# oxfordcontrol/Clarabel.rs

Measured on AMD Instinct MI355X. Metric: IPM iterations/sec (KKT factor+solve) at n=10^6 SOCP, 1/2/4/8 GPUs, higher is better.
Workload: dtype f64

## Files before the change

### clarabel.rs_amd/__init__.py

```python
import ctypes as C
import os
import subprocess

import numpy as np

_HERE = os.path.dirname(os.path.abspath(__file__))
LIB_PATH = os.environ.get("CLARABEL_HIP_LIB") or os.path.join(_HERE, "libclarabel_hip.so")
SHIP_LIB_PATH = os.path.join(_HERE, "libclarabel_hip_ship.so")
HEADER_PATH = os.path.join(os.path.dirname(_HERE), "include", "clarabel_hip.h")

u64 = np.uint64
f64 = np.float64
P_U64 = C.POINTER(C.c_uint64)
P_I64 = C.POINTER(C.c_int64)
P_F64 = C.POINTER(C.c_double)
P_I8 = C.POINTER(C.c_int8)
P_I32 = C.POINTER(C.c_int32)

OK, ERR_DIM, ERR_EMPTY_COLUMN, ERR_NOT_TRIU, ERR_ZERO_PIVOT, ERR_BAD_PERM = 0, -1, -2, -3, -4, -5
ERR_NOT_FACTORED, ERR_NO_DEVICE, ERR_HIP, ERR_ARG, ERR_UNSUPPORTED = -6, -7, -8, -9, -10
ERR_UPDATE_NOT_ALLOWED = -11
STATUS_NAMES = {0: "ok", -1: "IncompatibleDimension", -2: "EmptyColumn", -3: "NotUpperTriangular",
                -4: "ZeroPivot", -5: "InvalidPermutation", -6: "NotFactored", -7: "NoDevice", -8: "HipError",
                -9: "BadArgument", -10: "Unsupported", -11: "UpdateNotAllowed"}
# ... 1471 lines not shown
            continue
        if form[0] == "full":
            idxs.append(offsets[k] + np.arange(length, dtype=np.int64))
        elif form[0] == "partial":
            if np.any(form[1] >= np.uint64(length)):
                raise ChipError(ERR_DIM, "update %s: member %d: an index is out of the member's range" % (key, k))
            idxs.append(offsets[k] + form[1].astype(np.int64))
        else:
            raise TypeError("update %s: member %d: the entries of a list are host arrays" % (key, k))
        vals.append(form[2])
    if not idxs:
        return ("none",)
    return ("partial", _u(np.concatenate(idxs)), _f(np.concatenate(vals)))


COMM_ID_BYTES = 128


def comm_unique_id():
    buf = (C.c_uint8 * COMM_ID_BYTES)()
    _check(lib().chip_comm_get_unique_id(buf), "chip_comm_get_unique_id")
    return bytes(buf)


class Comm:

    def __init__(self, unique_id, world, rank, device=-1):
        assert len(unique_id) == COMM_ID_BYTES
        self._h = C.c_void_p()
        buf = (C.c_uint8 * COMM_ID_BYTES).from_buffer_copy(unique_id)
        _check(lib().chip_comm_create(C.byref(self._h), buf, C.c_int32(world), C.c_int32(rank), C.c_int32(device)),
               "chip_comm_create")
        self.world, self.rank = world, rank

    def __del__(self):
        if getattr(self, "_h", None):
            lib().chip_comm_destroy(self._h)
            self._h = None

    def attach(self, kkt):
        _check(lib().chip_kkt_attach_comm(kkt._h, self._h), "attach_comm")

    def allgather_step(self, kkt, send_ptr, recv_ptr, counts):
        cnt = np.ascontiguousarray(counts, dtype=np.int64)
        assert len(cnt) == self.world
        _check(lib().chip_kkt_allgather_step(kkt._h, self._h, C.c_void_p(send_ptr), C.c_void_p(recv_ptr),
                                             cnt.ctypes.data_as(P_I64)), "allgather_step")

    def wait(self, kkt):
        _check(lib().chip_kkt_wait_comm(kkt._h, self._h), "wait_comm")

    def debug_spin(self, blocks, threads=256, usec=60.0):
        lib().chip_comm_debug_spin.argtypes = [C.c_void_p, C.c_int32, C.c_int32, C.c_double]
        _check(lib().chip_comm_debug_spin(self._h, blocks, threads, float(usec)), "comm_debug_spin")

    def synchronize(self):
        _check(lib().chip_comm_synchronize(self._h), "comm_synchronize")

    def allreduce(self, vals, op="sum"):
        v = np.ascontiguousarray(np.atleast_1d(vals), dtype=np.float64).copy()
        _check(lib().chip_comm_allreduce(self._h, _pf(v), C.c_int32(len(v)), C.c_int32({"sum": 0, "min": 1, "max": 2}[op])),
               "comm_allreduce")
        return v

    def barrier(self):
        self.allreduce([0.0])


_HIPRT = None


def _hiprt():
    global _HIPRT
    if _HIPRT is None:
        lib()
        _HIPRT = C.CDLL("libamdhip64.so.7")
    return _HIPRT


class DeviceArray:

    def __init__(self, n_or_array):
        rt = _hiprt()
        host = None
        if not np.isscalar(n_or_array):
            host = _f(n_or_array)
            n = len(host)
        else:
            n = int(n_or_array)
        self.n = n
        self._p = C.c_void_p()
        rc = rt.hipMalloc(C.byref(self._p), C.c_size_t(max(n, 1) * 8))
        if rc != 0:
            raise RuntimeError("hipMalloc failed: %d" % rc)
        if host is not None:
            self.copy_from(host)
        else:
            rt.hipMemset(self._p, 0, C.c_size_t(max(n, 1) * 8))

    @classmethod
    def view(cls, ptr, n):
        a = cls.__new__(cls)
        a.n = int(n)
        a._p = C.c_void_p(ptr)
        a._borrowed = True
        return a

    @property
    def ptr(self):
        return self._p.value

    def copy_from(self, host):
        host = _f(host)
        assert len(host) == self.n
        rc = _hiprt().hipMemcpy(self._p, host.ctypes.data_as(C.c_void_p), C.c_size_t(self.n * 8), C.c_int(1))
        if rc != 0:
            raise RuntimeError("hipMemcpy H2D failed: %d" % rc)

    def numpy(self):
        out = np.zeros(self.n)
        rc = _hiprt().hipMemcpy(out.ctypes.data_as(C.c_void_p), self._p, C.c_size_t(self.n * 8), C.c_int(2))
        if rc != 0:
            raise RuntimeError("hipMemcpy D2H failed: %d" % rc)
        return out

    def __del__(self):
        if getattr(self, "_borrowed", False):
            return
        if getattr(self, "_p", None) and self._p.value:
            try:
                _hiprt().hipFree(self._p)
            except Exception:
                pass
            self._p = C.c_void_p()


def debug_spin(device, blocks, threads=256, lds_bytes=0, usec=1000.0):
    lib().chip_debug_spin.argtypes = [C.c_int32, C.c_int32, C.c_int32, C.c_int32, C.c_double]
    _check(lib().chip_debug_spin(device, blocks, threads, lds_bytes, float(usec)), "debug_spin")


def debug_set_switch(name, value=None):
    lib().chip_debug_set_switch.argtypes = [C.c_char_p, C.c_char_p]
    _check(lib().chip_debug_set_switch(name.encode(), None if value is None else str(value).encode()), "debug_set_switch")


def debug_counter(kkt, name):
    out = C.c_double(0.0)
    lib().chip_debug_counter.argtypes = [C.c_void_p, C.c_char_p, C.POINTER(C.c_double)]
    _check(lib().chip_debug_counter(kkt._h, name.encode(), C.byref(out)), "debug_counter")
    return out.value


def set_device(ordinal):
    rc = _hiprt().hipSetDevice(C.c_int(int(ordinal)))
    if rc != 0:
        raise RuntimeError("hipSetDevice(%d) failed: %d" % (ordinal, rc))


def device_synchronize():
    _hiprt().hipDeviceSynchronize()
```

### clarabel.rs_amd/csrc/bundle_ir.hip

```cpp
#include "dev_common.hpp"
#include "bundle_symv.hpp"
#include "grid_sync.hpp"

namespace chip {
namespace dev {

namespace {

constexpr int IR_SH_FWD = 3, IR_SH_BWD = 3, IR_SH_SYMV = 3;
constexpr int IR_RPT = 2;
constexpr int IR_FATCAP = 256;

template <bool FWDMODE, int SH, int RPT, int TW>
__device__ __forceinline__ void bundle_sweep_cols(const LdlView &v, const BundleView &bv, int b, double *xs,
                                                  const double *xt, double *tacc, int k, int *fat, int &nfat,
                                                  const double *__restrict__ dinv = nullptr) {
    constexpr int CH = RPT * TW;
    const int s0 = bv.bundle_ptr[b], nloc = bv.bundle_ptr[b + 1] - s0;
    const int *lv = bv.blvl + bv.blvl_ptr[b];
    const int nl = bv.blvl_ptr[b + 1] - bv.blvl_ptr[b] - 1;
    const int lane = threadIdx.x & 63, wv = threadIdx.x >> 6;
    if (FWDMODE && (int)threadIdx.x < 8) tacc[threadIdx.x] = 0.0;
    double tpart = 0.0;
    struct Chunk {
// ... 97 lines not shown
#pragma unroll
                        for (int e = 0; e < SH; ++e) {
                            ii[u][e] = (tb[u] + e < te[u]) ? ci[u][e] : -1;
                            vv[u][e] = cv[u][e];
                        }
                } else {
#pragma unroll
                    for (int u = 0; u < RPT; ++u)
#pragma unroll
                        for (int e = 0; e < SH; ++e) {
                            const unsigned t = (unsigned)(tb[u] + kk + e);
                            const bool ok = (int)t < te[u];
                            ii[u][e] = ok ? (int)v.Li16[t] : -1;
                            vv[u][e] = ok ? v.Lx[t] : 0.0;
                        }
                }
#pragma unroll
                for (int u = 0; u < RPT; ++u)
#pragma unroll
                    for (int e = 0; e < SH; ++e) {
                        const int i = ii[u][e];
                        if (FWDMODE) {
                            const double val = vv[u][e] * yj[u];
                            int tgt = -1;
                            if (i >= 0) {
                                if (i < nloc) tgt = i;
                                else if (k == 1) tpart += val;
                                else atomicAdd(&tacc[i - nloc], val);
                            }
                            lds_scatter_add(xs, tgt, -val);
                        } else if (i >= 0) {
                            sum[u] += vv[u][e] * (i < nloc ? xs[i] : xt[i - nloc]);
                        }
                    }
            }
            if (!FWDMODE) {
#pragma unroll
                for (int u = 0; u < RPT; ++u)
                    if (jr[u] >= 0) xs[jr[u] - s0] = xs[jr[u] - s0] * dj[u] - sum[u];
            }
        }
        if (!FWDMODE && level_ends) {
            __syncthreads();
            const int nf = min(nfat, IR_FATCAP);
            for (int f = wv; f < nf; f += TW / 64) {
                const int j = fat[f];
                double sacc = 0.0;
                for (int t = v.Lp[j] + lane; t < v.Lp[j + 1]; t += 64) {
                    const int i = (int)v.Li16[t];
                    sacc += v.Lx[t] * (i < nloc ? xs[i] : xt[i - nloc]);
                }
                sacc = wave_sum(sacc);
                if (lane == 0) xs[j - s0] -= sacc;
            }
        }
        cur = nx1;
        nx1 = nx2;
        nx2 = advance(nx2);
    }
    __syncthreads();
    if (FWDMODE && k == 1) {
        tpart = wave_sum_all(tpart);
        if (lane == 0 && tpart != 0.0) atomicAdd(&tacc[0], tpart);
        __syncthreads();
    }
}

constexpr int FLAT_U = 4;
constexpr int FLAT_MAXLEV = 64;
constexpr int FLAT_MIN_NODES = 512;
__device__ __forceinline__ void flat_level_table(const LdlView &v, const BundleView &bv, int b, int *lev_e) {
    const int *lv = bv.blvl + bv.blvl_ptr[b];
    const int nl = bv.blvl_ptr[b + 1] - bv.blvl_ptr[b] - 1;
    if ((int)threadIdx.x <= nl && nl <= FLAT_MAXLEV) lev_e[threadIdx.x] = v.Lp[lv[threadIdx.x]];
}
template <bool FWDMODE, int TW>
__device__ __forceinline__ void bundle_sweep_flat(const LdlView &v, const BundleView &bv, int b, double *xs,
                                                  const double *xt, double *tacc, int k, const int *lev_e, int dl = 0) {
    const int s0 = bv.bundle_ptr[b], nloc = bv.bundle_ptr[b + 1] - s0;
    const int nl = bv.blvl_ptr[b + 1] - bv.blvl_ptr[b] - 1;
    int tid = threadIdx.x;
    asm volatile("" : "+v"(tid));
    const int lane = tid & 63;
    if (FWDMODE && tid < 8) tacc[tid] = 0.0;
    if (!FWDMODE)
        for (int i = tid; i < nloc; i += TW) xs[i] *= v.Dinv[s0 + i];
    double tpart = 0.0;
    int step = 0, base = 0, ee = 0;
    auto level_range = [&](int st_, int &eb_, int &ee_) {
        const int l = FWDMODE ? st_ : nl - 1 - st_;
        eb_ = lev_e[l];
        ee_ = lev_e[l + 1];
    };
    auto skip_empty = [&]() {
        while (step < nl) {
            level_range(step, base, ee);
            if (base < ee) return;
            ++step;
        }
    };
    lds_barrier();
    if (TW == 512) {
        for (int st_ = 0; st_ < nl; ++st_) {
            int eb_, ee_;
            level_range(st_, eb_, ee_);
            for (int bs = eb_; bs < ee_; bs += TW * FLAT_U) {
                int ii[FLAT_U], jj[FLAT_U];
                double vv[FLAT_U];
#pragma unroll
                for (int u = 0; u < FLAT_U; ++u) {
                    const int t = bs + u * TW + tid;
                    const bool ok = t < ee_;
                    ii[u] = ok ? (int)v.Li16[t + dl] : -1;
                    jj[u] = ok ? (int)v.Lj16[t + dl] : 0;
                    vv[u] = ok ? v.Lx[t] : 0.0;
                }
#pragma unroll
                for (int u = 0; u < FLAT_U; ++u) {
                    const int i = ii[u];
                    if (i < 0) continue;
                    if (FWDMODE) {
                        const double val = vv[u] * xs[jj[u]];
                        if (i < nloc) atomicAdd(&xs[i], -val);
                        else if (k == 1) tpart += val;
                        else atomicAdd(&tacc[i - nloc], val);
                    } else {
                        atomicAdd(&xs[jj[u]], -(vv[u] * (i < nloc ? xs[i] : xt[i - nloc])));
                    }
                }
            }
            lds_barrier();
        }
        if (FWDMODE && k == 1) {
            tpart = wave_sum_all(tpart);
            if (lane == 0 && tpart != 0.0) atomicAdd(&tacc[0], tpart);
        }
        lds_barrier();
        return;
    }
    skip_empty();
    int ci[FLAT_U], cj[FLAT_U], ni[FLAT_U], nj[FLAT_U];
    double cv[FLAT_U], nv[FLAT_U];
    auto request = [&](int bs, int en, int *ii, int *jj, double *vv) {
#pragma unroll
        for (int u = 0; u < FLAT_U; ++u) {
            const int t = bs + u * TW + tid;
            const bool ok = t < en;
            ii[u] = ok ? (int)v.Li16[t + dl] : -1;
            jj[u] = ok ? (int)v.Lj16[t + dl] : 0;
            vv[u] = ok ? v.Lx[t] : 0.0;
        }
    };
    if (step < nl) request(base, ee, ci, cj, cv);
    while (step < nl) {
        int nstep = step, nbase = base + TW * FLAT_U, nee = ee;
        if (nbase >= nee) {
            nstep = step + 1;
            while (nstep < nl) {
                level_range(nstep, nbase, nee);
                if (nbase < nee) break;
                ++nstep;
            }
        }
        if (nstep < nl) request(nbase, nee, ni, nj, nv);
#pragma unroll
        for (int u = 0; u < FLAT_U; ++u) {
            const int i = ci[u];
            if (i < 0) continue;
            if (FWDMODE) {
                const double val = cv[u] * xs[cj[u]];
                if (i < nloc) atomicAdd(&xs[i], -val);
                else if (k == 1) tpart += val;
                else atomicAdd(&tacc[i - nloc], val);
            } else {
                atomicAdd(&xs[cj[u]], -(cv[u] * (i < nloc ? xs[i] : xt[i - nloc])));
            }
        }
        if (nstep != step) lds_barrier();
        step = nstep;
        base = nbase;
        ee = nee;
#pragma unroll
        for (int u = 0; u < FLAT_U; ++u) {
            ci[u] = ni[u];
            cj[u] = nj[u];
            cv[u] = nv[u];
        }
    }
    if (FWDMODE && k == 1) {
        tpart = wave_sum_all(tpart);
        if (lane == 0 && tpart != 0.0) atomicAdd(&tacc[0], tpart);
    }
    lds_barrier();
}

template <int TW>
__device__ __forceinline__ void bundle_symv_flat(const LdlView &v, const BundleView &bv, const double *x,
                                                 const double *__restrict__ b, double *spill, double *xs, double *red,
                                                 int k, int bid, const double *xt, double *out_norm, double *out_share) {
    const int *__restrict__ Up = v.Up;
    const unsigned short *__restrict__ Ucol16 = v.Ucol16, *__restrict__ Urow16 = v.Urow16;
    const double *__restrict__ Ux = v.Ux;
    const int s0 = bv.bundle_ptr[bid], nloc = bv.bundle_ptr[bid + 1] - s0;
    const int nleaf = bv.blvl[bv.blvl_ptr[bid] + 1] - s0, nin = nloc - nleaf;
    int tid = threadIdx.x;
    asm volatile("" : "+v"(tid));
    auto xpos = [&](int t) { return t < nleaf ? t : nloc + (t - nleaf); };
    constexpr int LR = 4, LS = 3;
    int tb[LR], te[LR];
#pragma unroll
    for (int u = 0; u < LR; ++u) {
        const int i = tid + u * TW;
        tb[u] = i < nleaf ? Up[s0 + i] : 0;
        te[u] = i < nleaf ? Up[s0 + i + 1] : 0;
    }
    const int fb = Up[s0 + nleaf], fe = Up[s0 + nloc];
    for (int t = tid; t < nin; t += TW) {
        const double xv = x[s0 + nleaf + t], bv_ = b[s0 + nleaf + t];
        xs[xpos(t)] = xv;
        xs[nleaf + t] = bv_;
    }
    double tpart = 0.0;
    __shared__ double tacc3[8];
    if (k > 1 && tid < 8) tacc3[tid] = 0.0;
    double mleaf = 0.0;
    bool nan = false;
    __syncthreads();
    for (int w0 = 0; w0 < nleaf; w0 += LR * TW) {
        int jj[LR][LS];
        double vv[LR][LS], xi[LR], bi[LR], acc[LR];
#pragma unroll
        for (int u = 0; u < LR; ++u) {
            const int i = w0 + tid + u * TW;
            xi[u] = i < nleaf ? x[s0 + i] : 0.0;
            bi[u] = i < nleaf ? b[s0 + i] : 0.0;
            acc[u] = 0.0;
#pragma unroll
            for (int q = 0; q < LS; ++q) {
                const int t = tb[u] + q;
                const bool ok = t < te[u];
                jj[u][q] = ok ? (int)Ucol16[t] : -1;
                vv[u][q] = ok ? Ux[t] : 0.0;
            }
        }
#pragma unroll
        for (int u = 0; u < LR; ++u) {
            const int i = w0 + tid + u * TW;
            auto apply = [&](int j, double val) {
                if (j >= nloc) {
                    acc[u] += val * xt[j - nloc];
                    if (k == 1) tpart += val * xi[u];
                    else atomicAdd(&tacc3[j - nloc], val * xi[u]);
                } else if (j == i) {
                    acc[u] += val * xi[u];
                } else {
                    acc[u] += val * xs[xpos(j - nleaf)];
                    atomicAdd(&xs[j], -(val * xi[u]));
                }
            };
#pragma unroll
            for (int q = 0; q < LS; ++q)
                if (jj[u][q] >= 0) apply(jj[u][q], vv[u][q]);
            for (int t = tb[u] + LS; t < te[u]; ++t) apply((int)Ucol16[t], Ux[t]);
            if (i < nleaf) {
                const double val = bi[u] - acc[u];
                spill[s0 + i] = val;
                if (val != val) nan = true;
                else mleaf = fmax(mleaf, fabs(val));
            }
            const int in = i + LR * TW;
            tb[u] = in < nleaf ? Up[s0 + in] : 0;
            te[u] = in < nleaf ? Up[s0 + in + 1] : 0;
        }
    }
    int ii[FLAT_U], jj[FLAT_U], ni[FLAT_U], nj[FLAT_U];
    double vv[FLAT_U], nv[FLAT_U];
    auto request = [&](int bs, int *pi, int *pj, double *pv) {
#pragma unroll
        for (int u = 0; u < FLAT_U; ++u) {
            const int t = bs + u * TW + tid;
            const bool ok = t < fe;
            pi[u] = ok ? (int)Urow16[t] : -1;
            pj[u] = ok ? (int)Ucol16[t] : 0;
            pv[u] = ok ? Ux[t] : 0.0;
        }
    };
    if (fb < fe) request(fb, ii, jj, vv);
    for (int base = fb; base < fe; base += TW * FLAT_U) {
        if (base + TW * FLAT_U < fe) request(base + TW * FLAT_U, ni, nj, nv);
        else {
#pragma unroll
            for (int u = 0; u < FLAT_U; ++u) ni[u] = -1;
        }
#pragma unroll
        for (int u = 0; u < FLAT_U; ++u) {
            const int i = ii[u], j = jj[u];
            if (i < 0) continue;
            const double xi = xs[xpos(i - nleaf)];
            if (j >= nloc) {
                atomicAdd(&xs[i], -(vv[u] * xt[j - nloc]));
                if (k == 1) tpart += vv[u] * xi;
                else atomicAdd(&tacc3[j - nloc], vv[u] * xi);
            } else if (j == i) {
                atomicAdd(&xs[i], -(vv[u] * xi));
            } else {
                atomicAdd(&xs[i], -(vv[u] * xs[xpos(j - nleaf)]));
// ... 407 lines not shown
                    for (int i = tid; i < nloc; i += TW) alt[s0 + i] = xs[i];
                } else {
                    for (int i = tid; i < nloc; i += TW) alt[s0 + i] = 1.0 * cur[s0 + i] + 1.0 * xs[i];
                }
                if (!ir.ir_enable) {
                    double mx = 0.0;
                    bool nan = false;
                    for (int i = tid; i < nloc; i += TW) {
                        const double val = xs[i];
                        if (val != val) nan = true;
                        else mx = fmax(mx, fabs(val));
                    }
                    mx = block_max(mx, red);
                    const bool anynan = __syncthreads_or(nan);
                    if (tid == 0) ir_store(&pn[(size_t)par * nb + b], anynan ? __longlong_as_double(0x7ff8000000000000ll) : mx);
                    continue;
                }
                __syncthreads();
                stamp();
                double *share_out = GR ? &gf.rsh[((size_t)par * nb + b) * 8] : &shs[(size_t)par * nb * k + (size_t)b * k];
                if (single && bv.symv_split && flat)
                    bundle_symv_flat<TW>(v, bv, alt, ir.bp, ir.ebuf, xs, red, k, b, st.candt, &pn[(size_t)par * nb + b], share_out);
                else if (single && bv.symv_split)
                    bundle_symv_split<IR_SH_SYMV, TW, 2>(bv, v.Up, v.Ucol16, v.Ux, alt, ir.bp, ir.ebuf, xs, red, k, b, st.candt,
                                                         &pn[(size_t)par * nb + b], share_out);
                else
                    bundle_symv_body<true, IR_SH_SYMV, TW, 2>(bv, v.Up, (const int *)v.Ucol16, v.Ux, alt, ir.bp, single ? nullptr : ir.ebuf, nullptr, nullptr,
                                       xs, red, lfold, b, st.candt, &pn[(size_t)par * nb + b], share_out);
                if (GR && grp >= 0) {
                    ++gph;
                    if (ir_group_arrive(gf.gcnt + grp * 32, gnb * gph)) {
                        group_sums(gf.rsh + (size_t)par * nb * 8);
                        if (tid == 0) {
                            double m = 0.0, mb = 0.0;
                            for (int i = 0; i < k; ++i) {
                                double sacc = st.tacc[i];
                                for (int c = 0; c < k; ++c) sacc += st.ktt[i * 8 + c] * st.candt[c];
                                const double rt = st.btop[i] - sacc;
                                ir_store(&grec[par * 32 + 16 + i], rt);
                                m = nanmax(m, fabs(rt));
                                mb = nanmax(mb, fabs(st.btop[i]));
                            }
                            ir_store(&grec[par * 32 + 24], m);
                            ir_store(&grec[par * 32 + 25], mb);
                        }
                    }
                }
            }
        }
        if (stop) break;
        pending = true;
        const bool more_possible = ir.ir_enable && round < ir.maxiter;
        if (GR && more_possible) {
            if (tid == 0) st.gen += 1;
            if (ir_arrive_nowait(ir.ctl, st.gen, G) == IR_LAST) {
                reduce_residual(par, round == 0);
                ir_release(ir.ctl, st.gen, G);
            }
            continue;
        }
        if (folded && more_possible) continue;
        stamp();
        if (tid == 0) st.gen += 1;
        const int state = ir_arrive_wait(ir.ctl, st.gen, G);
        if (state == IR_TIMEOUT) {
            if (tid == 0) ir.res[2] = 1;
            return;
        }
        stamp();
        if (state == IR_LAST) {
            reduce_residual(par, round == 0);
            ir_release(ir.ctl, st.gen, G);
        }
        __syncthreads();
        decide(round, par);
        pending = false;
        if (__builtin_amdgcn_readfirstlane(st.done)) break;
    }
    stamp();
    const int ok = __builtin_amdgcn_readfirstlane(st.ok);
    if (ok) {
        double *cur = __builtin_amdgcn_readfirstlane(st.sel) ? ir.xb : ir.xa;
        auto put = [&](int j, double val) {
            const int o = ir.perm[j];
            if (o < ir.n) {
                if (ir.lhsx) ir.lhsx[o] = val;
            } else if (o < ir.n + ir.m) {
                if (ir.lhsz) ir.lhsz[o - ir.n] = val;
            }
        };
        for (int b = blockIdx.x; b < nb; b += G) {
            const int s0 = bv.bundle_ptr[b], nloc = bv.bundle_ptr[b + 1] - s0;
            const int nruns = ir.runs ? ir.run_ptr[b + 1] - ir.run_ptr[b] : 0;
            if (nruns > 0 && nruns <= IR_MAXRUNS) {
                __syncthreads();
                if (tid < 3 * nruns) st.runs[tid] = ir.runs[3 * ir.run_ptr[b] + tid];
                __syncthreads();
                int r = 0;
                for (int i = tid; i < nloc; i += TW) {
                    while (i >= st.runs[3 * r] + st.runs[3 * r + 2]) ++r;
                    const int o = st.runs[3 * r + 1] + (i - st.runs[3 * r]);
                    const double val = cur[s0 + i];
                    if (o < ir.n) {
                        if (ir.lhsx) ir.lhsx[o] = val;
                    } else if (o < ir.n + ir.m) {
                        if (ir.lhsz) ir.lhsz[o - ir.n] = val;
                    }
                }
            } else {
                for (int i = tid; i < nloc; i += TW) put(s0 + i, cur[s0 + i]);
            }
        }
        if ((GR ? gfirst : blockIdx.x == 0) && tid < k) {
            put(topnode(tid), st.curt[tid]);
            cur[topnode(tid)] = st.curt[tid];
        }
    }
    if (GR && gfirst && tid == 0) {
        __hip_atomic_store(gf.gcnt + grp * 32, 0, __ATOMIC_RELAXED, __HIP_MEMORY_SCOPE_AGENT);
        __hip_atomic_store(gf.gcnt + grp * 32 + 1, 0, __ATOMIC_RELAXED, __HIP_MEMORY_SCOPE_AGENT);
    }
    if (blockIdx.x == 0 && tid == 0) {
        ir.res[0] = ok ? 1 : -1;
        ir.res[1] = st.rounds;
        ir.res[3] = st.sel;
        pub[64] = st.normb;
        pub[65] = st.norme;
    }
    stamp();
    ir_grid_exit(ir.ctl, __builtin_amdgcn_readfirstlane(st.gen) + 1, G);
}


constexpr int IRS_NPT = 12;
__device__ __forceinline__ int opaque_tid() {
    int t = threadIdx.x;
    asm volatile("" : "+v"(t));
    return t;
}

struct RunWalk {
    const int *runs;
    int r;
    __device__ __forceinline__ int orig(int i) {
        while (i >= runs[3 * r] + runs[3 * r + 2]) ++r;
        return runs[3 * r + 1] + (i - runs[3 * r]);
    }
};

template <int TW, int NPT, int NLP>
__device__ __forceinline__ void irs_symv(const LdlView &v, const IrView &ir, const int *runs, const double (&c)[NPT],
                                         bool keep_e, double *xs, double *red, double *tacc3, int k, int s0,
                                         int nloc, int nleaf, const double *xt, double *out_norm, double *out_share,
                                         int du) {
    double cl[NLP];
    const int *__restrict__ Up = v.Up;
    const unsigned short *__restrict__ Ucol16 = v.Ucol16, *__restrict__ Urow16 = v.Urow16;
    const double *__restrict__ Ux = v.Ux;
    const int tid = opaque_tid();
    auto xpos = [&](int t) { return t < nleaf ? t : nloc + (t - nleaf); };
    auto rhs_of = [&](int o) { return o < ir.n ? ir.rx[o] : (o < ir.n + ir.m ? ir.rz[o - ir.n] : 0.0); };
    constexpr int LR = 4, LS = 3;
    static_assert(NLP % LR == 0 && NLP <= NPT, "leaf passes");
    int tb[LR], te[LR];
#pragma unroll
    for (int u = 0; u < LR; ++u) {
        const int i = tid + u * TW;
        tb[u] = i < nleaf ? Up[s0 + i] : 0;
        te[u] = i < nleaf ? Up[s0 + i + 1] : 0;
    }
    const int fb = Up[s0 + nleaf], fe = Up[s0 + nloc];
    {
        RunWalk rw{runs, 0};
        double bq[NPT];
#pragma unroll
        for (int u = 0; u < NPT; ++u) {
            const int i = tid + u * TW;
            bq[u] = (i >= nleaf && i < nloc) ? rhs_of(rw.orig(i)) : 0.0;
        }
        lds_barrier();
#pragma unroll
        for (int u = 0; u < NPT; ++u) {
            const int i = tid + u * TW;
            if (i >= nleaf && i < nloc) {
                xs[xpos(i - nleaf)] = c[u];
                xs[i] = bq[u];
            }
        }
#pragma unroll
        for (int u = 0; u < NLP; ++u) cl[u] = c[u];
    }
    double tpart = 0.0;
    if (k > 1 && tid < 8) tacc3[tid] = 0.0;
    double mleaf = 0.0;
    bool nan = false;
    lds_barrier();
    RunWalk rl{runs, 0};
#pragma unroll
    for (int p = 0; p < NLP / LR; ++p) {
        if (p * LR * TW < nleaf) {
            int jj[LR][LS];
            double vv[LR][LS], bi[LR], acc[LR];
#pragma unroll
            for (int u = 0; u < LR; ++u) {
                const int i = (p * LR + u) * TW + tid;
                bi[u] = i < nleaf ? rhs_of(rl.orig(i)) : 0.0;
                acc[u] = 0.0;
#pragma unroll
                for (int q = 0; q < LS; ++q) {
                    const int t = tb[u] + q;
                    const bool ok = t < te[u];
                    jj[u][q] = ok ? (int)Ucol16[t + du] : -1;
                    vv[u][q] = ok ? Ux[t] : 0.0;
                }
            }
#pragma unroll
            for (int u = 0; u < LR; ++u) {
                const int i = (p * LR + u) * TW + tid;
                const double xi = cl[p * LR + u];
                auto apply = [&](int j, double val) {
                    if (j >= nloc) {
                        acc[u] += val * xt[j - nloc];
                        if (k == 1) tpart += val * xi;
                        else atomicAdd(&tacc3[j - nloc], val * xi);
                    } else if (j == i) {
                        acc[u] += val * xi;
                    } else {
                        acc[u] += val * xs[xpos(j - nleaf)];
                        atomicAdd(&xs[j], -(val * xi));
                    }
                };
#pragma unroll
                for (int q = 0; q < LS; ++q)
                    if (jj[u][q] >= 0) apply(jj[u][q], vv[u][q]);
                for (int t = tb[u] + LS; t < te[u]; ++t) apply((int)Ucol16[t + du], Ux[t]);
                if (i < nleaf) {
                    const double val = bi[u] - acc[u];
                    if (keep_e) cl[p * LR + u] = val;
                    if (val != val) nan = true;
                    else mleaf = fmax(mleaf, fabs(val));
                }
                const int in = i + LR * TW;
                tb[u] = in < nleaf ? Up[s0 + in] : 0;
                te[u] = in < nleaf ? Up[s0 + in + 1] : 0;
            }
        }
    }
    {
        int ii[FLAT_U], jj[FLAT_U], ni[FLAT_U], nj[FLAT_U];
        double vv[FLAT_U], nv[FLAT_U];
        auto request = [&](int bs, int *pi, int *pj, double *pv) {
#pragma unroll
            for (int u = 0; u < FLAT_U; ++u) {
                const int t = bs + u * TW + tid;
                const bool ok = t < fe;
                pi[u] = ok ? (int)Urow16[t + du] : -1;
                pj[u] = ok ? (int)Ucol16[t + du] : 0;
                pv[u] = ok ? Ux[t] : 0.0;
            }
        };
        if (fb < fe) request(fb, ii, jj, vv);
        for (int base = fb; base < fe; base += TW * FLAT_U) {
            if (base + TW * FLAT_U < fe) request(base + TW * FLAT_U, ni, nj, nv);
            else {
#pragma unroll
                for (int u = 0; u < FLAT_U; ++u) ni[u] = -1;
            }
#pragma unroll
            for (int u = 0; u < FLAT_U; ++u) {
                const int i = ii[u], j = jj[u];
                if (i < 0) continue;
                const double xi = xs[xpos(i - nleaf)];
                if (j >= nloc) {
                    atomicAdd(&xs[i], -(vv[u] * xt[j - nloc]));
                    if (k == 1) tpart += vv[u] * xi;
                    else atomicAdd(&tacc3[j - nloc], vv[u] * xi);
                } else if (j == i) {
                    atomicAdd(&xs[i], -(vv[u] * xi));
                } else {
                    atomicAdd(&xs[i], -(vv[u] * xs[xpos(j - nleaf)]));
                    atomicAdd(&xs[j], -(vv[u] * xi));
                }
            }
#pragma unroll
            for (int u = 0; u < FLAT_U; ++u) {
                ii[u] = ni[u];
                jj[u] = nj[u];
                vv[u] = nv[u];
            }
        }
    }
    lds_barrier();
    double m = mleaf;
#pragma unroll
    for (int u = 0; u < NPT; ++u) {
        const int i = tid + u * TW;
        if (i >= nleaf && i < nloc) {
            const double val = xs[i];
            if (val != val) nan = true;
            else m = fmax(m, fabs(val));
        }
    }
    if (keep_e) {
#pragma unroll
        for (int u = 0; u < NLP; ++u)
            if (tid + u * TW < nleaf) xs[tid + u * TW] = cl[u];
    }
    m = block_max(m, red);
    const bool anynan = __syncthreads_or(nan);
    if (tid == 0)
        __hip_atomic_store(out_norm, anynan ? __longlong_as_double(0x7ff8000000000000ll) : m, __ATOMIC_RELAXED,
                           __HIP_MEMORY_SCOPE_AGENT);
    if (k == 1) {
        tpart = block_sum(tpart, red);
        if (tid == 0) __hip_atomic_store(out_share, tpart, __ATOMIC_RELAXED, __HIP_MEMORY_SCOPE_AGENT);
    } else if (k > 1) {
        lds_barrier();
        if (tid == 0)
            for (int i = 0; i < k; ++i)
                __hip_atomic_store(out_share + i, tacc3[i], __ATOMIC_RELAXED, __HIP_MEMORY_SCOPE_AGENT);
    }
}

template <int TW, int NLP>
__global__ __launch_bounds__(TW) __attribute__((amdgpu_waves_per_eu(4, 4)))
void k_bundle_irs(LdlView v, BundleView bv, FoldView fold, IrView ir) {
    constexpr int NPT = IRS_NPT;
    extern __shared__ __attribute__((aligned(16))) char smem[];
    double *xs = (double *)smem;
    __shared__ double red[16];
    __shared__ int lev_e[FLAT_MAXLEV + 1];
    __shared__ double tacc3[8];
    __shared__ IrState st;
    __shared__ int pat[2];
    const int nb = bv.nb, G = gridDim.x, tid = threadIdx.x, b = blockIdx.x;
    const int k = fold.k;
    const bool folded = k > 0;
    const int NF = k ? fold.NF : ir.N;
    if (ir.test_drop && b == G - 1 && G > 1) return;
    const int s0 = bv.bundle_ptr[b], nloc = bv.bundle_ptr[b + 1] - s0;
    const int nleaf = bv.blvl[bv.blvl_ptr[b] + 1] - s0;
    double *pnb = ir.part;
    double *pn = pnb + nb;
    double *shf = pn + 2 * nb;
    double *shs = shf + (size_t)nb * k;
    double *pub = shs + 2 * (size_t)nb * k;
    auto rhs_of = [&](int o) { return o < ir.n ? ir.rx[o] : (o < ir.n + ir.m ? ir.rz[o - ir.n] : 0.0); };
    if (tid == 0) {
        st.normb = st.norme = st.lastnorme = 0.0;
        st.rounds = 0;
        st.ok = 1;
        st.done = 0;
        st.sel = 0;
        st.par = 0;
        st.gen = 0;
        st.pad = 0;
        pat[0] = ir.pat_off ? ir.pat_off[2 * b] : 0;
        pat[1] = ir.pat_off ? ir.pat_off[2 * b + 1] : 0;
        if (b == 0) {
            ir.res[0] = 0;
            ir.res[2] = 0;
        }
    }
    if (tid < 64) {
        st.ltt[tid] = 0.0;
        st.ktt[tid] = 0.0;
    }
    {
        const int r0 = ir.run_ptr[b], nruns = ir.run_ptr[b + 1] - r0;
        if (tid < 3 * nruns) st.runs[tid] = ir.runs[3 * r0 + tid];
    }
    flat_level_table(v, bv, b, lev_e);
    __syncthreads();
    auto load_top_constants = [&]() {
        if (tid < 8) {
            st.btop[tid] = tid < k ? rhs_of(ir.perm[NF + tid]) : 0.0;
            if (ir.bp && tid < k && b == 0) ir.bp[NF + tid] = st.btop[tid];
            st.curt[tid] = 0.0;
            st.dinvt[tid] = tid < k ? v.Dinv[NF + tid] : 0.0;
        } else if (tid >= 64 && tid < 64 + k * k) {
            const int ti = (tid - 64) / k, tj = (tid - 64) % k;
            const int q = fold.tt[tid - 64];
            if (q >= 0) st.ltt[ti * 8 + tj] = v.Lx[q];
        } else if (tid >= 128 && tid < 128 + k) {
            const int i = tid - 128;
            for (int t = fold.sp[i]; t < fold.sp[i + 1]; ++t) st.ktt[i * 8 + fold.scol[t]] += v.Ux[fold.sslot[t]];
        }
    };
    if (k == 0) load_top_constants();
    int dbgn = 0;
    auto stamp = [&]() {
        if (ir.dbg_all) {
            if (tid == 0 && dbgn < 31) {
                if (dbgn == 0)
                    ir.dbg_all[(size_t)b * 32] = (long long)__builtin_amdgcn_s_getreg((32 - 1) << 11 | 4) |
                                                 ((long long)__builtin_amdgcn_s_getreg((32 - 1) << 11 | 20) << 32);
                ir.dbg_all[(size_t)b * 32 + 1 + dbgn++] = wall_clock64();
            }
        } else if (ir.dbg && tid == 0 && (b == 0 || b == G / 2) && dbgn < 64)
            ir.dbg[(b ? 64 : 0) + dbgn++] = wall_clock64();
    };
    __shared__ double redm[4 * 16];
    const int nmsg = 2 * k + 2;
    const int tagbase = ir.epoch << 8;
    auto barrier = [&](bool fwd, bool resid, int rpar, bool first) -> int {
        if (tid == 0) st.gen += 1;
        const int state = ir_arrive_nowait(ir.ctl, st.gen, G);
        const int tag = tagbase | (__builtin_amdgcn_readfirstlane(st.gen) & 0xff);
        if (state == IR_LAST) {
            double f0 = 0.0, r0 = 0.0, mb = 0.0, m = 0.0;
            for (int q = tid; q < nb; q += TW) {
                if (fwd && k >= 1) f0 += ir_load(&shf[(size_t)q * k]);
                if (resid) {
                    if (first) mb = nanmax(mb, ir_load(&pnb[q]));
                    m = nanmax(m, ir_load(&pn[(size_t)rpar * nb + q]));
                    if (ir.ir_enable && k >= 1) r0 += ir_load(&shs[(size_t)rpar * nb * k + (size_t)q * k]);
                }
            }
            f0 = wave_sum(f0);
            r0 = wave_sum(r0);
#pragma unroll
            for (int o = 32; o > 0; o >>= 1) {
                mb = nanmax(mb, __shfl_down(mb, o, 64));
                m = nanmax(m, __shfl_down(m, o, 64));
            }
            const int lane = tid & 63, wv = tid >> 6;
            if (lane == 0) {
                redm[wv * 4 + 0] = f0;
                redm[wv * 4 + 1] = r0;
                redm[wv * 4 + 2] = mb;
                redm[wv * 4 + 3] = m;
            }
            __syncthreads();
            if (tid == 0) {
                double tf = redm[0], tr = redm[1], tmb = redm[2], tm = redm[3];
                for (int w = 1; w < TW / 64; ++w) {
                    tf += redm[w * 4 + 0];
                    tr += redm[w * 4 + 1];
                    tmb = nanmax(tmb, redm[w * 4 + 2]);
                    tm = nanmax(tm, redm[w * 4 + 3]);
                }
                if (k >= 1) {
                    st.pubv[0] = tf;
                    st.pubv[k + 2] = tr;
                }
                st.pubv[k] = tm;
                if (first || !resid) st.pubv[k + 1] = tmb;
            }
            for (int i = 1; i < k; ++i) {
                double pf = 0.0, pr = 0.0;
                for (int q = tid; q < nb; q += TW) {
                    if (fwd) pf += ir_load(&shf[(size_t)q * k + i]);
                    if (resid && ir.ir_enable) pr += ir_load(&shs[(size_t)rpar * nb * k + (size_t)q * k + i]);
                }
                pf = block_sum(pf, red);
                pr = block_sum(pr, red);
                if (tid == 0) {
                    st.pubv[i] = pf;
                    st.pubv[k + 2 + i] = pr;
                }
            }
            __syncthreads();
            ir_publish(ir.rel, st.pubv, nmsg, tag, G);
            return IR_LAST;
        }
        return ir_wait_record(ir.rel, st.pubv, nmsg, tag);
    };
    auto decide = [&](int round, int par) {
        if (tid == 0) {
            double m = st.pubv[k];
            if (round == 0) {
                double nbm = st.pubv[k + 1];
                for (int i = 0; i < k; ++i) nbm = nanmax(nbm, fabs(st.btop[i]));
                st.normb = nbm;
            }
            for (int i = 0; i < k; ++i) {
                double sacc = st.pubv[k + 2 + i];
                for (int cc = 0; cc < k; ++cc) sacc += st.ktt[i * 8 + cc] * st.candt[cc];
                st.rtop[i] = ir.ir_enable ? st.btop[i] - sacc : st.candt[i];
                m = nanmax(m, fabs(st.rtop[i]));
            }
            const double newnorm = m, tol = ir.abstol + ir.reltol * st.normb;
            bool accept, done = false;
            if (round == 0) {
                accept = true;
                st.norme = newnorm;
                if (!(newnorm - newnorm == 0.0)) {
                    st.ok = 0;
                    done = true;
                } else if (!ir.ir_enable || ir.maxiter <= 0 || newnorm <= tol) {
                    done = true;
                }
            } else {
                st.rounds += 1;
                if (!(newnorm - newnorm == 0.0)) {
                    st.ok = 0;
                    accept = false;
                    done = true;
                } else {
                    const double improved = st.lastnorme / newnorm;
                    accept = !(improved < ir.stopratio) || improved > 1.0;
                    if (improved < ir.stopratio) done = true;
                    if (accept) st.norme = newnorm;
                }
            }
            st.pad = accept ? 1 : 0;
            if (accept) {
                st.sel ^= 1;
                for (int i = 0; i < k; ++i) st.curt[i] = st.candt[i];
            }
            if (!done && (st.rounds >= ir.maxiter || st.norme <= tol)) done = true;
            st.lastnorme = st.norme;
            st.done = done ? 1 : 0;
        }
        __syncthreads();
    };
    stamp();
    {
        double c[NPT];
        RunWalk rw{st.runs, 0};
#pragma unroll
        for (int u = 0; u < NPT; ++u) {
            const int i = tid + u * TW;
            c[u] = i < nloc ? rhs_of(rw.orig(i)) : 0.0;
        }
        double mx = 0.0;
        bool nan = false;
#pragma unroll
        for (int u = 0; u < NPT; ++u) {
            const int i = tid + u * TW;
            if (i < nloc) {
                xs[i] = c[u];
                if (ir.bp) ir.bp[s0 + i] = c[u];
                if (c[u] != c[u]) nan = true;
                else mx = fmax(mx, fabs(c[u]));
            }
        }
        mx = block_max(mx, red);
        const bool anynan = __syncthreads_or(nan);
        if (tid == 0) ir_store(&pnb[b], anynan ? __longlong_as_double(0x7ff8000000000000ll) : mx);
    }
    bool pending = false;
    double xk[NPT];
    bool xk_valid = false;
    bool spec_done = false;
    for (int round = 0;; ++round) {
        const int par = round & 1;
        __syncthreads();
        stamp();
        bundle_sweep_flat<true, TW>(v, bv, b, xs, nullptr, st.tacc, k, lev_e, __builtin_amdgcn_readfirstlane(pat[0]));
        stamp();
        if (tid < k) ir_store(&shf[(size_t)b * k + tid], st.tacc[tid]);
        if (folded) {
            stamp();
            if (round == 0) load_top_constants();
            if (barrier(true, pending, par ^ 1, round == 1) == IR_TIMEOUT) {
                if (tid == 0) ir.res[2] = 1;
                return;
            }
            stamp();
            if (pending) {
                decide(round - 1, par ^ 1);
                pending = false;
                if (__builtin_amdgcn_readfirstlane(st.done)) break;
            }
            if (tid == 0) {
                for (int i = 0; i < k; ++i) {
                    double sacc = (round == 0 ? st.btop[i] : st.rtop[i]) - st.pubv[i];
                    for (int j = 0; j < i; ++j) sacc -= st.ltt[i * 8 + j] * st.dxt[j];
                    st.dxt[i] = sacc;
                }
                for (int i = k - 1; i >= 0; --i) {
                    double sacc = st.dxt[i] * st.dinvt[i];
                    for (int j = i + 1; j < k; ++j) sacc -= st.ltt[j * 8 + i] * st.dxt[j];
                    st.dxt[i] = sacc;
                }
                for (int i = 0; i < k; ++i)
                    st.candt[i] = round == 0 ? st.dxt[i] : 1.0 * st.curt[i] + 1.0 * st.dxt[i];
            }
        }
        __syncthreads();
        stamp();
        bundle_sweep_flat<false, TW>(v, bv, b, xs, st.dxt, nullptr, k, lev_e, __builtin_amdgcn_readfirstlane(pat[0]));
        stamp();
        const bool more_possible = ir.ir_enable && round < ir.maxiter;
        double c[NPT];
        {
            const int tid = opaque_tid();
            const int sel = __builtin_amdgcn_readfirstlane(st.sel);
            double *cur = sel ? ir.xb : ir.xa;
            double *alt = sel ? ir.xa : ir.xb;
            if (round == 0) {
#pragma unroll
                for (int u = 0; u < NPT; ++u) {
                    const int i = tid + u * TW;
                    c[u] = i < nloc ? xs[i] : 0.0;
                }
            } else {
                if (!xk_valid) {
#pragma unroll
                    for (int u = 0; u < NPT; ++u) {
                        const int i = tid + u * TW;
                        xk[u] = i < nloc ? cur[s0 + i] : 0.0;
                    }
                }
#pragma unroll
                for (int u = 0; u < NPT; ++u) {
                    const int i = tid + u * TW;
                    c[u] = i < nloc ? 1.0 * xk[u] + 1.0 * xs[i] : 0.0;
                }
            }
            if (more_possible && round == 0 && (ir.sf_flags & 1)) {
#pragma unroll
                for (int u = 0; u < NPT; ++u) xk[u] = c[u];
                xk_valid = true;
            } else if (more_possible || !ir.spec_out) {
#pragma unroll
                for (int u = 0; u < NPT; ++u) {
                    const int i = tid + u * TW;
                    if (i < nloc) {
                        alt[s0 + i] = c[u];
                        if (xk_valid) cur[s0 + i] = xk[u];
                    }
                }
                xk_valid = false;
            } else {
                RunWalk rw{st.runs, 0};
#pragma unroll
                for (int u = 0; u < NPT; ++u) {
                    const int i = tid + u * TW;
                    if (i < nloc) {
                        const int o = rw.orig(i);
                        if (o < ir.n) {
                            if (ir.lhsx) ir.lhsx[o] = c[u];
                        } else if (o < ir.n + ir.m) {
                            if (ir.lhsz) ir.lhsz[o - ir.n] = c[u];
                        }
                    }
                }
                spec_done = true;
            }
        }
        if (!ir.ir_enable) {
            double mx = 0.0;
            bool nan = false;
#pragma unroll
            for (int u = 0; u < NPT; ++u) {
                if (tid + u * TW < nloc) {
                    if (c[u] != c[u]) nan = true;
                    else mx = fmax(mx, fabs(c[u]));
                }
            }
            mx = block_max(mx, red);
            const bool anynan = __syncthreads_or(nan);
            if (tid == 0) ir_store(&pn[(size_t)par * nb + b], anynan ? __longlong_as_double(0x7ff8000000000000ll) : mx);
        } else {
            stamp();
            irs_symv<TW, NPT, NLP>(v, ir, st.runs, c, more_possible, xs, red, tacc3, k, s0, nloc, nleaf, st.candt,
                                   &pn[(size_t)par * nb + b], &shs[(size_t)par * nb * k + (size_t)b * k],
                                   __builtin_amdgcn_readfirstlane(pat[1]));
        }
        pending = true;
        if (folded && more_possible) continue;
        stamp();
        if (barrier(false, true, par, round == 0) == IR_TIMEOUT) {
            if (tid == 0) ir.res[2] = 1;
            return;
        }
        stamp();
        decide(round, par);
        pending = false;
        if (__builtin_amdgcn_readfirstlane(st.done)) break;
    }
    stamp();
    const int ok = __builtin_amdgcn_readfirstlane(st.ok);
    if (ok) {
        const bool accepted_last = __builtin_amdgcn_readfirstlane(st.pad) != 0;
        if (!(spec_done && accepted_last)) {
            const int tid = opaque_tid();
            const double *cur = __builtin_amdgcn_readfirstlane(st.sel) ? ir.xb : ir.xa;
            if (!xk_valid) {
#pragma unroll
                for (int u = 0; u < NPT; ++u) {
                    const int i = tid + u * TW;
                    xk[u] = i < nloc ? cur[s0 + i] : 0.0;
                }
            }
            RunWalk rw{st.runs, 0};
#pragma unroll
            for (int u = 0; u < NPT; ++u) {
                const int i = tid + u * TW;
                if (i < nloc) {
                    const int o = rw.orig(i);
                    if (o < ir.n) {
                        if (ir.lhsx) ir.lhsx[o] = xk[u];
                    } else if (o < ir.n + ir.m) {
                        if (ir.lhsz) ir.lhsz[o - ir.n] = xk[u];
                    }
                }
            }
        }
        if (b == 0 && tid < k) {
            const int o = ir.perm[NF + tid];
            if (o < ir.n) {
                if (ir.lhsx) ir.lhsx[o] = st.curt[tid];
            } else if (o < ir.n + ir.m) {
                if (ir.lhsz) ir.lhsz[o - ir.n] = st.curt[tid];
            }
        }
    }
    if (b == 0 && tid == 0) {
        ir.res[0] = ok ? 1 : -1;
        ir.res[1] = st.rounds;
        ir.res[3] = st.sel;
        pub[64] = st.normb;
        pub[65] = st.norme;
    }
    stamp();
    ir_grid_exit(ir.ctl, __builtin_amdgcn_readfirstlane(st.gen) + 1, G);
}

}

int ir_ctl_ints() { return IR_CTL_INTS; }
int ir_rel_ints() { return IR_REL_INTS; }
size_t ir_part_doubles(int nb, int k) { return (size_t)nb * (3 + 3 * (size_t)k) + 72; }
static size_t bundle_ir_lds(const BundleView &bv) {
    return ((size_t)std::max(bv.max_nodes, bv.ir_lds_doubles) * sizeof(double) + 15) & ~(size_t)15;
}
template <int TW> static int bundle_ir_capacity_tw(const BundleView &bv) {
    const size_t lds = bundle_ir_lds(bv);
    if (raise_dynamic_lds((const void *)k_bundle_ir<TW, false>, (size_t)lds) != hipSuccess ||
        raise_dynamic_lds((const void *)k_bundle_ir<TW, true>, (size_t)lds) != hipSuccess) {
        (void)hipGetLastError();
        return 0;
    }
    int per_cu = 0, dev = 0;
    hipDeviceProp_t prop;
    int per_cu_g = 0;
    if (hipOccupancyMaxActiveBlocksPerMultiprocessor(&per_cu, (const void *)k_bundle_ir<TW, false>, TW, lds) != hipSuccess ||
        hipOccupancyMaxActiveBlocksPerMultiprocessor(&per_cu_g, (const void *)k_bundle_ir<TW, true>, TW, lds) != hipSuccess ||
        hipGetDevice(&dev) != hipSuccess || hipGetDeviceProperties(&prop, dev) != hipSuccess) {
        (void)hipGetLastError();
        return 0;
    }
    per_cu = std::min(per_cu, per_cu_g);
    hipFuncAttributes fa;
    if (hipFuncGetAttributes(&fa, (const void *)k_bundle_ir<TW, true>) != hipSuccess) {
        (void)hipGetLastError();
        return 0;
    }
    const size_t per_wg = ((fa.sharedSizeBytes + lds + 1023) / 1024) * 1024;
    const int by_lds = (int)(prop.maxSharedMemoryPerMultiProcessor / per_wg);
    const int by_waves = (TW == 512 ? 24 : 16) / (TW / 64);
    per_cu = std::min(per_cu, std::min(by_lds, by_waves));
    return per_cu * prop.multiProcessorCount;
}
int bundle_ir_capacity(const BundleView &bv, int *tw) {
    if (!bv.nb) return 0;
    const int c256 = bundle_ir_capacity_tw<256>(bv);
    hipDeviceProp_t prop;
    int dev = 0;
    if (hipGetDevice(&dev) != hipSuccess || hipGetDeviceProperties(&prop, dev) != hipSuccess) return 0;
    if (c256 >= 4 * prop.multiProcessorCount) {
        *tw = 256;
        return c256;
    }
    const bool no1024 = false;
    if (!no1024 && bv.nb <= prop.multiProcessorCount) {
        const int c1024 = bundle_ir_capacity_tw<1024>(bv);
        if (c1024 >= bv.nb) {
            *tw = 1024;
            return c1024;
        }
    }
    *tw = 512;
    return bundle_ir_capacity_tw<512>(bv);
}
bool bundle_irs_capacity_ok(const BundleView &bv) {
    if (!bv.nb || !bv.symv_split) return false;
    const size_t lds = bundle_ir_lds(bv);
    if (raise_dynamic_lds((const void *)k_bundle_irs<256, 4>, lds) != hipSuccess) return false;
    int per_cu = 0, dev = 0;
    hipDeviceProp_t prop;
    hipFuncAttributes fa;
    if (hipOccupancyMaxActiveBlocksPerMultiprocessor(&per_cu, (const void *)k_bundle_irs<256, 4>, 256, lds) != hipSuccess ||
        hipGetDevice(&dev) != hipSuccess || hipGetDeviceProperties(&prop, dev) != hipSuccess ||
        hipFuncGetAttributes(&fa, (const void *)k_bundle_irs<256, 4>) != hipSuccess) {
        (void)hipGetLastError();
        return false;
    }
    const size_t per_wg = ((fa.sharedSizeBytes + lds + 1023) / 1024) * 1024;
    per_cu = std::min(per_cu, std::min((int)(prop.maxSharedMemoryPerMultiProcessor / per_wg), 4));
    return per_cu * prop.multiProcessorCount >= bv.nb;
}
bool irs_bundle_ok(int nloc, int nleaf, int nlevels, int nruns) {
    return nloc >= FLAT_MIN_NODES && nloc <= IRS_NPT * 256 && nleaf <= 4 * 256 && nlevels <= FLAT_MAXLEV && nruns > 0 &&
           nruns <= IR_MAXRUNS;
}
int bundle_ir(hipStream_t s, const LdlView &v, const BundleView &bv, const FoldView &fold, const IrView &ir, int grid,
              int tw, const GFoldView &gf) {
    const size_t lds = bundle_ir_lds(bv);
    if (ir.sf) {
        k_bundle_irs<256, 4><<<bv.nb, 256, lds, s>>>(v, bv, fold, ir);
        return (int)hipGetLastError();
    }
    if (gf.ng > 0) {
        if (tw == 256) k_bundle_ir<256, true><<<grid, 256, lds, s>>>(v, bv, fold, ir, gf);
        else if (tw == 1024) k_bundle_ir<1024, true><<<grid, 1024, lds, s>>>(v, bv, fold, ir, gf);
        else k_bundle_ir<512, true><<<grid, 512, lds, s>>>(v, bv, fold, ir, gf);
    } else {
        if (tw == 256) k_bundle_ir<256, false><<<grid, 256, lds, s>>>(v, bv, fold, ir, gf);
        else if (tw == 1024) k_bundle_ir<1024, false><<<grid, 1024, lds, s>>>(v, bv, fold, ir, gf);
        else k_bundle_ir<512, false><<<grid, 512, lds, s>>>(v, bv, fold, ir, gf);
    }
    return (int)hipGetLastError();
}

// ... 3 lines not shown
```

### clarabel.rs_amd/csrc/capi.cpp

```cpp
#include <algorithm>
#include <cmath>
#include <cstdio>
#include <cstdlib>
#include <cstring>
#include <memory>

#include "engine.hpp"
#include "host_util.hpp"
#include "problem_update.hpp"
#include "../../include/clarabel_hip_testing.h"

using namespace chip;

namespace {

thread_local std::string g_last;

const i64 *as_i64(const uint64_t *p) { return reinterpret_cast<const i64 *>(p); }

void fill_info(const Engine &E, chip_info *info) {
    std::memset(info, 0, sizeof(*info));
    std::strncpy(info->name, "hip", sizeof(info->name) - 1);
    info->threads = 1;
    info->direct = 1;
// ... 30 lines not shown
        state += 3 * side * side + 2 * side;
        maxdim = std::max<int>(maxdim, (int)side);
        scratch_stride = maxdim > 64 ? 4LL * maxdim * maxdim + 4LL * maxdim + 16 : 0;
    }
};
template <typename Mem>
int psd_view_build(Mem &mem, dev::PsdView &pv, const PsdSizing &sz, const int *mapHs, int *fail_flag) {
    int rc;
    const size_t nc = sz.start.size();
    int *q[4] = {nullptr, nullptr, nullptr, nullptr};
    const std::vector<int> *src[4] = {&sz.start, &sz.dim, &sz.hs, &sz.off};
    for (int k = 0; k < 4; k++) {
        if ((rc = mem.alloc(&q[k], nc))) return rc;
        if (nc) CHIP_HIP(hipMemcpy(q[k], src[k]->data(), nc * sizeof(int), hipMemcpyHostToDevice));
    }
    double *qs;
    if ((rc = mem.alloc(&qs, (size_t)(sz.state ? sz.state : 1)))) return rc;
    pv.ncones = (int)nc;
    pv.maxdim = sz.maxdim;
    pv.scratch = nullptr;
    pv.scratch_stride = sz.scratch_stride;
    if (sz.scratch_stride)
        if ((rc = mem.alloc(&pv.scratch, (size_t)sz.scratch_stride * nc))) return rc;
    pv.start = q[0];
    pv.dim = q[1];
    pv.hs_start = q[2];
    pv.state_off = q[3];
    pv.state = qs;
    pv.mapHs = mapHs;
    pv.fail = fail_flag;
    return CHIP_OK;
}

#ifdef CHIP_TESTING
struct DebugPsd {
    PsdSizing sz;
    i64 m = 0;
    DevPool mem;
    dev::PsdView pv{};
    int *fail_flag = nullptr;
    int gen = 0, last_jacobi_lds = 0;
    bool uploaded = false;
    int device = 0;
    hipStream_t stream = nullptr;
    ~DebugPsd() {
        if (stream) {
            (void)hipStreamSynchronize(stream);
            (void)hipStreamDestroy(stream);
        }
    }
    int ready() {
        if (uploaded) {
            CHIP_HIP(hipSetDevice(device));
            return CHIP_OK;
        }
        if (chip_device_count() < 1) return fail(CHIP_ERR_NO_DEVICE, "chip_debug_psd: no HIP device");
        CHIP_HIP(hipGetDevice(&device));
        int rc;
        if ((rc = mem.alloc(&fail_flag, 1))) return rc;
        CHIP_HIP(hipMemset(fail_flag, 0, sizeof(int)));
        if ((rc = psd_view_build(mem, pv, sz, nullptr, fail_flag))) return rc;
        CHIP_HIP(hipMemset(pv.state, 0, (size_t)(sz.state ? sz.state : 1) * sizeof(double)));
        CHIP_HIP(hipStreamCreateWithFlags(&stream, hipStreamNonBlocking));
        uploaded = true;
        return CHIP_OK;
    }
};
struct DebugPsdStage {
    DevPool mem;
    struct Buf {
        void *host, *dev;
        size_t bytes;
    };
    std::vector<Buf> outs;
    int in(const double *host, size_t len, const double **devp) {
        double *d = nullptr;
        *devp = nullptr;
        if (!host) return CHIP_OK;
        int rc = mem.upload(&d, host, len);
        *devp = d;
        return rc;
    }
    int out(double *host, size_t len, double **devp) {
        *devp = nullptr;
        if (!host) return CHIP_OK;
        int rc = mem.upload(devp, (const double *)host, len);
        if (rc) return rc;
        outs.push_back(Buf{host, *devp, len * sizeof(double)});
        return CHIP_OK;
    }
    int finish(hipStream_t s) {
        CHIP_HIP(hipGetLastError());
        CHIP_HIP(hipStreamSynchronize(s));
        for (const Buf &b : outs)
            if (b.bytes) CHIP_HIP(hipMemcpy(b.host, b.dev, b.bytes, hipMemcpyDeviceToHost));
        return CHIP_OK;
    }
};
#endif

}

struct chip_ldl {
    Engine E;
    std::vector<double> hK;
    bool dirty = true;
    double *d_b = nullptr, *d_x = nullptr, *d_y = nullptr;
    struct IndexSet {
        int *pos = nullptr;
        int8_t *signs = nullptr;
        i64 k = 0;
    };
    std::vector<IndexSet> sets;
    double *d_vals = nullptr;
    i64 d_vals_cap = 0;
    bool dev_values = false;
    double *r_bp = nullptr, *r_x = nullptr, *r_e = nullptr, *r_w = nullptr;
    std::vector<void *> pinned;
    ~chip_ldl() {
        for (void *p : pinned) (void)hipHostUnregister(p);
    }
};

struct chip_kkt {
    KktLayout K;
    Engine E;
    int *mapHs = nullptr, *diag_full = nullptr, *mapP = nullptr, *mapA = nullptr;
    int nn_count = 0, zero_count = 0;
    int *nn_rows = nullptr, *nn_hsidx = nullptr, *zero_rows = nullptr;
    dev::SocView soc{};
    dev::Ns3View ns3{};
    dev::GpwView gpw{};
    std::vector<int> gpw_cone_index, gpw_state_off, gpw_dim1;
    dev::PsdView psd{};
    bool has_hostHs = false;
    double *d_s = nullptr, *d_z = nullptr, *d_w = nullptr, *d_lam = nullptr;
    double *d_rhs = nullptr, *d_lhs = nullptr;
    struct SolveVecs {
        double *bp = nullptr, *x = nullptr, *e = nullptr, *dx = nullptr;
        int last_ir = 0;
    } wk[2];
    double *d_tmp = nullptr;
    size_t tmp_len = 0;
    double last_eps = 0;
    bool scaling_pending_check = false;
    bool psd_rows_all_blocks = false;
    int scaling_gen = 0;
    bool x_holds_b = false;
    double static_diag_max = 0.0;
    const double *rhs_x = nullptr, *rhs_z = nullptr;
    bool rhs_deferred = false;
    int *ir_run_ptr = nullptr, *ir_runs = nullptr;
    bool ir_sf = false, bp_stale = false;
    int pend_update = 0;
    int pend_update_ok = 1;
    std::vector<int> pend_slots;
    struct FusedArgs {
        const double *rx, *rz;
        double *lx, *lz;
    } fused_args[Engine::IR_RING] = {};
    int fused_fallbacks = 0;
    #ifdef CHIP_TESTING
    bool ir_test_drop = switches().ir_test_drop;
#else
    static constexpr bool ir_test_drop = false;
#endif
    int world = 1;
    double *d_partial = nullptr;
    int partial_cap = 0;
    std::vector<double> h_partial;
};

extern "C" {

void chip_settings_default(chip_settings *s) {
    std::memset(s, 0, sizeof(*s));
    s->static_regularization_enable = 1;
    s->static_regularization_constant = 1e-8;
    s->static_regularization_proportional = 2.220446049250313e-16 * 2.220446049250313e-16;
    s->dynamic_regularization_enable = 1;
    s->dynamic_regularization_eps = 1e-13;
    s->dynamic_regularization_delta = 2e-7;
    s->iterative_refinement_enable = 1;
    s->iterative_refinement_reltol = 1e-13;
    s->iterative_refinement_abstol = 1e-12;
    s->iterative_refinement_max_iter = 10;
    s->iterative_refinement_stop_ratio = 5.0;
    s->device = -1;
    s->amd_dense_scale = 1.5;
    s->use_graph = 0;
    s->linesearch_backtrack_step = 0.8;
    s->min_terminate_step_length = 1e-4;
}

int32_t chip_auto_select(double lnz, double n_div, double n_mult_subs_ldl) {
    const double flops = n_div + n_mult_subs_ldl, thresh = 40.0;
    return (flops / lnz) < thresh ? 0 : 1;
}

const char *chip_last_error(void) {
    g_last = get_error();
    return g_last.c_str();
}

int32_t chip_device_count(void) {
    int n = 0;
    if (hipGetDeviceCount(&n) != hipSuccess) return 0;
    return n;
}

int32_t chip_amd_order(int64_t n, const uint64_t *colptr, const uint64_t *rowval, double dense_scale,
                       uint64_t *perm, uint64_t *iperm, double *info3) {
    if (n < 0 || !colptr || !perm) return fail(CHIP_ERR_ARG, "chip_amd_order: bad argument");
    for (i64 c = 0; c < n; c++)
        for (uint64_t p = colptr[c]; p < colptr[c + 1]; p++)
            if (rowval[p] > (uint64_t)c) return fail(CHIP_ERR_NOT_TRIU, "matrix is not upper triangular");
    std::vector<i64> p;
    AmdInfo info;
    int rc = amd_order(n, as_i64(colptr), as_i64(rowval), dense_scale, p, &info);
    if (rc) return fail(CHIP_ERR_ARG, "amd_order failed");
    for (i64 k = 0; k < n; k++) {
        perm[k] = (uint64_t)p[k];
        if (iperm) iperm[p[k]] = (uint64_t)k;
    }
    if (info3) {
        info3[0] = info.lnz;
        info3[1] = info.ndiv;
        info3[2] = info.nmultsubs_ldl;
    }
    return CHIP_OK;
}

static int target_workgroups(const chip_settings &st) {
    if (switches().has_target_wg) return switches().target_wg;
    if (st.device == CHIP_DEVICE_HOST_ONLY) return 1024;
    int dev = st.device, cus = 0;
    if (dev < 0 && hipGetDevice(&dev) != hipSuccess) return 1024;
    if (hipDeviceGetAttribute(&cus, hipDeviceAttributeMultiprocessorCount, dev) != hipSuccess || cus <= 0) {
        (void)hipGetLastError();
        return 1024;
    }
    return 4 * cus;
}

int32_t chip_ldl_create(chip_ldl **out, int64_t n, const uint64_t *colptr, const uint64_t *rowval,
                        const double *nzval, const int8_t *dsigns, const uint64_t *perm_or_null,
                        const chip_settings *settings) {
    if (!out || n < 0 || !colptr || !rowval || !nzval) return fail(CHIP_ERR_ARG, "chip_ldl_create: bad argument");
    *out = nullptr;
    switches_reload();
    chip_settings st;
    if (settings) st = *settings;
    else chip_settings_default(&st);
    std::vector<i64> perm0;
    if (perm_or_null) perm0.assign(as_i64(perm_or_null), as_i64(perm_or_null) + n);
    Symbolic S;
    int rc = analyse(n, as_i64(colptr), as_i64(rowval), dsigns, perm0, st.amd_dense_scale, S, 0);
    if (rc) return rc;
    std::unique_ptr<chip_ldl> h(new chip_ldl());
    h->hK.assign(nzval, nzval + S.nnzK);
    if (st.device == CHIP_DEVICE_HOST_ONLY) {
        h->E.init_host_only(S, st);
        *out = h.release();
        return CHIP_OK;
    }
    rc = h->E.init(S, st);
    if (rc) return rc;
    h->dirty = true;
    if ((rc = h->E.alloc(&h->d_b, (size_t)n))) return rc;
    if ((rc = h->E.alloc(&h->d_x, (size_t)n))) return rc;
    if ((rc = h->E.alloc(&h->d_y, (size_t)n))) return rc;
    *out = h.release();
    return CHIP_OK;
}

void chip_ldl_destroy(chip_ldl *h) { delete h; }

static int ldl_plain_on_device(chip_ldl *h, int kind, const uint64_t *index, const double *values, double scalar,
                               const int8_t *signs, int64_t k);
int32_t chip_ldl_update_values(chip_ldl *h, const uint64_t *index, const double *values, int64_t k) {
    if (!h) return CHIP_ERR_ARG;
    if (h->dev_values) return ldl_plain_on_device(h, 0, index, values, 0.0, nullptr, k);
    for (i64 i = 0; i < k; i++) {
        if (index[i] >= (uint64_t)h->E.nnzK) return fail(CHIP_ERR_ARG, "update_values: index out of range");
        h->hK[index[i]] = values[i];
    }
    h->dirty = true;
    return CHIP_OK;
}
int32_t chip_ldl_scale_values(chip_ldl *h, const uint64_t *index, double scale, int64_t k) {
    if (!h) return CHIP_ERR_ARG;
    if (h->dev_values) return ldl_plain_on_device(h, 1, index, nullptr, scale, nullptr, k);
    for (i64 i = 0; i < k; i++) {
        if (index[i] >= (uint64_t)h->E.nnzK) return fail(CHIP_ERR_ARG, "scale_values: index out of range");
        h->hK[index[i]] *= scale;
    }
    h->dirty = true;
    return CHIP_OK;
}
int32_t chip_ldl_offset_values(chip_ldl *h, const uint64_t *index, double offset, const int8_t *signs,
                               int64_t k) {
    if (!h) return CHIP_ERR_ARG;
    if (h->dev_values) return ldl_plain_on_device(h, 2, index, nullptr, offset, signs, k);
    for (i64 i = 0; i < k; i++) {
        if (index[i] >= (uint64_t)h->E.nnzK) return fail(CHIP_ERR_ARG, "offset_values: index out of range");
        if (signs[i] > 0) h->hK[index[i]] += offset;
        else if (signs[i] < 0) h->hK[index[i]] -= offset;
    }
    h->dirty = true;
    return CHIP_OK;
}
int32_t chip_ldl_set_values(chip_ldl *h, const double *kkt_nzval) {
    if (!h || !kkt_nzval) return CHIP_ERR_ARG;
    std::memcpy(h->hK.data(), kkt_nzval, (size_t)h->E.nnzK * sizeof(double));
    h->dirty = true;
    h->dev_values = false;
    return CHIP_OK;
}
extern "C++" {
namespace chip {
int kkt_device(const ::chip_kkt *h) { return h->E.device; }
hipStream_t kkt_stream(::chip_kkt *h) { return h->E.host_only ? nullptr : h->E.stream; }
void kkt_set_world(::chip_kkt *h, int world) { h->world = world; }
int kkt_note_exchange(::chip_kkt *h, hipStream_t comm_stream) {
    Engine &E = h->E;
    if (!E.exch_event && hipEventCreateWithFlags(&E.exch_event, hipEventDisableTiming) != hipSuccess) {
        (void)hipGetLastError();
        E.exch_event = nullptr;
        return CHIP_ERR_HIP;
    }
    if (hipEventRecord(E.exch_event, comm_stream) != hipSuccess) {
        (void)hipGetLastError();
        return CHIP_ERR_HIP;
    }
    E.exch_pending = true;
    return CHIP_OK;
}
bool kkt_host_only(const ::chip_kkt *h) { return h->E.host_only; }
int kkt_update_values_dev(::chip_kkt *h, int block, const double *src_dev, const int64_t *idx_dev, int k) {
    Engine &E = h->E;
    if (E.host_only) return fail(CHIP_ERR_NO_DEVICE, "host-only handle: no numeric work without a GPU");
    dev::pu_scatter(E.stream, E.Kx, block == 0 ? h->mapP : h->mapA, src_dev, idx_dev, k);
    CHIP_HIP(hipGetLastError());
    return CHIP_OK;
}
void kkt_set_static_diag_max(::chip_kkt *h, double v) { h->static_diag_max = v; }
}
}

#define NEED_DEVICE(E) \
    if ((E).host_only) return fail(CHIP_ERR_NO_DEVICE, "host-only handle: no numeric work without a GPU")

int32_t chip_ldl_get_symbolic(const chip_ldl *h, uint64_t *etree, uint64_t *Lp, uint64_t *Li,
                              uint64_t *lvlptr) {
    if (!h) return CHIP_ERR_ARG;
    return h->E.get_symbolic(etree, Lp, Li, lvlptr);
}

int32_t chip_ldl_refactor(chip_ldl *h) {
    if (!h) return CHIP_ERR_ARG;
    Engine &E = h->E;
    NEED_DEVICE(E);
    CHIP_HIP(hipSetDevice(E.device));
    if (h->dirty && !h->dev_values && E.nnzK) {
        int rc = E.upload_values(h->hK.data());
        if (rc) return rc;
    }
    h->dirty = false;
    return E.refactor(false, nullptr);
}
int32_t chip_ldl_solve_dev(chip_ldl *h, double *x_dev, const double *b_dev) {
    if (!h) return CHIP_ERR_ARG;
    Engine &E = h->E;
    NEED_DEVICE(E);
    if (!E.factored) return fail(CHIP_ERR_NOT_FACTORED, "solve() before the first refactor()");
    CHIP_HIP(hipSetDevice(E.device));
    dev::permute_in(E.stream, h->d_y, b_dev, E.perm, E.N);
    E.enqueue_solve_inplace(E.ctx[0], h->d_y);
    dev::permute_out(E.stream, x_dev, h->d_y, E.perm, E.N);
    CHIP_HIP(hipGetLastError());
    return CHIP_OK;
}
int32_t chip_ldl_solve(chip_ldl *h, double *x, const double *b) {
    if (!h) return CHIP_ERR_ARG;
    Engine &E = h->E;
    NEED_DEVICE(E);
    if (!E.factored) return fail(CHIP_ERR_NOT_FACTORED, "solve() before the first refactor()");
    CHIP_HIP(hipSetDevice(E.device));
    const size_t bytes = (size_t)E.N * sizeof(double);
    if (E.N) CHIP_HIP(hipMemcpyAsync(h->d_b, b, bytes, hipMemcpyHostToDevice, E.stream));
    int rc = chip_ldl_solve_dev(h, h->d_x, h->d_b);
    if (rc) return rc;
    if (E.N) CHIP_HIP(hipMemcpyAsync(x, h->d_x, bytes, hipMemcpyDeviceToHost, E.stream));
    CHIP_HIP(hipStreamSynchronize(E.stream));
    return CHIP_OK;
}
int32_t chip_ldl_info(const chip_ldl *h, chip_info *info) {
    if (!h || !info) return CHIP_ERR_ARG;
    fill_info(h->E, info);
    if (h->E.factored && !h->E.host_only) {
        i64 c = 0;
        int rc = count_positive(const_cast<Engine &>(h->E), &c);
        if (rc) return rc;
        info->positive_inertia = c;
    }
    return CHIP_OK;
}
int32_t chip_ldl_get_perm(const chip_ldl *h, uint64_t *perm) {
    if (!h || !perm) return CHIP_ERR_ARG;
    for (int i = 0; i < h->E.N; i++) perm[i] = (uint64_t)h->E.h_perm[i];
    return CHIP_OK;
}
int32_t chip_ldl_get_factors(chip_ldl *h, uint64_t *Lp, uint64_t *Li, double *Lx, double *D, double *Dinv) {
    if (!h) return CHIP_ERR_ARG;
    Engine &E = h->E;
    NEED_DEVICE(E);
    CHIP_HIP(hipSetDevice(E.device));
    CHIP_HIP(hipStreamSynchronize(E.stream));
    const size_t n = (size_t)E.N, nl = (size_t)E.nnzL;
    std::vector<int> tmp;
    if (Lp) {
        tmp.resize(n + 1);
        CHIP_HIP(hipMemcpy(tmp.data(), E.Lp, (n + 1) * sizeof(int), hipMemcpyDeviceToHost));
        for (size_t i = 0; i <= n; i++) Lp[i] = (uint64_t)tmp[i];
    }
    if (Li && nl) {
        tmp.resize(nl);
        CHIP_HIP(hipMemcpy(tmp.data(), E.Li, nl * sizeof(int), hipMemcpyDeviceToHost));
        for (size_t i = 0; i < nl; i++) Li[i] = (uint64_t)tmp[i];
    }
    if (Lx && nl) CHIP_HIP(hipMemcpy(Lx, E.Lx, nl * sizeof(double), hipMemcpyDeviceToHost));
    if (D && n) CHIP_HIP(hipMemcpy(D, E.D, n * sizeof(double), hipMemcpyDeviceToHost));
    if (Dinv && n) CHIP_HIP(hipMemcpy(Dinv, E.Dinv, n * sizeof(double), hipMemcpyDeviceToHost));
    return CHIP_OK;
}

static std::vector<int> narrow_plain(const std::vector<i64> &v, size_t n) {
    std::vector<int> o(n);
    for (size_t i = 0; i < n; i++) o[i] = (int)v[i];
    return o;
}

int32_t chip_kkt_create(chip_kkt **out, int64_t n, int64_t m, const uint64_t *Pcolptr,
                        const uint64_t *Prowval, const double *Pnzval, const uint64_t *Acolptr,
                        const uint64_t *Arowval, const double *Anzval, int64_t ncones,
                        const int32_t *cone_tags, const int64_t *cone_dims, const int64_t *cone_dims2,
                        const double *cone_alphas_or_null, const chip_settings *settings,
                        const uint64_t *perm_or_null) {
    if (!out || n < 0 || m < 0 || !Pcolptr || !Acolptr) return fail(CHIP_ERR_ARG, "chip_kkt_create: bad argument");
    *out = nullptr;
    switches_reload();
    chip_settings st;
    if (settings) st = *settings;
    else chip_settings_default(&st);
    std::unique_ptr<chip_kkt> h(new chip_kkt());
    KktLayout &K = h->K;
    i64 mm = 0;
    PhaseClock clk;
    clk.tag = "kkt_create";
    int rc = build_cone_specs(ncones, cone_tags, cone_dims, cone_dims2, K.cones, mm, K.p, K.nHs);
    if (rc) return CHIP_ERR_ARG;
    if (mm != m) return fail(CHIP_ERR_DIM, "cone dimensions do not add up to m");
    rc = assemble_kkt_triu(n, m, as_i64(Pcolptr), as_i64(Prowval), Pnzval, as_i64(Acolptr), as_i64(Arowval),
                           Anzval, K);
    if (rc) return rc;
    clk("KKT assembly");
    std::vector<i64> perm0;
    if (perm_or_null) perm0.assign(as_i64(perm_or_null), as_i64(perm_or_null) + K.N);
    Symbolic S;
    std::vector<i32> clique_of;
    {
        i32 g = 0;
        for (const ConeSpec &c : K.cones)
            if (!c.hs_diag && c.numel >= 16) {
                if (clique_of.empty()) clique_of.assign((size_t)K.N, -1);
                for (i64 r = 0; r < c.numel; r++) clique_of[(size_t)(n + c.start + r)] = g;
                g++;
            }
    }
    rc = analyse(K.N, K.colptr.data(), K.rowval.data(), K.dsigns.data(), perm0, st.amd_dense_scale, S, target_workgroups(st),
                 clique_of.empty() ? nullptr : &clique_of);
    if (rc) return rc;
    clk("analysis (total)");
    Engine &E = h->E;
    PatternShare pat;
    {
        const i32 nbun = S.bundle_ptr.empty() ? 0 : (i32)S.bundle_ptr.size() - 1;
        bool cand = !S.Li16.empty() && S.gf_ng == 0 && S.nfold >= 1 && nbun > 0;
        for (i32 b = 0; b < nbun && cand; b++) {
            const i32 s0 = S.bundle_ptr[(size_t)b], nloc = S.bundle_ptr[(size_t)b + 1] - s0;
            const i32 nleaf = S.blvl[(size_t)S.blvl_ptr[(size_t)b] + 1] - s0;
            cand = dev::irs_bundle_ok(nloc, nleaf, S.blvl_ptr[(size_t)b + 1] - S.blvl_ptr[(size_t)b] - 1, 1);
        }
        if (cand) {
            bundle_pattern_classes(S, pat);
            E.note_patterns(pat);
            clk("pattern classes");
        }
    }
    if (st.device == CHIP_DEVICE_HOST_ONLY) {
        E.init_host_only(S, st);
        *out = h.release();
        return CHIP_OK;
    }
    rc = E.init(S, st);
    if (rc) return rc;
    clk("engine init (uploads)");
    if (K.nnz) {
        rawvec<double> vx((size_t)K.nnz);
        run_threads(K.nnz >= (i64)1 << 22 ? host_threads() : 1, [&](int t, int TT) {
            for (i64 u = K.nnz * t / TT; u < K.nnz * (t + 1) / TT; u++) vx[(size_t)u] = K.nzval[(size_t)S.v2k[(size_t)u]];
        });
        CHIP_HIP(hipMemcpy(E.Kx, vx.data(), (size_t)K.nnz * sizeof(double), hipMemcpyHostToDevice));
    }
    const bigvec &k2v = S.k2v;
    auto narrow = [&k2v](const auto &v, size_t cnt) {
        rawvec<int> o(cnt);
        run_threads(cnt >= (size_t)1 << 22 ? host_threads() : 1, [&](int t, int TT) {
            for (size_t i = cnt * (size_t)t / (size_t)TT; i < cnt * (size_t)(t + 1) / (size_t)TT; i++) o[i] = k2v[(size_t)v[i]];
        });
        return o;
    };
    {
        double mx = 0.0;
        for (i64 i = 0; i < K.n; i++) {
            const double a = K.nzval[(size_t)K.diagP[(size_t)i]];
            if (a != a) mx = a;
            else if (mx == mx) mx = std::max(mx, std::fabs(a));
        }
        h->static_diag_max = mx;
    }

    if ((rc = E.upload(&h->mapHs, narrow(K.mapHs, (size_t)K.nHs), (size_t)K.nHs))) return rc;
    if ((rc = E.upload(&h->diag_full, narrow(K.diag_full, (size_t)K.N), (size_t)K.N))) return rc;
    const size_t nnzP = (size_t)Pcolptr[n], nnzA = (size_t)Acolptr[n];
    if ((rc = E.upload(&h->mapP, narrow(K.mapP, nnzP), nnzP))) return rc;
    if ((rc = E.upload(&h->mapA, narrow(K.mapA, nnzA), nnzA))) return rc;

    std::vector<int> nn_rows, nn_hs, zero_rows, s_start, s_dim, s_hs, s_sidx, s_ptr, mapU, mapV, mapD;
    std::vector<int> n3_start, n3_hs, n3_tag;
    PsdSizing pd;
    std::vector<int> gp_start, gp_d1, gp_d2, gp_hs, gp_off, gp_mapptr, gp_map, gp_mapD;
    i64 gp_state = 0;
    std::vector<double> n3_alpha;
    for (const ConeSpec &c : K.cones) {
        if (c.tag == CHIP_CONE_NONNEGATIVE) {
            for (i64 k = 0; k < c.numel; k++) {
                nn_rows.push_back((int)(c.start + k));
                nn_hs.push_back((int)(c.block_start + k));
            }
        } else if (c.tag == CHIP_CONE_ZERO) {
            for (i64 k = 0; k < c.numel; k++) zero_rows.push_back((int)(c.start + k));
        } else if (c.tag == CHIP_CONE_SECONDORDER) {
            s_start.push_back((int)c.start);
            s_dim.push_back((int)c.numel);
            s_hs.push_back((int)c.block_start);
            s_sidx.push_back((int)c.sparse_idx);
        } else if (c.tag == CHIP_CONE_EXPONENTIAL || c.tag == CHIP_CONE_POWER) {
            const size_t ci = (size_t)(&c - K.cones.data());
            n3_start.push_back((int)c.start);
            n3_hs.push_back((int)c.block_start);
            n3_tag.push_back((int)c.tag);
            const double al = cone_alphas_or_null ? cone_alphas_or_null[ci] : 0.5;
            if (c.tag == CHIP_CONE_POWER && !(al > 0.0 && al < 1.0))
                return fail(CHIP_ERR_ARG, "PowerConeT exponent must lie in (0,1)");
            n3_alpha.push_back(al);
        } else if (c.tag == CHIP_CONE_GENPOWER) {
            gp_start.push_back((int)c.start);
            gp_d1.push_back((int)c.dim);
            gp_d2.push_back((int)c.dim2);
            gp_hs.push_back((int)c.block_start);
            gp_off.push_back((int)gp_state);
            gp_state += 6 * c.dim + 4 * c.dim2 + 3;
            gp_mapptr.push_back((int)gp_map.size());
            const i64 sidx = c.sparse_idx;
            for (i64 k = 0; k < c.dim; k++) gp_map.push_back(k2v[(size_t)K.sp_q[K.sp_q_ptr[sidx] + k]]);
            for (i64 k = 0; k < c.dim2; k++) gp_map.push_back(k2v[(size_t)K.sp_r[K.sp_r_ptr[sidx] + k]]);
            for (i64 k = 0; k < c.numel; k++) gp_map.push_back(k2v[(size_t)K.sp_u[K.sp_ptr[sidx] + k]]);
            for (int k = 0; k < 3; k++) gp_mapD.push_back(k2v[(size_t)K.sp_D[3 * sidx + k]]);
            h->gpw_cone_index.push_back((int)(&c - K.cones.data()));
        } else if (c.tag == CHIP_CONE_PSDTRIANGLE) {
            pd.add(c.start, c.dim, c.block_start);
        } else {
            h->has_hostHs = true;
        }
    }
    {
        dev::GpwView &gv = h->gpw;
        gv.ncones = (int)gp_start.size();
        int *g1, *g2, *g3, *g4, *g5, *g6, *g7, *g8;
        double *gs;
        if ((rc = E.upload(&g1, gp_start, gp_start.size()))) return rc;
        if ((rc = E.upload(&g2, gp_d1, gp_d1.size()))) return rc;
        if ((rc = E.upload(&g3, gp_d2, gp_d2.size()))) return rc;
        if ((rc = E.upload(&g4, gp_hs, gp_hs.size()))) return rc;
        if ((rc = E.upload(&g5, gp_off, gp_off.size()))) return rc;
        if ((rc = E.upload(&g6, gp_mapptr, gp_mapptr.size()))) return rc;
        if ((rc = E.upload(&g7, gp_map, gp_map.size()))) return rc;
        if ((rc = E.upload(&g8, gp_mapD, gp_mapD.size()))) return rc;
        std::vector<double> st0((size_t)(gp_state ? gp_state : 1), 0.0);
        for (size_t c = 0; c < gp_start.size(); c++) {
            double *st = st0.data() + gp_off[c];
            for (int k = 0; k < gp_d1[c]; k++) st[k] = 1.0 / gp_d1[c];
            st[6 * gp_d1[c] + 4 * gp_d2[c] + 1] = 1.0;
            st[6 * gp_d1[c] + 4 * gp_d2[c] + 2] = (double)gp_d1[c];
        }
        if ((rc = E.upload(&gs, st0, st0.size()))) return rc;
        gv.start = g1;
        gv.dim1 = g2;
        gv.dim2 = g3;
        gv.hs_start = g4;
        gv.state_off = g5;
        gv.map_ptr = g6;
        gv.mapQRP = g7;
        gv.mapD = g8;
        gv.mapHs = h->mapHs;
        gv.state = gs;
        h->gpw_state_off = gp_off;
        h->gpw_dim1 = gp_d1;
    }
    {
        dev::PsdView &pv = h->psd;
        if ((rc = psd_view_build(E, pv, pd, h->mapHs, &E.mb_dev->soc_fail))) return rc;
        if (pv.ncones > 0 && pd.maxdim <= 64 && E.dblk.nblk > 0) {
            const int nblk = E.dblk.nblk;
            std::vector<i32> blk_cone((size_t)nblk, -1), row_ij(E.h_dblk_node.size(), 0);
            std::vector<char> covered(pd.start.size(), 0);
            size_t nc = 0;
            for (int b = 0, o = 0; b < nblk; o += E.h_dblk_m[(size_t)b], b++) {
                const i32 mb = E.h_dblk_m[(size_t)b];
                const i64 z0 = (i64)E.h_perm[(size_t)E.h_dblk_node[(size_t)o]] - n;
                if (z0 < 0) continue;
                const size_t c = (size_t)(std::upper_bound(pd.start.begin(), pd.start.end(), (i32)z0) - pd.start.begin());
                if (c == 0) continue;
                const i32 st = pd.start[c - 1], nd = pd.dim[c - 1], numel = nd * (nd + 1) / 2;
                if (mb != numel || covered[c - 1]) continue;
                bool ok = true;
                for (i32 a = 0; a < mb && ok; a++) {
                    const i64 t = (i64)E.h_perm[(size_t)E.h_dblk_node[(size_t)(o + a)]] - n - st;
                    if (t < 0 || t >= numel) {
                        ok = false;
                        break;
                    }
                    i32 j = (i32)((std::sqrt(8.0 * (double)t + 1.0) - 1.0) * 0.5);
                    while ((i64)j * (j + 1) / 2 > t) j--;
                    while ((i64)(j + 1) * (j + 2) / 2 <= t) j++;
                    row_ij[(size_t)(o + a)] = (i32)(t - (i64)j * (j + 1) / 2) | (j << 16);
                }
                if (!ok) continue;
                blk_cone[(size_t)b] = (i32)(c - 1);
                covered[c - 1] = 1;
                nc++;
            }
            if (nc == pd.start.size()) {
                h->psd_rows_all_blocks = std::all_of(blk_cone.begin(), blk_cone.end(), [](i32 c) { return c >= 0; });
                int *r1, *r2;
                if ((rc = E.upload(&r1, blk_cone, blk_cone.size()))) return rc;
                if ((rc = E.upload(&r2, row_ij, row_ij.size()))) return rc;
                pv.rows_nblk = nblk;
                pv.blk_cone = r1;
                pv.row_ij = r2;
                pv.blk_m = E.dblk.m;
                pv.blk_rowbase = E.dblk.rowbase;
                pv.blk_start = E.dblk.start;
            }
        }
    }
    {
        dev::Ns3View &nv = h->ns3;
        nv.ncones = (int)n3_start.size();
        int *p1, *p2, *p3;
        double *pa, *pst;
        if ((rc = E.upload(&p1, n3_start, n3_start.size()))) return rc;
        if ((rc = E.upload(&p2, n3_hs, n3_hs.size()))) return rc;
        if ((rc = E.upload(&p3, n3_tag, n3_tag.size()))) return rc;
        if ((rc = E.upload(&pa, n3_alpha, n3_alpha.size()))) return rc;
        if ((rc = E.alloc(&pst, (size_t)(nv.ncones ? nv.ncones : 1) * 18))) return rc;
        CHIP_HIP(hipMemset(pst, 0, (size_t)(nv.ncones ? nv.ncones : 1) * 18 * sizeof(double)));
        nv.start = p1;
        nv.hs_start = p2;
        nv.tag = p3;
        nv.alpha = pa;
        nv.state = pst;
        nv.mapHs = h->mapHs;
    }
    const size_t nsp = K.sp_ptr.size() ? K.sp_ptr.size() - 1 : 0;
    s_ptr = narrow_plain(K.sp_ptr, nsp + 1);
    {
        const auto nu = narrow(K.sp_u, (size_t)(nsp ? K.sp_ptr[nsp] : 0)), nv_ = narrow(K.sp_v, (size_t)(nsp ? K.sp_ptr[nsp] : 0));
        mapU.assign(nu.begin(), nu.end());
        mapV.assign(nv_.begin(), nv_.end());
    }
    for (size_t s = 0; s < nsp; s++) {
        mapD.push_back(k2v[(size_t)K.sp_D[3 * s]]);
        mapD.push_back(k2v[(size_t)K.sp_D[3 * s + 1]]);
    }
    h->nn_count = (int)nn_rows.size();
    h->zero_count = (int)zero_rows.size();
    if ((rc = E.upload(&h->nn_rows, nn_rows, nn_rows.size()))) return rc;
    if ((rc = E.upload(&h->nn_hsidx, nn_hs, nn_hs.size()))) return rc;
    if ((rc = E.upload(&h->zero_rows, zero_rows, zero_rows.size()))) return rc;
    dev::SocView &sv = h->soc;
    sv.ncones = (int)s_start.size();
    int *p_start, *p_dim, *p_hs, *p_sidx, *p_ptr, *p_mu, *p_mv, *p_md;
    if ((rc = E.upload(&p_start, s_start, s_start.size()))) return rc;
    if ((rc = E.upload(&p_dim, s_dim, s_dim.size()))) return rc;
    if ((rc = E.upload(&p_hs, s_hs, s_hs.size()))) return rc;
    if ((rc = E.upload(&p_sidx, s_sidx, s_sidx.size()))) return rc;
    if ((rc = E.upload(&p_ptr, s_ptr, s_ptr.size()))) return rc;
    if ((rc = E.upload(&p_mu, mapU, mapU.size()))) return rc;
    if ((rc = E.upload(&p_mv, mapV, mapV.size()))) return rc;
    if ((rc = E.upload(&p_md, mapD, mapD.size()))) return rc;
    sv.start = p_start;
    sv.dim = p_dim;
    sv.hs_start = p_hs;
    sv.sparse_idx = p_sidx;
    sv.sp_ptr = p_ptr;
    sv.mapHs = h->mapHs;
    sv.mapU = p_mu;
    sv.mapV = p_mv;
    sv.mapD = p_md;
    if ((rc = E.alloc(&h->d_s, (size_t)m))) return rc;
    if ((rc = E.alloc(&h->d_z, (size_t)m))) return rc;
    if ((rc = E.alloc(&h->d_w, (size_t)m))) return rc;
    if ((rc = E.alloc(&h->d_lam, (size_t)m))) return rc;
    CHIP_HIP(hipMemset(h->d_w, 0, (size_t)(m ? m : 1) * sizeof(double)));
    CHIP_HIP(hipMemset(h->d_lam, 0, (size_t)(m ? m : 1) * sizeof(double)));
    sv.w = h->d_w;
    sv.lam = h->d_lam;
    double *st8;
    if ((rc = E.alloc(&st8, (size_t)(sv.ncones ? sv.ncones : 1) * 8))) return rc;
    CHIP_HIP(hipMemset(st8, 0, (size_t)(sv.ncones ? sv.ncones : 1) * 8 * sizeof(double)));
    sv.eta = st8;
    sv.d = st8;
    sv.fail = &E.mb_dev->soc_fail;
    if ((rc = E.alloc(&h->d_rhs, (size_t)(n + m)))) return rc;
    if ((rc = E.alloc(&h->d_lhs, (size_t)(n + m)))) return rc;
    if ((rc = E.alloc(&h->wk[0].bp, (size_t)K.N))) return rc;
    if ((rc = E.alloc(&h->wk[0].x, (size_t)K.N))) return rc;
    if ((rc = E.alloc(&h->wk[0].e, (size_t)K.N))) return rc;
    if ((rc = E.alloc(&h->wk[0].dx, (size_t)K.N))) return rc;
    h->tmp_len = std::max<size_t>({(size_t)K.N, (size_t)K.nHs, nnzP, nnzA, 1});
    if ((rc = E.alloc(&h->d_tmp, h->tmp_len))) return rc;
    CHIP_HIP(hipMemset(h->wk[0].bp, 0, (size_t)(K.N ? K.N : 1) * sizeof(double)));
    if (E.ir_fused) {
        std::vector<int> rp(1, 0), runs;
        const std::vector<i32> &pm = E.h_perm;
        const i64 n1 = K.n, n2 = K.n + K.m;
        auto range_of = [&](i64 o) { return o < n1 ? 0 : (o < n2 ? 1 : 2); };
        for (int b = 0; b < E.bundles.nb; b++) {
            const int s0 = S.bundle_ptr[(size_t)b], s1 = S.bundle_ptr[(size_t)b + 1];
            int t = s0;
            while (t < s1) {
                int e = t + 1;
                while (e < s1 && pm[(size_t)e] == pm[(size_t)e - 1] + 1 && range_of(pm[(size_t)e]) == range_of(pm[(size_t)t])) e++;
                runs.push_back(t - s0);
                runs.push_back(pm[(size_t)t]);
                runs.push_back(e - t);
                t = e;
            }
            rp.push_back((int)(runs.size() / 3));
        }
        if (!runs.empty() && (i64)(runs.size() / 3) * 64 <= (i64)E.NF) {
            if ((rc = E.upload(&h->ir_run_ptr, rp, rp.size()))) return rc;
            if ((rc = E.upload(&h->ir_runs, runs, runs.size()))) return rc;
            bool sf = E.gfold.ng == 0 && E.fold.k >= 1 && E.ir_tw == 256 && E.bundles.symv_split && E.bundles.nb == E.ir_grid &&
                      !switches().no_ir_sf && !switches().no_flat;
            for (int b = 0; b < E.bundles.nb && sf; b++) {
                const int s0 = S.bundle_ptr[(size_t)b], nloc = S.bundle_ptr[(size_t)b + 1] - s0;
                const int nleaf = S.blvl[(size_t)S.blvl_ptr[(size_t)b] + 1] - s0;
                const int nlev = S.blvl_ptr[(size_t)b + 1] - S.blvl_ptr[(size_t)b] - 1;
                sf = dev::irs_bundle_ok(nloc, nleaf, nlev, rp[(size_t)b + 1] - rp[(size_t)b]);
            }
            h->ir_sf = sf && dev::bundle_irs_capacity_ok(E.bundles);
            if (h->ir_sf && !switches().no_shared_pattern && (rc = E.upload_patterns(pat))) return rc;
        }
    }
    clk("maps, cone tables");
    *out = h.release();
    return CHIP_OK;
}

void chip_kkt_destroy(chip_kkt *h) { delete h; }

int32_t chip_kkt_dims(const chip_kkt *h, int64_t out[8]) {
    if (!h) return CHIP_ERR_ARG;
    out[0] = h->K.n;
    out[1] = h->K.m;
    out[2] = h->K.p;
    out[3] = h->K.N;
    out[4] = h->K.nnz;
    out[5] = h->K.nHs;
    out[6] = h->E.NF;
    out[7] = h->E.nnzU;
    return CHIP_OK;
}
int32_t chip_kkt_degree(const chip_kkt *h, int64_t *degree) {
    if (!h || !degree) return CHIP_ERR_ARG;
    i64 d = 0;
    for (const ConeSpec &c : h->K.cones) {
        switch (c.tag) {
        case CHIP_CONE_ZERO: break;
        case CHIP_CONE_NONNEGATIVE: d += c.dim; break;
        case CHIP_CONE_SECONDORDER: d += 1; break;
        case CHIP_CONE_PSDTRIANGLE: d += c.dim; break;
        case CHIP_CONE_EXPONENTIAL:
        case CHIP_CONE_POWER: d += 3; break;
        case CHIP_CONE_GENPOWER: d += c.dim + 1; break;
        default: break;
        }
    }
    *degree = d;
    return CHIP_OK;
}
static int32_t get_supernodes(const Engine &E, int64_t *count, uint64_t *ptr, uint64_t *cols) {
    if (!count) return CHIP_ERR_ARG;
    *count = E.nsn > 0 ? E.nsn : 0;
    if (ptr)
        for (size_t i = 0; i < E.h_sn_ptr.size(); i++) ptr[i] = (uint64_t)E.h_sn_ptr[i];
    if (cols)
        for (size_t i = 0; i < E.h_sn_col.size(); i++) cols[i] = (uint64_t)E.h_sn_col[i];
    return CHIP_OK;
}
int32_t chip_kkt_get_supernodes(const chip_kkt *h, int64_t *count, uint64_t *ptr, uint64_t *cols) {
    return h ? get_supernodes(h->E, count, ptr, cols) : CHIP_ERR_ARG;
}
int32_t chip_ldl_get_supernodes(const chip_ldl *h, int64_t *count, uint64_t *ptr, uint64_t *cols) {
    return h ? get_supernodes(h->E, count, ptr, cols) : CHIP_ERR_ARG;
}
int32_t chip_kkt_get_matrix(const chip_kkt *h, uint64_t *colptr, uint64_t *rowval, double *nzval) {
    if (!h) return CHIP_ERR_ARG;
    const KktLayout &K = h->K;
    if (colptr)
        for (i64 i = 0; i <= K.N; i++) colptr[i] = (uint64_t)K.colptr[i];
    if (rowval)
        for (i64 i = 0; i < K.nnz; i++) rowval[i] = (uint64_t)K.rowval[i];
    if (nzval) std::memcpy(nzval, K.nzval.data(), (size_t)K.nnz * sizeof(double));
    return CHIP_OK;
}
int32_t chip_kkt_get_map(const chip_kkt *h, uint64_t *mapP, uint64_t *mapA, uint64_t *mapHs, uint64_t *diagP,
                         uint64_t *diag_full, int8_t *dsigns) {
    if (!h) return CHIP_ERR_ARG;
    const KktLayout &K = h->K;
    auto cp = [](uint64_t *dst, const auto &src, size_t n) {
        if (dst)
            for (size_t i = 0; i < n; i++) dst[i] = (uint64_t)src[i];
    };
    cp(mapP, K.mapP, K.mapP.size() - 1);
    cp(mapA, K.mapA, K.mapA.size() - 1);
    cp(mapHs, K.mapHs, (size_t)K.nHs);
    cp(diagP, K.diagP, (size_t)K.n);
    cp(diag_full, K.diag_full, (size_t)K.N);
    if (dsigns) std::memcpy(dsigns, K.dsigns.data(), (size_t)K.N);
    return CHIP_OK;
}

int32_t chip_kkt_update_scaling_dev(chip_kkt *h, const double *s_dev, const double *z_dev, double mu,
                                    int32_t strategy) {
    if (!h) return CHIP_ERR_ARG;
    Engine &E = h->E;
    NEED_DEVICE(E);
    CHIP_HIP(hipSetDevice(E.device));
    h->scaling_gen += 1;
    h->soc.fail_gen = h->scaling_gen;
    h->psd.fail_gen = h->scaling_gen;
    dev::sym_update_scaling(E.stream, h->soc, h->nn_rows, h->nn_count, s_dev, z_dev, h->d_w, h->d_lam);
    dev::ns3_update_scaling(E.stream, h->ns3, s_dev, z_dev, mu, strategy);
    dev::gpw_update_scaling(E.stream, h->gpw, z_dev, mu);
    dev::psd_update_scaling(E.stream, h->psd, s_dev, z_dev);
    CHIP_HIP(hipGetLastError());
    h->scaling_pending_check = h->soc.ncones > 0 || h->psd.ncones > 0;
    return 1;
}
int32_t chip_kkt_update_scaling(chip_kkt *h, const double *s, const double *z, double mu, int32_t strategy) {
    if (!h || !s || !z) return CHIP_ERR_ARG;
    Engine &E = h->E;
    NEED_DEVICE(E);
    CHIP_HIP(hipSetDevice(E.device));
    const size_t bytes = (size_t)h->K.m * sizeof(double);
    if (bytes) {
        CHIP_HIP(hipMemcpyAsync(h->d_s, s, bytes, hipMemcpyHostToDevice, E.stream));
        CHIP_HIP(hipMemcpyAsync(h->d_z, z, bytes, hipMemcpyHostToDevice, E.stream));
    }
    int rc = chip_kkt_update_scaling_dev(h, h->d_s, h->d_z, mu, strategy);
    if (rc < 0) return rc;
    if (h->soc.ncones || h->psd.ncones) {
        rc = E.read_mailbox();
        if (rc) return rc;
        h->scaling_pending_check = false;
        return E.mb_host->soc_fail == h->scaling_gen ? 0 : 1;
    }
    CHIP_HIP(hipStreamSynchronize(E.stream));
    return 1;
}

static int update_enqueue(chip_kkt *h, const double *hsblocks_or_null) {
    Engine &E = h->E;
    const KktLayout &K = h->K;
    CHIP_HIP(hipSetDevice(E.device));
    if (h->has_hostHs) {
        if (!hsblocks_or_null)
            return fail(CHIP_ERR_ARG, "update: Hs blocks are required for PSD cones");
        for (const ConeSpec &c : K.cones) {
            if (c.tag <= CHIP_CONE_PSDTRIANGLE) continue;
            CHIP_HIP(hipMemcpyAsync(h->d_tmp + c.block_start, hsblocks_or_null + c.block_start,
                                    (size_t)c.block_len * sizeof(double), hipMemcpyHostToDevice, E.stream));
            dev::scatter_values(E.stream, E.Kx, h->mapHs + c.block_start, h->d_tmp + c.block_start,
                                (int)c.block_len, -1.0);
        }
    }
    const bool slot_eps = !(h->has_hostHs || h->ns3.ncones || h->gpw.ncones || h->psd.ncones);
    unsigned long long *dslots = slot_eps && E.st.static_regularization_enable ? E.diag_slots() : nullptr;
    dev::sym_write_kkt(E.stream, h->soc, h->nn_rows, h->nn_hsidx, h->nn_count, h->d_w, h->mapHs, E.Kx, dslots);
    dev::ns3_write_hs(E.stream, h->ns3, E.Kx);
    dev::gpw_write_kkt(E.stream, h->gpw, E.Kx);
    const bool direct = h->psd_rows_all_blocks && dev::psd_write_hs_rows_active(h->psd) && E.hs_direct_begin();
    dev::psd_write_hs(E.stream, h->psd, E.Kx, direct ? E.Lx : nullptr, direct ? E.dblk_l0 : nullptr);
    return E.refactor_enqueue(h->E.st.static_regularization_enable != 0, slot_eps ? nullptr : h->diag_full,
                              h->static_diag_max);
}
static int update_verdict(chip_kkt *h, int ok) {
    Engine &E = h->E;
    if (ok < 0) return ok;
    h->last_eps = E.st.static_regularization_enable ? E.mb_host->eps : 0.0;
    if (h->scaling_pending_check) {
        h->scaling_pending_check = false;
        if (E.mb_host->soc_fail == h->scaling_gen) return 0;
    }
// ... 296 lines not shown
    CHIP_HIP(hipStreamSynchronize(E.stream));
    E.sx_valid = false;
    h->dirty = true;
    return CHIP_OK;
}
int32_t chip_ldl_scale_values_id(chip_ldl *h, int32_t id, double scale) {
    chip_ldl::IndexSet *st;
    int rc = ldl_set_of(h, id, &st);
    if (rc) return rc;
    Engine &E = h->E;
    NEED_DEVICE(E);
    CHIP_HIP(hipSetDevice(E.device));
    if ((rc = ldl_values_to_device(h))) return rc;
    dev::scale_values(E.stream, E.Kx, st->pos, (int)st->k, scale);
    E.sx_valid = false;
    h->dirty = true;
    return CHIP_OK;
}
int32_t chip_ldl_offset_values_id(chip_ldl *h, int32_t id, double offset) {
    chip_ldl::IndexSet *st;
    int rc = ldl_set_of(h, id, &st);
    if (rc) return rc;
    Engine &E = h->E;
    NEED_DEVICE(E);
    CHIP_HIP(hipSetDevice(E.device));
    if ((rc = ldl_values_to_device(h))) return rc;
    dev::offset_values(E.stream, E.Kx, st->pos, st->signs, (int)st->k, offset);
    E.sx_valid = false;
    h->dirty = true;
    return CHIP_OK;
}
int32_t chip_ldl_pin_buffer(chip_ldl *h, void *ptr, uint64_t bytes) {
    if (!h || !ptr || !bytes) return CHIP_ERR_ARG;
    NEED_DEVICE(h->E);
    CHIP_HIP(hipSetDevice(h->E.device));
    for (void *p : h->pinned)
        if (p == ptr) return CHIP_OK;
    CHIP_HIP(hipHostRegister(ptr, (size_t)bytes, hipHostRegisterDefault));
    h->pinned.push_back(ptr);
    return CHIP_OK;
}
int32_t chip_ldl_solve_refined(chip_ldl *h, double *x, const double *b, const chip_settings *ir_settings, int32_t *iterations) {
    if (!h || !x || !b) return CHIP_ERR_ARG;
    Engine &E = h->E;
    NEED_DEVICE(E);
    if (!E.factored) return fail(CHIP_ERR_NOT_FACTORED, "solve() before the first refactor()");
    CHIP_HIP(hipSetDevice(E.device));
    int rc;
    const size_t N = (size_t)E.N;
    if (!h->r_bp) {
        if ((rc = E.alloc(&h->r_bp, N))) return rc;
        if ((rc = E.alloc(&h->r_x, N))) return rc;
        if ((rc = E.alloc(&h->r_e, N))) return rc;
        if ((rc = E.alloc(&h->r_w, N))) return rc;
    }
    if (h->dirty && !h->dev_values && E.nnzK) {
        if ((rc = E.upload_values(h->hK.data()))) return rc;
        E.sx_valid = false;
        h->dirty = false;
    }
    struct RestoreSettings {
        Engine &E;
        chip_settings saved;
        ~RestoreSettings() { E.st = saved; }
    } restore{E, E.st};
    if (ir_settings) {
        E.st.iterative_refinement_enable = ir_settings->iterative_refinement_enable;
        E.st.iterative_refinement_reltol = ir_settings->iterative_refinement_reltol;
        E.st.iterative_refinement_abstol = ir_settings->iterative_refinement_abstol;
        E.st.iterative_refinement_max_iter = ir_settings->iterative_refinement_max_iter;
        E.st.iterative_refinement_stop_ratio = ir_settings->iterative_refinement_stop_ratio;
    }
    if (N) CHIP_HIP(hipMemcpyAsync(h->d_b, b, N * sizeof(double), hipMemcpyHostToDevice, E.stream));
    SolveCtx &c = E.ctx[0];
    if ((rc = E.zero_norm_sets(c))) return rc;
    dev::permute_in(E.stream, h->r_bp, h->d_b, E.perm, E.N);
    if (N) CHIP_HIP(hipMemcpyAsync(h->r_x, h->r_bp, N * sizeof(double), hipMemcpyDeviceToDevice, E.stream));
    dev::norm_inf(E.stream, h->r_bp, E.N, c.norm_set(0), c.norm_nan(0));
    E.enqueue_solve_inplace(c, h->r_x);
    int its = 0;
    const int ok = refine_core(E, c, h->r_bp, h->r_x, h->r_e, h->r_w, its);
    if (ok == 0) (void)E.sweeps_after_failure();
    if (iterations) *iterations = its;
    if (ok != 1) return ok;
    dev::permute_out(E.stream, h->d_x, h->r_x, E.perm, E.N);
    if (N) CHIP_HIP(hipMemcpyAsync(x, h->d_x, N * sizeof(double), hipMemcpyDeviceToHost, E.stream));
    CHIP_HIP(hipStreamSynchronize(E.stream));
    return 1;
}

static int fused_enqueue(chip_kkt *h, double *lhsx_dev, double *lhsz_dev, int *slot) {
    Engine &E = h->E;
    int rc0;
    if (!E.factored) return fail(CHIP_ERR_NOT_FACTORED, "solve() before the first update()");
    const chip_settings &st = E.st;
    *slot = E.ir_next;
    E.ir_next = (E.ir_next + 1) % Engine::IR_RING;
    dev::IrView ir{};
    ir.rx = h->rhs_x;
    ir.rz = h->rhs_z;
    ir.n = (int)h->K.n;
    ir.m = (int)h->K.m;
    ir.N = E.N;
    ir.perm = E.perm;
    ir.run_ptr = h->ir_run_ptr;
    ir.runs = h->ir_runs;
    ir.bp = h->wk[0].bp;
    ir.xa = h->wk[0].x;
    ir.xb = h->wk[0].e;
    ir.ebuf = h->wk[0].dx;
    ir.lhsx = lhsx_dev;
    ir.lhsz = lhsz_dev;
    ir.part = E.ir_part;
    ir.ctl = E.ir_ctl;
    ir.rel = E.ir_rel;
    ir.epoch = (E.ir_epoch = (E.ir_epoch + 1) & 0x3fffff);
    ir.res = E.ir_res + 4 * *slot;
    ir.abstol = st.iterative_refinement_abstol;
    ir.reltol = st.iterative_refinement_reltol;
    ir.stopratio = st.iterative_refinement_stop_ratio;
    ir.maxiter = st.iterative_refinement_max_iter;
    ir.ir_enable = st.iterative_refinement_enable;
    static long long *dbg_dev = nullptr;
    const bool dbg_on = switches().ir_debug > 0;
    if (dbg_on && !dbg_dev) {
        (void)hipMalloc((void **)&dbg_dev, 256 * sizeof(long long));
    }
    if (dbg_on) (void)hipMemsetAsync(dbg_dev, 0, 256 * sizeof(long long), E.stream);
    ir.dbg = dbg_on ? dbg_dev : nullptr;
    const bool dbg_all_on = switches().ir_debug >= 2;
    static long long *dbg_all_dev = nullptr;
    static size_t dbg_all_len = 0;
    ir.dbg_all = nullptr;
    if (dbg_all_on) {
        const size_t need = (size_t)E.ir_grid * 32;
        if (need > dbg_all_len) {
            if (dbg_all_dev) (void)hipFree(dbg_all_dev);
            (void)hipMalloc((void **)&dbg_all_dev, need * sizeof(long long));
            dbg_all_len = need;
        }
        (void)hipMemsetAsync(dbg_all_dev, 0, need * sizeof(long long), E.stream);
        ir.dbg_all = dbg_all_dev;
    }
    ir.test_drop = h->ir_test_drop ? 1 : 0;
    ir.flat = switches().no_flat ? 0 : 1;
    const bool step_kernel = E.gstep_solve_on && !switches().no_step_kernel && ir.maxiter <= 30;
    ir.sf = (h->ir_sf && !step_kernel) ? 1 : 0;
    if (ir.sf) ir.bp = nullptr;
    {
        auto overlap = [](const double *a, size_t na, const double *b_, size_t nb_) {
            return a && b_ && a < b_ + nb_ && b_ < a + na;
        };
        const size_t n = (size_t)h->K.n, m = (size_t)h->K.m;
        const int flags = switches().irs_flags < 0 ? 3 : switches().irs_flags;
        ir.sf_flags = flags;
        ir.spec_out = (flags & 2) && !(overlap(lhsx_dev, n, ir.rx, n) || overlap(lhsx_dev, n, ir.rz, m) || overlap(lhsz_dev, m, ir.rx, n) ||
                        overlap(lhsz_dev, m, ir.rz, m));
    }
    h->bp_stale = ir.sf != 0;
    if ((rc0 = E.wait_for_exchange())) return rc0;
    h->fused_args[*slot] = {h->rhs_x, h->rhs_z, lhsx_dev, lhsz_dev};
    h->rhs_deferred = false;
    h->x_holds_b = false;
    E.prof_begin(PF_IR);
    int rc;
    if (step_kernel) {
        E.gstep.epoch += 1;
        dev::GStepView gsv = E.gstep;
        if (!E.gstep_vals_valid) gsv.gsl = gsv.gsu = nullptr;
        rc = dev::gstep_solve(E.stream, E.view(), E.bundles, ir, E.gfold, gsv);
    } else if (ir.sf) {
        dev::LdlView lv = E.view();
        ir.pat_off = nullptr;
        if (E.pat_off && !switches().no_shared_pattern) {
            lv.Li16 = E.pat_Li16;
            lv.Lj16 = E.pat_Lj16;
            lv.Ucol16 = E.pat_Ucol16;
            lv.Urow16 = E.pat_Urow16;
            ir.pat_off = E.pat_off;
        }
        rc = dev::bundle_ir(E.stream, lv, E.bundles, E.fold, ir, E.ir_grid, E.ir_tw, E.gfold);
    } else {
        rc = dev::bundle_ir(E.stream, E.view(), E.bundles, E.fold, ir, E.ir_grid, E.ir_tw, E.gfold);
    }
    E.prof_end(PF_IR);
    if (rc) return fail(CHIP_ERR_HIP, hip_err((hipError_t)rc, "fused solve launch"));
    if (dbg_all_on) {
        (void)hipStreamSynchronize(E.stream);
        std::vector<long long> t((size_t)E.ir_grid * 32);
        (void)hipMemcpy(t.data(), dbg_all_dev, t.size() * sizeof(long long), hipMemcpyDeviceToHost);
        const std::string &path = switches().ir_debug_file;
        if (FILE *f = std::fopen(path.empty() ? "/tmp/chip_ir_stamps.bin" : path.c_str(), "wb")) {
            const int g = E.ir_grid;
            std::fwrite(&g, sizeof(int), 1, f);
            std::fwrite(t.data(), sizeof(long long), t.size(), f);
            std::fclose(f);
        }
    } else if (dbg_on) {
        long long t[256];
        (void)hipStreamSynchronize(E.stream);
        (void)hipMemcpy(t, dbg_dev, sizeof(t), hipMemcpyDeviceToHost);
        for (int w = 0; w < 2; w++) {
            std::fprintf(stderr, "k_bundle_ir wg%d phases (us):", w);
            for (int i = 1; i < 64 && t[64 * w + i]; i++) std::fprintf(stderr, " %.1f", (t[64 * w + i] - t[64 * w + i - 1]) * 0.01);
            std::fprintf(stderr, "\n");
        }
    }
    return CHIP_OK;
}
constexpr int FUSED_TIMEOUT = -1000;
static int fused_verdict(chip_kkt *h, int slot) {
    Engine &E = h->E;
    const int *r = E.ir_res_host + 4 * slot;
    if (r[2] || r[0] == 0) {
        (void)hipMemsetAsync(E.ir_ctl, 0, E.ir_ctl_len * sizeof(int), E.stream);
        return FUSED_TIMEOUT;
    }
    h->wk[0].last_ir = r[1];
    return r[0] > 0 ? 1 : 0;
}
static int fused_retry_unfused(chip_kkt *h, int slot) {
    Engine &E = h->E;
    const chip_kkt::FusedArgs &a = h->fused_args[slot];
    h->fused_fallbacks += 1;
    h->rhs_x = a.rx;
    h->rhs_z = a.rz;
    h->rhs_deferred = true;
    h->x_holds_b = true;
    const int ok = solve_core(h, 0);
    if (ok != 1) return ok;
    dev::getlhs_perm(E.stream, a.lx, a.lz, h->wk[0].x, E.iperm, (int)h->K.n, (int)h->K.m);
    CHIP_HIP(hipGetLastError());
    CHIP_HIP(hipStreamSynchronize(E.stream));
    return 1;
}
static int fused_read_ring(chip_kkt *h) { return h->E.read_mailbox(); }

int32_t chip_kkt_solve_dev(chip_kkt *h, double *lhsx_dev, double *lhsz_dev) {
    if (!h) return CHIP_ERR_ARG;
    Engine &E = h->E;
    NEED_DEVICE(E);
    CHIP_HIP(hipSetDevice(E.device));
    if (h->bp_stale && !h->rhs_deferred) {
        h->rhs_deferred = true;
        h->x_holds_b = true;
    }
    if (E.ir_fused && h->rhs_deferred && (E.prof_family == PF_NONE || E.prof_family >= PF_IR)) {
        int slot = 0;
        int rc = fused_enqueue(h, lhsx_dev, lhsz_dev, &slot);
        if (rc) return rc;
        if ((rc = fused_read_ring(h))) return rc;
        rc = fused_verdict(h, slot);
        return rc == FUSED_TIMEOUT ? fused_retry_unfused(h, slot) : rc;
    }
    int ok = solve_core(h, 0);
    if (ok != 1) return ok;
    dev::getlhs_perm(E.stream, lhsx_dev, lhsz_dev, h->wk[0].x, E.iperm, (int)h->K.n, (int)h->K.m);
    CHIP_HIP(hipGetLastError());
    return 1;
}
int32_t chip_kkt_solve_dev_enqueue(chip_kkt *h, double *lhsx_dev, double *lhsz_dev) {
    if (!h) return CHIP_ERR_ARG;
    Engine &E = h->E;
    NEED_DEVICE(E);
    CHIP_HIP(hipSetDevice(E.device));
    if ((int)h->pend_slots.size() >= Engine::IR_RING) return fail(CHIP_ERR_ARG, "solve_dev_enqueue: 16 solves pending, collect first");
    if (h->bp_stale && !h->rhs_deferred) {
        h->rhs_deferred = true;
        h->x_holds_b = true;
    }
    if (E.ir_fused && h->rhs_deferred && (E.prof_family == PF_NONE || E.prof_family >= PF_IR)) {
        int slot = 0;
        int rc = fused_enqueue(h, lhsx_dev, lhsz_dev, &slot);
        if (rc) return rc;
        h->pend_slots.push_back(slot);
        return CHIP_OK;
    }
    if (h->pend_update) {
        h->pend_update = 2;
        h->pend_update_ok = update_verdict(h, E.refactor_collect());
        if (h->pend_update_ok != 1) {
            h->pend_slots.push_back(-1 - 0);
            return CHIP_OK;
        }
    }
    const int ok = chip_kkt_solve_dev(h, lhsx_dev, lhsz_dev);
    if (ok < 0) return ok;
    h->pend_slots.push_back(-1 - ok);
    return CHIP_OK;
}
int32_t chip_kkt_solve2_dev_enqueue(chip_kkt *h, const double *rhsx_a, const double *rhsz_a, double *lhsx_a, double *lhsz_a,
                                    const double *rhsx_b, const double *rhsz_b, double *lhsx_b, double *lhsz_b) {
    if (!h) return CHIP_ERR_ARG;
    Engine &E = h->E;
    NEED_DEVICE(E);
    CHIP_HIP(hipSetDevice(E.device));
    if ((int)h->pend_slots.size() + 2 > Engine::IR_RING) return fail(CHIP_ERR_ARG, "solve2_dev_enqueue: 16 solves pending, collect first");
    int rc;
    if (E.ir_fused || !E.pair_ok() || switches().no_solve_pair || E.prof_family != PF_NONE) {
        if ((rc = chip_kkt_setrhs_dev(h, rhsx_a, rhsz_a))) return rc;
        if ((rc = chip_kkt_solve_dev_enqueue(h, lhsx_a, lhsz_a))) return rc;
        if ((rc = chip_kkt_setrhs_dev(h, rhsx_b, rhsz_b))) return rc;
        return chip_kkt_solve_dev_enqueue(h, lhsx_b, lhsz_b);
    }
    if (h->pend_update) {
        h->pend_update = 2;
        h->pend_update_ok = update_verdict(h, E.refactor_collect());
        if (h->pend_update_ok != 1) {
            h->pend_slots.push_back(-1);
            h->pend_slots.push_back(-1);
            return CHIP_OK;
        }
    }
    if (!E.factored) return fail(CHIP_ERR_NOT_FACTORED, "solve() before the first update()");
    const size_t N = (size_t)E.N;
    chip_kkt::SolveVecs &wb = h->wk[1];
    if (!wb.bp) {
        if ((rc = E.alloc(&wb.bp, N))) return rc;
        if ((rc = E.alloc(&wb.x, N))) return rc;
        if ((rc = E.alloc(&wb.e, N))) return rc;
        if ((rc = E.alloc(&wb.dx, N))) return rc;
    }
    if ((rc = E.pair_begin())) return rc;
    const int n = (int)h->K.n, m = (int)h->K.m;
    h->rhs_deferred = false;
    h->x_holds_b = false;
    h->bp_stale = false;
    const double *const rhsx[2] = {rhsx_a, rhsx_b}, *const rhsz[2] = {rhsz_a, rhsz_b};
    double *const lhsx[2] = {lhsx_a, lhsx_b}, *const lhsz[2] = {lhsz_a, lhsz_b};
    const bool lockstep = E.pair_lockstep_ok();
    for (int k = 0; k < 2; k++) {
        chip_kkt::SolveVecs &w = h->wk[k];
// ... 356 lines not shown
    *beta_out = b;
    return CHIP_OK;
}
int32_t chip_kkt_info(const chip_kkt *h, chip_info *info) {
    if (!h || !info) return CHIP_ERR_ARG;
    fill_info(h->E, info);
    info->threads = h->world;
    info->last_ir_iterations = h->wk[0].last_ir;
    info->last_regularizer = h->last_eps;
    if (h->E.factored && !h->E.host_only) {
        i64 c = 0;
        int rc = count_positive(const_cast<Engine &>(h->E), &c);
        if (rc) return rc;
        info->positive_inertia = c;
    }
    return CHIP_OK;
}
int32_t chip_kkt_get_perm(const chip_kkt *h, uint64_t *perm) {
    if (!h || !perm) return CHIP_ERR_ARG;
    for (int i = 0; i < h->E.N; i++) perm[i] = (uint64_t)h->E.h_perm[i];
    return CHIP_OK;
}
int32_t chip_kkt_get_symbolic(const chip_kkt *h, uint64_t *etree, uint64_t *Lp, uint64_t *Li,
                              uint64_t *lvlptr) {
    if (!h) return CHIP_ERR_ARG;
    return h->E.get_symbolic(etree, Lp, Li, lvlptr);
}
int32_t chip_kkt_get_values(chip_kkt *h, double *nzval) {
    if (!h || !nzval) return CHIP_ERR_ARG;
    Engine &E = h->E;
    NEED_DEVICE(E);
    CHIP_HIP(hipSetDevice(E.device));
    return E.download_values(nzval);
}
int32_t chip_kkt_synchronize(chip_kkt *h) {
    if (!h) return CHIP_ERR_ARG;
    NEED_DEVICE(h->E);
    CHIP_HIP(hipStreamSynchronize(h->E.stream));
    return CHIP_OK;
}
void *chip_kkt_stream(chip_kkt *h) { return (h && !h->E.host_only) ? (void *)h->E.stream : nullptr; }
int32_t chip_kkt_profile(chip_kkt *h, int32_t family) {
    if (!h) return CHIP_ERR_ARG;
    h->E.prof_collect();
    h->E.prof_family = family;
    h->E.prof_ms_total = 0;
    h->E.prof_launches = 0;
    return CHIP_OK;
}
int32_t chip_kkt_profile_read(chip_kkt *h, double out[8]) {
    if (!h) return CHIP_ERR_ARG;
    h->E.prof_collect();
    std::memset(out, 0, 8 * sizeof(double));
    out[0] = (double)h->E.prof_launches;
    out[1] = h->E.prof_ms_total;
    out[2] = (double)h->E.prof_family;
    return CHIP_OK;
}
int32_t chip_kkt_step_kernels(const chip_kkt *h) {
    if (!h) return CHIP_ERR_ARG;
    const bool on = !switches().no_step_kernel;
    return (on && h->E.gstep_solve_on ? 1 : 0) | (on && h->E.gstep_factor_on ? 2 : 0) | (h->ir_sf && !(on && h->E.gstep_solve_on) ? 4 : 0);
}
int32_t chip_kkt_fused_fallbacks(const chip_kkt *h) { return h ? h->fused_fallbacks : CHIP_ERR_ARG; }
int32_t chip_kkt_work_model(const chip_kkt *h, double out[8]) {
    if (!h || !out) return CHIP_ERR_ARG;
    std::memcpy(out, h->E.sn_model, 8 * sizeof(double));
    out[5] = h->E.gfold.ng;
    out[6] = h->E.bundles.nb;
    out[7] = h->E.ir_fused ? h->E.ir_tw : 0;
    return CHIP_OK;
}
int32_t chip_kkt_sweep_model(const chip_kkt *h, double out[4]) {
    if (!h || !out) return CHIP_ERR_ARG;
    const Engine &E = h->E;
    int gl = 0, sl = 0;
    for (char f : E.sn_lvl_g) gl += f != 0;
    for (size_t l = 0; l + 1 < E.sn_lvl_ptr.size(); l++) sl += E.sn_lvl_ptr[l + 1] > E.sn_lvl_ptr[l];
    out[0] = E.sn_g_ntasks > 0 ? E.sn_g_entries : 0.0;
    out[1] = E.sn_g_ntasks > 0 ? gl : 0;
    out[2] = sl;
    out[3] = E.sn_g_ntasks > 0 ? 1 : 0;
    return CHIP_OK;
}
#ifdef CHIP_TESTING
int32_t chip_debug_spin(int32_t device, int32_t blocks, int32_t threads, int32_t lds_bytes, double usec) {
    static hipStream_t spin_stream[16] = {};
    if (device < 0 || device >= 16 || blocks < 0 || threads <= 0 || threads > 1024 || lds_bytes < 0 || lds_bytes > 160 * 1024)
        return CHIP_ERR_ARG;
    int prev = -1;
    (void)hipGetDevice(&prev);
    struct Restore {
        int d;
        ~Restore() {
            if (d >= 0) (void)hipSetDevice(d);
        }
    } restore{prev};
    CHIP_HIP(hipSetDevice(device));
    if (blocks == 0) {
        if (spin_stream[device]) CHIP_HIP(hipStreamSynchronize(spin_stream[device]));
        return CHIP_OK;
    }
    if (!spin_stream[device]) CHIP_HIP(hipStreamCreateWithFlags(&spin_stream[device], hipStreamNonBlocking));
    dev::debug_spin(spin_stream[device], blocks, threads, lds_bytes, usec);
    CHIP_HIP(hipGetLastError());
    return CHIP_OK;
}
int32_t chip_debug_set_switch(const char *name, const char *value_or_null) {
    return switches_set(name, value_or_null) ? CHIP_OK : fail(CHIP_ERR_ARG, "chip_debug_set_switch: unknown switch");
}
int32_t chip_debug_counter(const void *kkt_handle, const char *name, double *out) {
    const chip_kkt *h = (const chip_kkt *)kkt_handle;
    if (!h || !name || !out) return CHIP_ERR_ARG;
    const std::string k(name);
    const Engine &E = h->E;
    if (k == "dense_blocks") *out = E.dblk.nblk;
    else if (k == "dense_block_rows") *out = E.dblk.nrows;
    else if (k == "nnzS") *out = (double)E.nnzS;
    else if (k == "psd_hs_row_blocks") *out = h->psd.rows_nblk;
    else if (k == "assembled_levels") {
        int c = 0;
        for (size_t l = 0; l + 1 < E.asm_lvl_ptr.size(); l++) c += E.asm_lvl_ptr[l + 1] > E.asm_lvl_ptr[l];
        *out = c;
    } else if (k == "assembled_targets") *out = E.asm_lvl_ptr.empty() ? 0 : E.asm_lvl_ptr.back();
    else if (k == "g_levels") {
        int c = 0;
        for (char f : E.sn_lvl_g) c += f != 0;
        *out = E.sn_g_ntasks > 0 ? c : 0;
    } else if (k == "sn_levels") {
        int c = 0;
        for (size_t l = 0; l + 1 < E.sn_lvl_ptr.size(); l++) c += E.sn_lvl_ptr[l + 1] > E.sn_lvl_ptr[l];
        *out = c;
    } else if (k == "g_entries") *out = E.sn_g_entries;
    else if (k == "gsweep_runs") *out = (double)E.gs_runs.size();
    else if (k == "gsweep_launches") *out = E.gs_launches;
    else if (k == "gsweep_recoveries") *out = E.gs_recoveries;
    else if (k == "tri2_launches") *out = E.tri2_launches;
    else if (k == "dblk2_launches") *out = (double)E.dblk2_launches;
    else if (k == "dblk_blocks") *out = E.dblk.nblk;
    else if (k == "hs_direct_refactors") *out = (double)E.hs_direct_refactors;
    else if (k == "gsweep_levels") {
        int c = 0;
        for (const auto &r : E.gs_runs) c += r.nlev;
        *out = c;
    }
    else if (k == "pattern_classes") *out = E.pat_classes;
    else if (k == "pattern_index_bytes") *out = (double)E.pat_index_bytes;
    else if (k == "pattern_bundles") *out = E.pat_bundles;
    else if (k == "pattern_full_index_bytes") *out = (double)E.pat_full_bytes;
    else if (k == "pattern_verified_bundles") *out = E.pat_verified;
    else if (k == "pattern_mismatches") *out = E.pat_mismatches;
    else if (k == "pattern_shared_bundles")
        *out = (h->ir_sf && E.pat_off && !switches().no_shared_pattern) ? E.bundles.nb : 0;
    else return fail(CHIP_ERR_ARG, "chip_debug_counter: unknown name");
    return CHIP_OK;
}
int32_t chip_debug_psd_create(void **out, int64_t ncones, const int64_t *dims) {
    if (!out) return fail(CHIP_ERR_ARG, "chip_debug_psd_create: bad argument");
    *out = nullptr;
    if (ncones < 1 || !dims) return fail(CHIP_ERR_ARG, "chip_debug_psd_create: bad argument");
    std::vector<i32> tags((size_t)ncones, CHIP_CONE_PSDTRIANGLE);
    std::vector<ConeSpec> specs;
    i64 m = 0, p = 0, nHs = 0;
    if (build_cone_specs(ncones, tags.data(), dims, nullptr, specs, m, p, nHs))
        return fail(CHIP_ERR_ARG, "chip_debug_psd_create: cones refused");
    for (const ConeSpec &c : specs)
        if (c.dim < 0 || c.dim > 1024) return fail(CHIP_ERR_ARG, "chip_debug_psd_create: side out of range (0 .. 1024)");
    std::unique_ptr<DebugPsd> h(new DebugPsd());
    for (const ConeSpec &c : specs) h->sz.add(c.start, c.dim, c.block_start);
    h->m = m;
    *out = h.release();
    return CHIP_OK;
}
void chip_debug_psd_destroy(void *h) { delete (DebugPsd *)h; }
int32_t chip_debug_psd_counter(const void *handle, const char *name, double *out) {
    const DebugPsd *h = (const DebugPsd *)handle;
    if (!h || !name || !out) return fail(CHIP_ERR_ARG, "chip_debug_psd_counter: bad argument");
    const std::string k(name);
    if (k == "gs") *out = h->sz.scratch_stride ? 1 : 0;
    else if (k == "jacobi_lds") *out = h->last_jacobi_lds;
    else if (k == "maxdim") *out = h->sz.maxdim;
    else if (k == "rows") *out = (double)h->m;
    else if (k == "scratch_stride") *out = (double)h->sz.scratch_stride;
    else if (k == "state_doubles") *out = (double)h->sz.state;
    else return fail(CHIP_ERR_ARG, "chip_debug_psd_counter: unknown name");
    return CHIP_OK;
}
int32_t chip_debug_psd_update_scaling(void *handle, const double *s, const double *z, int32_t *ok) {
    DebugPsd *h = (DebugPsd *)handle;
    if (!h || !s || !z || !ok) return fail(CHIP_ERR_ARG, "chip_debug_psd_update_scaling: bad argument");
    int rc;
    if ((rc = h->ready())) return rc;
    DebugPsdStage st;
    const double *ds, *dz;
    if ((rc = st.in(s, (size_t)h->m, &ds)) || (rc = st.in(z, (size_t)h->m, &dz))) return rc;
    h->pv.fail_gen = ++h->gen;
    dev::psd_update_scaling(h->stream, h->pv, ds, dz);
    h->last_jacobi_lds = dev::psd_last_jacobi_lds();
    if ((rc = st.finish(h->stream))) return rc;
    int flag = 0;
    CHIP_HIP(hipMemcpy(&flag, h->fail_flag, sizeof(int), hipMemcpyDeviceToHost));
    *ok = flag == h->gen ? 0 : 1;
    return CHIP_OK;
}
int32_t chip_debug_psd_state(void *handle, int64_t cone, double *out) {
    DebugPsd *h = (DebugPsd *)handle;
    if (!h || !out || cone < 0 || cone >= (int64_t)h->sz.dim.size())
        return fail(CHIP_ERR_ARG, "chip_debug_psd_state: bad argument");
    int rc;
    if ((rc = h->ready())) return rc;
    const size_t n = (size_t)h->sz.dim[(size_t)cone];
    CHIP_HIP(hipStreamSynchronize(h->stream));
    CHIP_HIP(hipMemcpy(out, h->pv.state + h->sz.off[(size_t)cone], (3 * n * n + 2 * n) * sizeof(double),
                       hipMemcpyDeviceToHost));
    return CHIP_OK;
}
int32_t chip_debug_psd_mul_hs(void *handle, double *y, const double *x) {
    DebugPsd *h = (DebugPsd *)handle;
    if (!h || !y || !x) return fail(CHIP_ERR_ARG, "chip_debug_psd_mul_hs: bad argument");
    int rc;
    if ((rc = h->ready())) return rc;
    DebugPsdStage st;
    double *dy;
    const double *dx;
    if ((rc = st.out(y, (size_t)h->m, &dy)) || (rc = st.in(x, (size_t)h->m, &dx))) return rc;
    dev::psd_mul_hs(h->stream, h->pv, dy, dx);
    return st.finish(h->stream);
}
int32_t chip_debug_psd_affine_ds(void *handle, double *ds) {
    DebugPsd *h = (DebugPsd *)handle;
    if (!h || !ds) return fail(CHIP_ERR_ARG, "chip_debug_psd_affine_ds: bad argument");
    int rc;
    if ((rc = h->ready())) return rc;
    DebugPsdStage st;
    double *dds;
    if ((rc = st.out(ds, (size_t)h->m, &dds))) return rc;
    dev::psd_affine_ds(h->stream, h->pv, dds);
    return st.finish(h->stream);
}
int32_t chip_debug_psd_combined_ds_shift(void *handle, double *shift, double *step_z, double *step_s, double sigma_mu) {
    DebugPsd *h = (DebugPsd *)handle;
    if (!h || !shift || !step_z || !step_s || step_z == step_s || shift == step_z || shift == step_s)
        return fail(CHIP_ERR_ARG, "chip_debug_psd_combined_ds_shift: bad argument");
    int rc;
    if ((rc = h->ready())) return rc;
    DebugPsdStage st;
    double *d0, *d1, *d2;
    if ((rc = st.out(shift, (size_t)h->m, &d0)) || (rc = st.out(step_z, (size_t)h->m, &d1)) ||
        (rc = st.out(step_s, (size_t)h->m, &d2)))
        return rc;
    dev::psd_combined_ds_shift(h->stream, h->pv, d0, d1, d2, sigma_mu);
    return st.finish(h->stream);
}
int32_t chip_debug_psd_ds_from_dz_offset(void *handle, double *out, const double *ds) {
    DebugPsd *h = (DebugPsd *)handle;
    if (!h || !out || !ds) return fail(CHIP_ERR_ARG, "chip_debug_psd_ds_from_dz_offset: bad argument");
    int rc;
    if ((rc = h->ready())) return rc;
    DebugPsdStage st;
    double *d0;
    const double *d1;
    if ((rc = st.out(out, (size_t)h->m, &d0)) || (rc = st.in(ds, (size_t)h->m, &d1))) return rc;
    dev::psd_ds_from_dz_offset(h->stream, h->pv, d0, d1);
    return st.finish(h->stream);
}
int32_t chip_debug_psd_step_length(void *handle, const double *dz, const double *ds, double amax, double *partial) {
    DebugPsd *h = (DebugPsd *)handle;
    if (!h || !dz || !ds || !partial) return fail(CHIP_ERR_ARG, "chip_debug_psd_step_length: bad argument");
    int rc;
    if ((rc = h->ready())) return rc;
    DebugPsdStage st;
    const double *d0, *d1;
    double *dp;
    if ((rc = st.in(dz, (size_t)h->m, &d0)) || (rc = st.in(ds, (size_t)h->m, &d1)) ||
        (rc = st.out(partial, h->sz.dim.size(), &dp)))
        return rc;
    (void)dev::psd_step_length(h->stream, h->pv, d0, d1, amax, dp);
    h->last_jacobi_lds = dev::psd_last_jacobi_lds();
    return st.finish(h->stream);
}
int32_t chip_debug_psd_margins(void *handle, const double *z, double *pmin, double *psum) {
    DebugPsd *h = (DebugPsd *)handle;
    if (!h || !z || !pmin || !psum) return fail(CHIP_ERR_ARG, "chip_debug_psd_margins: bad argument");
    int rc;
    if ((rc = h->ready())) return rc;
    DebugPsdStage st;
    const double *d0;
    double *dmin, *dsum;
    if ((rc = st.in(z, (size_t)h->m, &d0)) || (rc = st.out(pmin, h->sz.dim.size(), &dmin)) ||
        (rc = st.out(psum, h->sz.dim.size(), &dsum)))
        return rc;
    (void)dev::psd_margins(h->stream, h->pv, d0, dmin, dsum);
    h->last_jacobi_lds = dev::psd_last_jacobi_lds();
    return st.finish(h->stream);
}
int32_t chip_debug_psd_barrier(void *handle, const double *z, const double *s, const double *dz, const double *ds,
                               double alpha, double *partial) {
    DebugPsd *h = (DebugPsd *)handle;
    if (!h || !z || !s || !dz || !ds || !partial) return fail(CHIP_ERR_ARG, "chip_debug_psd_barrier: bad argument");
    int rc;
    if ((rc = h->ready())) return rc;
    DebugPsdStage st;
    const double *d0, *d1, *d2, *d3;
    double *dp;
    const size_t m = (size_t)h->m;
    if ((rc = st.in(z, m, &d0)) || (rc = st.in(s, m, &d1)) || (rc = st.in(dz, m, &d2)) || (rc = st.in(ds, m, &d3)) ||
        (rc = st.out(partial, h->sz.dim.size(), &dp)))
// ... 8 lines not shown
```

### clarabel.rs_amd/csrc/grid_sync.hpp

```cpp
#pragma once
#include "dev_common.hpp"

namespace chip {
namespace dev {

namespace {

constexpr int IR_NSUB = 32;
constexpr int IR_CTL_INTS = 32 * (1 + 2 * IR_NSUB);

enum { IR_TIMEOUT = 0, IR_WAITED = 1, IR_LAST = 2 };
__device__ __forceinline__ int ir_arrive_wait(int *ctl, int gen, int nwg) {
    __shared__ int s_state;
    __syncthreads();
    if (threadIdx.x == 0) {
        __builtin_amdgcn_fence(__ATOMIC_RELEASE, "workgroup");
        __builtin_amdgcn_s_waitcnt(0);
        const int sub = blockIdx.x % IR_NSUB;
        const int members = nwg / IR_NSUB + (sub < nwg % IR_NSUB ? 1 : 0);
        int state = IR_WAITED;
        if (atomicAdd(ctl + 32 * (1 + sub), 1) + 1 == members * gen) {
            if (atomicAdd(ctl, 1) + 1 == min(IR_NSUB, nwg) * gen) state = IR_LAST;
        }
        if (state != IR_LAST) {
            const int *rel = ctl + 32 * (1 + IR_NSUB + sub);
            long long spins = 0;
            while (__hip_atomic_load(rel, __ATOMIC_RELAXED, __HIP_MEMORY_SCOPE_AGENT) < gen) {
                __builtin_amdgcn_s_sleep(8);
                if (++spins > (1ll << 21)) {
                    state = IR_TIMEOUT;
                    break;
                }
            }
        }
        s_state = state;
    }
    __syncthreads();
    return s_state;
}
__device__ __forceinline__ void ir_release(int *ctl, int gen, int nwg) {
    __syncthreads();
    if (threadIdx.x == 0) {
        __builtin_amdgcn_fence(__ATOMIC_RELEASE, "workgroup");
        __builtin_amdgcn_s_waitcnt(0);
        for (int q = 0; q < min(IR_NSUB, nwg); ++q)
            __hip_atomic_store(ctl + 32 * (1 + IR_NSUB + q), gen, __ATOMIC_RELAXED, __HIP_MEMORY_SCOPE_AGENT);
    }
}
__device__ __forceinline__ void ir_grid_exit(int *ctl, int gen, int nwg) {
    if (threadIdx.x != 0) return;
    const int sub = blockIdx.x % IR_NSUB;
    const int members = nwg / IR_NSUB + (sub < nwg % IR_NSUB ? 1 : 0);
    if (atomicAdd(ctl + 32 * (1 + sub), 1) + 1 == members * gen) {
        if (atomicAdd(ctl, 1) + 1 == min(IR_NSUB, nwg) * gen) {
            for (int q = 0; q < IR_NSUB; ++q) {
                __hip_atomic_store(ctl + 32 * (1 + q), 0, __ATOMIC_RELAXED, __HIP_MEMORY_SCOPE_AGENT);
                __hip_atomic_store(ctl + 32 * (1 + IR_NSUB + q), 0, __ATOMIC_RELAXED, __HIP_MEMORY_SCOPE_AGENT);
            }
            __hip_atomic_store(ctl, 0, __ATOMIC_RELAXED, __HIP_MEMORY_SCOPE_AGENT);
        }
    }
}
__device__ __forceinline__ int ir_arrive_nowait(int *ctl, int gen, int nwg) {
    __shared__ int s_state2;
    __syncthreads();
    if (threadIdx.x == 0) {
        __builtin_amdgcn_fence(__ATOMIC_RELEASE, "workgroup");
        __builtin_amdgcn_s_waitcnt(0);
        const int sub = blockIdx.x % IR_NSUB;
        const int members = nwg / IR_NSUB + (sub < nwg % IR_NSUB ? 1 : 0);
        int state = IR_WAITED;
        if (atomicAdd(ctl + 32 * (1 + sub), 1) + 1 == members * gen) {
            if (atomicAdd(ctl, 1) + 1 == min(IR_NSUB, nwg) * gen) state = IR_LAST;
        }
        s_state2 = state;
    }
    __syncthreads();
    return s_state2;
}
__device__ __forceinline__ int ir_wait_word(const int *word, int gen) {
    __shared__ int s_state3;
    __syncthreads();
    if (threadIdx.x == 0) {
        int state = IR_WAITED;
        long long spins = 0;
        while (__hip_atomic_load(word, __ATOMIC_RELAXED, __HIP_MEMORY_SCOPE_AGENT) < gen) {
            __builtin_amdgcn_s_sleep(2);
            if (++spins > (1ll << 22)) {
                state = IR_TIMEOUT;
                break;
            }
        }
        s_state3 = state;
    }
    __syncthreads();
    return s_state3;
}
__device__ __forceinline__ bool ir_group_arrive(int *cnt, int expect) {
    __shared__ int s_glast;
    __syncthreads();
    if (threadIdx.x == 0) {
        __builtin_amdgcn_fence(__ATOMIC_RELEASE, "workgroup");
        __builtin_amdgcn_s_waitcnt(0);
        s_glast = (atomicAdd(cnt, 1) + 1 == expect) ? 1 : 0;
    }
    __syncthreads();
    return s_glast != 0;
}
__device__ __forceinline__ double ir_load(const double *p) {
    return __hip_atomic_load(p, __ATOMIC_RELAXED, __HIP_MEMORY_SCOPE_AGENT);
}
__device__ __forceinline__ void ir_store(double *p, double val) {
    __hip_atomic_store(p, val, __ATOMIC_RELAXED, __HIP_MEMORY_SCOPE_AGENT);
}

__device__ __forceinline__ double block_nanmax(double v, double *red) {
#pragma unroll
    for (int o = 32; o > 0; o >>= 1) v = nanmax(v, __shfl_down(v, o, 64));
    const int lane = threadIdx.x & 63, wv = threadIdx.x >> 6;
    __syncthreads();
    if (lane == 0) red[wv] = v;
    __syncthreads();
    double t = red[0];
    for (int i = 1; i < (int)(blockDim.x >> 6); ++i) t = nanmax(t, red[i]);
    return t;
}

__device__ __forceinline__ double lds_block_nanmax(double m, bool bad, double *red) {
    m = wave_max_all(m);
    const bool wbad = __ballot(bad) != 0ull;
    const int lane = threadIdx.x & 63, wv = threadIdx.x >> 6;
    lds_barrier();
    if (lane == 0) red[wv] = wbad ? __longlong_as_double(0x7ff8000000000000ll) : m;
    lds_barrier();
    double t = red[0];
    for (int i = 1; i < (int)(blockDim.x >> 6); ++i) t = nanmax(t, red[i]);
    return t;
}

typedef int msg_v4i __attribute__((ext_vector_type(4)));
__device__ __forceinline__ void msg_store(int *slot, double val, int tag) {
    msg_v4i m;
    m.x = __double2loint(val);
    m.y = tag;
    m.z = __double2hiint(val);
    m.w = tag;
    asm volatile("global_store_dwordx4 %0, %1, off sc1\n\ts_nop 3" ::"v"(slot), "v"(m) : "memory");
}
__device__ __forceinline__ msg_v4i msg_load(const int *slot) {
    msg_v4i m;
    asm volatile("global_load_dwordx4 %0, %1, off sc1\n\ts_waitcnt vmcnt(0)" : "=&v"(m) : "v"(slot) : "memory");
    return m;
}

__device__ __forceinline__ void msg_load2(const int *slot_a, const int *slot_b, msg_v4i &a, msg_v4i &b) {
    asm volatile("global_load_dwordx4 %0, %2, off sc1\n\tglobal_load_dwordx4 %1, %3, off sc1\n\ts_waitcnt vmcnt(0)"
                 : "=&v"(a), "=&v"(b)
                 : "v"(slot_a), "v"(slot_b)
                 : "memory");
}
__device__ __forceinline__ void msg_load3(const int *slot_a, const int *slot_b, const int *slot_c, msg_v4i &a, msg_v4i &b,
                                          msg_v4i &c) {
    asm volatile("global_load_dwordx4 %0, %3, off sc1\n\tglobal_load_dwordx4 %1, %4, off sc1\n\tglobal_load_dwordx4 %2, %5, off sc1\n\t"
                 "s_waitcnt vmcnt(0)"
                 : "=&v"(a), "=&v"(b), "=&v"(c)
                 : "v"(slot_a), "v"(slot_b), "v"(slot_c)
                 : "memory");
}
__device__ __forceinline__ bool msg_ready(const msg_v4i &m, int tag) { return m.y == tag && m.w == tag; }
__device__ __forceinline__ double msg_value(const msg_v4i &m) { return __hiloint2double(m.z, m.x); }

constexpr int IR_REC_MSGS = 32;
constexpr int IR_REL_INTS = IR_NSUB * IR_REC_MSGS * 4;
__device__ __forceinline__ void ir_publish(int *rel, const double *vals, int nmsg, int tag, int nwg) {
    const int nsub = min(IR_NSUB, nwg);
    for (int t = threadIdx.x; t < nsub * nmsg; t += blockDim.x) {
        const int sgrp = t / nmsg, j = t - sgrp * nmsg;
        msg_store(rel + (sgrp * IR_REC_MSGS + j) * 4, vals[j], tag);
    }
}
__device__ __forceinline__ int ir_wait_record(const int *rel, double *vals, int nmsg, int tag) {
    __shared__ int s_state4;
    if (threadIdx.x < 64) {
        const int lane = threadIdx.x;
        const int *slot = rel + ((int)(blockIdx.x % IR_NSUB) * IR_REC_MSGS + (lane < nmsg ? lane : 0)) * 4;
        int state = IR_WAITED;
        long long spins = 0;
        msg_v4i m;
        for (;;) {
            m = msg_load(slot);
            if (__all(msg_ready(m, tag) ? 1 : 0)) break;
            __builtin_amdgcn_s_sleep(4);
            if (++spins > (1ll << 21)) {
                state = IR_TIMEOUT;
                break;
            }
        }
        if (state != IR_TIMEOUT && lane < nmsg) vals[lane] = msg_value(m);
        if (lane == 0) s_state4 = state;
    }
    __syncthreads();
    return s_state4;
}

}

}
}
```

### clarabel.rs_amd/csrc/kernels.hpp

```cpp
#pragma once
#include <hip/hip_runtime.h>

#include <cstdint>

namespace chip {
namespace dev {

struct LdlView {
    int N;
    int nnzL;
    const int *Lp, *Li;
    const int *Rp, *Rcol, *Rpos;
    const int *Tpos;
    double *Lx, *Rx;
    double *D, *Dinv;
    const int8_t *dsigns;
    int *status;
    double reg_eps, reg_delta;
    const int *Up, *Ucol;
    const double *Ux;
    const double *eps_ptr;
    const unsigned long long *eps_slots;
    unsigned long long *eps_clear;
    double eps_c, eps_prop, eps_static_max;
    double *eps_out;
    const unsigned short *Li16, *Ucol16;
    const unsigned short *Lj16, *Urow16;
    const unsigned short *Rk16, *Ro16;
    const unsigned short *fu_rec, *fu_slot;
    const int *fu_ptr;
    int mirror_rows;
    const unsigned short *sLi16, *sLj16;
};

struct BundleView {
    int nb;
    const int *bundle_ptr, *blvl_ptr, *blvl;
    int max_nodes;
    int max_entries;
    int ir_lds_doubles, symv_split;
    int max_levels;
    long long *fdbg;
};

struct FoldView {
    int k, NF;
    const int *rseg;
    const int *tt;
    const int *sp, *scol, *sslot;
    double *acc;
    const double *top_k;
    int *cnt;
    int top_sign;
};
struct GFoldView {
    int ng;
    const int *ptr, *node;
    const int *bptr;
    const int *bgrp;
    const int *tt;
    const int *sp, *scol, *sslot;
    double *fsh;
    double *rsh;
    double *rec;
    int *gcnt;
    double *fac;
};
constexpr int FOLD_SLOTS = 16, FOLD_STRIDE = 16;
inline __host__ __device__ int fold_acc_index(int kind, int row, int slot) {
    return ((kind * 8 + row) * FOLD_SLOTS + slot) * FOLD_STRIDE;
}
struct TopBlkView {
    int nblocks, w, NF, N;
    const int *Rsplit, *Lsplit;
    double *T;
    double *ys;
    int *counters;
};
struct ListView {
    const int *idx;
    int count;
};
struct ChunkView {
    const int *row, *beg, *end;
    int count;
};

void scatter_init(hipStream_t s, const double *Kx, const int *a2l, int nnzK, int nnzL, double *Lx,
                  double *D, const int8_t *dsigns, const double *eps_or_null, const int *fill_idx,
                  int nfill, int *status);
void eps_from_slots(hipStream_t s, unsigned long long *slots, double c, double prop, double static_max,
                    double *scal);
void scatter_rest(hipStream_t s, const double *Kx, const int *a2l, const int *rest, int nrest, int nnzL, double *Lx, double *D,
                  const int8_t *dsigns, const double *eps, int *status);
void gather_values(hipStream_t s, double *Sx, const double *Kx, const int *Smap, int nnzS);
struct DblkView {
    int nblk = 0, split = 1, mmax = 0, nrows = 0;
    const int *p0 = nullptr, *m = nullptr, *rowbase = nullptr;
    const int *start = nullptr;
    const int *rownode = nullptr;
    double *P = nullptr;
};
int dblk_attributes(int mmax);
void dblk_symv(hipStream_t s, const DblkView &d, const double *Kx, const double *x, double *bt);
void dblk_symv2(hipStream_t s, const DblkView &d, const double *Kx, const double *x0, const double *x1, double *P1, double *bt0);
void dblk_finish(hipStream_t s, const DblkView &d, double *bt);
void diag_absmax_eps(hipStream_t s, const double *Kx, const int *diag_idx, int N, double c,
                     double prop, double *scal );
void scatter_values(hipStream_t s, double *Kx, const int *map, const double *vals, int k, double scale);
void offset_values(hipStream_t s, double *Kx, const int *map, const int8_t *signs, int k, double offset);
void scale_values(hipStream_t s, double *Kx, const int *map, int k, double scale);

int bundle_factor(hipStream_t s, const LdlView &v, const BundleView &bv, const FoldView &fold, int lds_doubles = 0);
bool bundle_factor_lds_ok(int lds_doubles);
void fold_top_pivot(hipStream_t s, const LdlView &v, const FoldView &fold);
void bundle_fwd(hipStream_t s, const LdlView &v, const BundleView &bv, double *x, const FoldView &fold);
void fold_top_solve(hipStream_t s, const LdlView &v, const FoldView &fold, double *x);
void fold_top_residual(hipStream_t s, const FoldView &fold, const double *Sx, const double *x, const double *b,
                       double *e, unsigned long long *nrm, int *nan);
void bundle_bwd(hipStream_t s, const LdlView &v, const BundleView &bv, double *x, const double *addv);
void bundle_symv(hipStream_t s, const BundleView &bv, const int *Up, const int *Ucol, const double *Ux,
                 const double *x, const double *b, double *e, unsigned long long *nrm, int *nan, const FoldView &fold, hipEvent_t ev0 = nullptr, hipEvent_t ev1 = nullptr);
struct IrView {
    const double *rx, *rz;
    int n, m, N;
    const int *perm;
    const int *run_ptr, *runs;
    double *bp;
    double *xa, *xb;
    union {
        double *ebuf;
        const int *pat_off;
    };
    double *lhsx, *lhsz;
    double *part;
    int *ctl;
    int *res;
    double abstol, reltol, stopratio;
    int maxiter, ir_enable;
    long long *dbg;
    long long *dbg_all;
    int test_drop;
    int flat;
    int *rel;
    int epoch;
    int sf_flags;
    int spec_out;
    int sf;
};
int ir_rel_ints();
int ir_ctl_ints();
size_t ir_part_doubles(int nb, int k);
int bundle_ir_capacity(const BundleView &bv, int *tw);
int bundle_ir(hipStream_t s, const LdlView &v, const BundleView &bv, const FoldView &fold, const IrView &ir, int grid,
              int tw, const GFoldView &gf);
bool bundle_irs_capacity_ok(const BundleView &bv);
bool irs_bundle_ok(int nloc, int nleaf, int nlevels, int nruns);
void gfold_top_factor(hipStream_t s, const LdlView &v, const BundleView &bv, const GFoldView &gf);

constexpr int GS_MAXL = 14;
constexpr int GS_LST = GS_MAXL + 2;
constexpr int GS_DESC = 64;
constexpr int GS_GTOP = 152;
constexpr int GS_MV = 12;
struct GStepView {
    int lr, ur, nr;
    const int *desc;
    const int *gtop;
    const unsigned short *lsrc;
    const unsigned int *lij;
    const unsigned short *usrc;
    const unsigned int *uij;
    const unsigned short *ufs;
    double *gsl, *gsu;
    int *msg;
    int *lmsg;
    int *fmsg;
    int epoch;
    long long *dbg;
};
int gstep_solve_capacity(const BundleView &bv, const GStepView &gs);
int gstep_solve(hipStream_t s, const LdlView &v, const BundleView &bv, const IrView &ir, const GFoldView &gf,
                const GStepView &gs);
bool gstep_factor_ok(const BundleView &bv);
int gstep_factor(hipStream_t s, const LdlView &v, const BundleView &bv, const GFoldView &gf, const GStepView &gs);

void factor_T(hipStream_t s, const LdlView &v, ListView cols);
void factor_W(hipStream_t s, const LdlView &v, ListView cols);
void factor_B(hipStream_t s, const LdlView &v, ChunkView chunks);
struct SnodeView {
    const int *sn_ptr, *sn_col;
    const long long *upd_ptr;
    const int *upd_slot;
    const int *sn_geo;
    const int *sn_cb;
    double *sn_d;
    const int8_t *sn_sg;
    long long *dbg;
    int *sn_cnt;
    double *U = nullptr, *Ud = nullptr;
    const long long *asm_uoff = nullptr;
    const int *asm_doff = nullptr;
    double *Gx = nullptr;
    const long long *g_off = nullptr;
};
struct SnodeAsmView {
    const int *tgt, *src_ptr;
    const long long *src;
    int t0 = 0, nt = 0;
};
int snode_kernel_attributes(int wmax, int nbmax);

enum { PFK_SN_UPDATE = 7, PFK_SN_DIAG = 8, PFK_SN_ROWS = 9, PFK_SN_EXTEND = 10, PFK_SN_TRI = 11 };
struct LaunchProf {
    void (*begin)(void *ctx, int family);
    void (*end)(void *ctx, int family);
    void *ctx;
};
void factor_snodes(hipStream_t s, const LdlView &v, const SnodeView &sv, const int *order, int count, int wmax_all,
                   int nblk, int hmax, int nbmax, const LaunchProf *lp = nullptr, const SnodeAsmView *av = nullptr);
void factor_finalize(hipStream_t s, const LdlView &v, ListView cols);

enum GatherMode { FWD = 0, BWD = 1, SYMV = 2, SPMV = 3 };
struct GatherArgs {
    const int *ptr, *idx;
    const double *val;
    const double *xin;
    double *out;
    const double *aux;
    unsigned long long *nrm;
    int *nan;
    double alpha;
};
constexpr int NRM_SLOTS = 64;
constexpr int NRM_STRIDE = 16;
void gather_Bprep(hipStream_t s, GatherMode m, const GatherArgs &a, ListView rows);
void solve_kernel_attributes();
void topblk_build(hipStream_t s, const LdlView &v, const TopBlkView &tb);
void topblk_solve(hipStream_t s, GatherMode m, const LdlView &v, const TopBlkView &tb, double *x);
void factor_chain(hipStream_t s, const LdlView &v, const int *t_idx, const int *t_ptr, const int *w_idx,
                  const int *w_ptr, int l0, int l1);
void gather_chain(hipStream_t s, GatherMode m, const GatherArgs &a, const int *t_idx, const int *t_ptr,
                  const int *w_idx, const int *w_ptr, int l0, int l1);
void gather_merged(hipStream_t s, GatherMode m, const GatherArgs &a, ListView t, ListView w, ChunkView c);
struct SnodeTriView {
    const int *blk_ptr;
    int *msg;
    int epoch;
    int *timeout_flag;
};
void solve_snodes(hipStream_t s, GatherMode m, const LdlView &v, const SnodeView &sv, const int *order, int count,
                  int wmax_all, int nbmax_all, int wlvl, int nblvl, double *x, const SnodeTriView *tri = nullptr,
                  const LaunchProf *lp = nullptr, double *x2 = nullptr, const SnodeTriView *tri2 = nullptr);
bool solve_snodes_is_tri(const SnodeTriView *tri, int wlvl);
int snode_g_max_width();
long long snode_g_ld(int h);
int snode_g_attributes(int hmax);
void snode_ginv(hipStream_t s, const LdlView &v, const SnodeView &sv, const int *order_all, const int *tasks, int ntasks);
void solve_snodes_g(hipStream_t s, GatherMode m, const LdlView &v, const SnodeView &sv, const int *order, int count, int wlvl,
                    int hlvl, double *x, double *yt, const LaunchProf *lp = nullptr, const GatherArgs *ga = nullptr,
                    ListView t = ListView{nullptr, 0}, ListView w = ListView{nullptr, 0}, ChunkView c = ChunkView{nullptr, nullptr, nullptr, 0});
struct GSweepLevel {
    int off, count;
    int gx;
    int tcount, wcount, ccount;
    int pad0, pad1;
    const int *trows, *wrows, *crow, *cbeg, *cend;
};
int snode_gsweep_capacity(GatherMode m, size_t lds);
size_t snode_gsweep_lds(GatherMode m, int hmax);
void solve_snodes_gsweep(hipStream_t s, GatherMode m, const LdlView &v, const SnodeView &sv, const int *order_all, double *x,
                         double *yt, const GSweepLevel *lv, int nlev, int grid, size_t lds, const GatherArgs &ga, int *ctl,
                         int *fail, const LaunchProf *lp = nullptr);
void debug_spin(hipStream_t s, int blocks, int threads, int lds_bytes, double usec);
void norm_rows(hipStream_t s, const double *v, ListView rows, unsigned long long *nrm, int *nan);

void permute_in(hipStream_t s, double *y, const double *b, const int *perm, int N);
void permute_out(hipStream_t s, double *x, const double *y, const int *perm, int N);
void setrhs_perm(hipStream_t s, double *bperm, double *xinit, const double *rhsx, const double *rhsz,
                 const int *perm, int n, int m, int N, unsigned long long *nrm, int *nan);
void getlhs_perm(hipStream_t s, double *lhsx, double *lhsz, const double *xperm, const int *iperm,
                 int n, int m);
void add_vec(hipStream_t s, double *dx, const double *x, int N);
void waxpby(hipStream_t s, double *w, double a, const double *x, double b, const double *y, int n);
int dot_scratch_doubles();
// ... 126 lines not shown
```

### include/clarabel_hip_testing.h

```cpp
#ifndef CLARABEL_HIP_TESTING_H
#define CLARABEL_HIP_TESTING_H
#include <stdint.h>
#ifdef __cplusplus
extern "C" {
#endif
int32_t chip_debug_spin(int32_t device, int32_t blocks, int32_t threads, int32_t lds_bytes, double usec);
int32_t chip_debug_set_switch(const char *name, const char *value_or_null);
int32_t chip_debug_counter(const void *kkt_handle, const char *name, double *out);
int32_t chip_comm_debug_spin(void *comm, int32_t blocks, int32_t threads, double usec);
int32_t chip_debug_transform_create(void **out, int64_t n, int64_t m, const uint64_t *Pcolptr, const uint64_t *Prowval,
                                    const double *Pnzval, const double *q, const uint64_t *Acolptr,
                                    const uint64_t *Arowval, const double *Anzval, const double *b, int64_t ncones,
                                    const int32_t *cone_tags, const int64_t *cone_dims, const int64_t *cone_dims2,
                                    const double *cone_alphas_or_null, const void *solver_settings);
void chip_debug_transform_destroy(void *h);
int32_t chip_debug_transform_get(const void *h, const char *name, int64_t *len, void *out);
int32_t chip_debug_transform_reverse(const void *h, const double *x2, const double *s2, const double *z2, double *x,
                                     double *s, double *z);
int32_t chip_debug_solver_internal_solution(void *solver, double *x2, double *s2, double *z2);
int32_t chip_debug_ipm_termination(const void *solver_settings, const double *info, int32_t iter, int32_t iterations,
                                   double solve_time, int32_t almost_post_process);
int32_t chip_debug_ipm_info_update(double *info, const double *sq, double tau, double kappa, double c, double normq,
                                   double normb);
int32_t chip_debug_batch_inject_nan(void *batch, int64_t member, int32_t iteration);
int32_t chip_debug_batch_counter(void *batch, const char *name, double *out);
int32_t chip_debug_bplan_create(void **out, int64_t nprob, const int64_t *n_part, const int64_t *m_part, int64_t ncones,
                                const int32_t *cone_tags, const int64_t *cone_dims);
void chip_debug_bplan_destroy(void *h);
int32_t chip_debug_bplan_get(const void *h, const char *name, int64_t *len, int32_t *out);
int32_t chip_debug_bplan_seg_reduce(void *h, int32_t count, const int32_t *kind, const int32_t *space,
                                    const int32_t *slot, const double *const *a, const double *const *b,
                                    int32_t nslots, double *out);
int32_t chip_debug_bplan_cone_minima(void *h, int32_t op, const double *dz, const double *ds, const double *z,
                                     const double *sv, const double *amax, double *out_min, double *out_sum_or_null);
int32_t chip_debug_bplan_blin(void *h, double *w, const double *x, const double *y, const double *sa, const double *sb,
                              double ca, double cb, int32_t space, const int32_t *mask, int32_t mask_mode);
int32_t chip_debug_bplan_bresid(void *h, double *rx, const double *rx_inf, const double *Px, const double *q,
                                double *rz, const double *rz_inf, const double *b, const double *tau);
int32_t chip_debug_bplan_bunit_shift(void *h, double *z, const double *alpha, int32_t primal, const int32_t *mask);
int32_t chip_debug_bplan_bunit_reset(void *h, double *x, double *sv, double *z, const int32_t *flag);
int32_t chip_debug_bplan_bunscale(void *h, double *xo, const double *x, const double *d, double *zo, const double *z,
                                  const double *e, double *so, const double *sv, const double *einv, const double *sx,
                                  const double *sz);
int32_t chip_debug_psd_create(void **out, int64_t ncones, const int64_t *dims);
void chip_debug_psd_destroy(void *h);
int32_t chip_debug_psd_counter(const void *h, const char *name, double *out);
int32_t chip_debug_psd_update_scaling(void *h, const double *s, const double *z, int32_t *ok);
int32_t chip_debug_psd_state(void *h, int64_t cone, double *out);
int32_t chip_debug_psd_mul_hs(void *h, double *y, const double *x);
int32_t chip_debug_psd_affine_ds(void *h, double *ds);
int32_t chip_debug_psd_combined_ds_shift(void *h, double *shift, double *step_z, double *step_s, double sigma_mu);
int32_t chip_debug_psd_ds_from_dz_offset(void *h, double *out, const double *ds);
int32_t chip_debug_psd_step_length(void *h, const double *dz, const double *ds, double amax, double *partial);
int32_t chip_debug_psd_margins(void *h, const double *z, double *pmin, double *psum);
int32_t chip_debug_psd_barrier(void *h, const double *z, const double *s, const double *dz, const double *ds,
                               double alpha, double *partial);
#ifdef __cplusplus
}
#endif
#endif
```

Baseline: 1703.

## Prefetch next sweep's first batch and per-bundle descriptors in fused IR kernel

Adds a precomputed per-bundle descriptor (offsets, level table, permutation runs) that each workgroup loads as one dword per lane, replacing several scattered index lookups at kernel start. The forward and backward triangular sweeps now start from a first batch of L entries, plus Dinv values for the backward sweep, that were issued early: during the grid barrier wait or at the end of the preceding symv. The diagonal scaling is applied from registers before the backward sweep. The aim is to hide global-memory latency at sweep boundaries, at the cost of extra register pressure and a more complex control path.

Result: faster. 1775 (median of 6 runs) (+4.2%).

```diff
diff --git a/clarabel.rs_amd/__init__.py b/clarabel.rs_amd/__init__.py
--- a/clarabel.rs_amd/__init__.py
+++ b/clarabel.rs_amd/__init__.py
@@ -1647,6 +1647,16 @@
     return out.value
 
 
+def debug_kkt_ints(kkt, name):
+    n = C.c_int64(0)
+    f = lib().chip_debug_kkt_ints
+    f.argtypes = [C.c_void_p, C.c_char_p, C.POINTER(C.c_int64), C.c_void_p]
+    _check(f(kkt._h, name.encode(), C.byref(n), None), "debug_kkt_ints")
+    out = np.zeros(n.value, dtype=np.int32)
+    _check(f(kkt._h, name.encode(), C.byref(n), out.ctypes.data_as(C.c_void_p)), "debug_kkt_ints")
+    return out
+
+
 def set_device(ordinal):
     rc = _hiprt().hipSetDevice(C.c_int(int(ordinal)))
     if rc != 0:
diff --git a/clarabel.rs_amd/csrc/bundle_ir.hip b/clarabel.rs_amd/csrc/bundle_ir.hip
--- a/clarabel.rs_amd/csrc/bundle_ir.hip
+++ b/clarabel.rs_amd/csrc/bundle_ir.hip
@@ -273,6 +273,121 @@
         }
     };
     if (step < nl) request(base, ee, ci, cj, cv);
+    while (step < nl) {
+        int nstep = step, nbase = base + TW * FLAT_U, nee = ee;
+        if (nbase >= nee) {
+            nstep = step + 1;
+            while (nstep < nl) {
+                level_range(nstep, nbase, nee);
+                if (nbase < nee) break;
+                ++nstep;
+            }
+        }
+        if (nstep < nl) request(nbase, nee, ni, nj, nv);
+#pragma unroll
+        for (int u = 0; u < FLAT_U; ++u) {
+            const int i = ci[u];
+            if (i < 0) continue;
+            if (FWDMODE) {
+                const double val = cv[u] * xs[cj[u]];
+                if (i < nloc) atomicAdd(&xs[i], -val);
+                else if (k == 1) tpart += val;
+                else atomicAdd(&tacc[i - nloc], val);
+            } else {
+                atomicAdd(&xs[cj[u]], -(cv[u] * (i < nloc ? xs[i] : xt[i - nloc])));
+            }
+        }
+        if (nstep != step) lds_barrier();
+        step = nstep;
+        base = nbase;
+        ee = nee;
+#pragma unroll
+        for (int u = 0; u < FLAT_U; ++u) {
+            ci[u] = ni[u];
+            cj[u] = nj[u];
+            cv[u] = nv[u];
+        }
+    }
+    if (FWDMODE && k == 1) {
+        tpart = wave_sum_all(tpart);
+        if (lane == 0 && tpart != 0.0) atomicAdd(&tacc[0], tpart);
+    }
+    lds_barrier();
+}
+
+struct FlatBatch {
+    int i[FLAT_U], j[FLAT_U];
+    double v[FLAT_U];
+};
+__device__ __forceinline__ void flat_batch_clear(FlatBatch &fb) {
+#pragma unroll
+    for (int u = 0; u < FLAT_U; ++u) fb.i[u] = -1, fb.j[u] = 0, fb.v[u] = 0.0;
+}
+template <bool FWDMODE, int TW>
+__device__ __forceinline__ void flat_request_first(const LdlView &v, const int *lev_e, int nl, int dl, int tid, FlatBatch &fb) {
+    int step = 0, base = 0, ee = 0;
+    while (step < nl) {
+        const int l = FWDMODE ? step : nl - 1 - step;
+        base = lev_e[l];
+        ee = lev_e[l + 1];
+        if (base < ee) break;
+        ++step;
+    }
+    if (step < nl) {
+#pragma unroll
+        for (int u = 0; u < FLAT_U; ++u) {
+            const int t = base + u * TW + tid;
+            const bool ok = t < ee;
+            const int tc = ok ? t : ee - 1;
+            const int ri = (int)v.Li16[tc + dl], rj = (int)v.Lj16[tc + dl];
+            const double rv = v.Lx[tc];
+            fb.i[u] = ok ? ri : -1;
+            fb.j[u] = ok ? rj : 0;
+            fb.v[u] = ok ? rv : 0.0;
+        }
+    } else {
+        flat_batch_clear(fb);
+    }
+}
+template <bool FWDMODE, int TW>
+__device__ __forceinline__ void bundle_sweep_flat_ahead(const LdlView &v, double *xs, const double *xt, double *tacc, int k,
+                                                        const int *lev_e, int dl, int nloc, int nl, const FlatBatch &first) {
+    static_assert(TW == 256, "two batches in flight: the 256-thread form only");
+    int tid = threadIdx.x;
+    asm volatile("" : "+v"(tid));
+    const int lane = tid & 63;
+    if (FWDMODE && tid < 8) tacc[tid] = 0.0;
+    double tpart = 0.0;
+    int step = 0, base = 0, ee = 0;
+    auto level_range = [&](int st_, int &eb_, int &ee_) {
+        const int l = FWDMODE ? st_ : nl - 1 - st_;
+        eb_ = lev_e[l];
+        ee_ = lev_e[l + 1];
+    };
+    lds_barrier();
+    while (step < nl) {
+        level_range(step, base, ee);
+        if (base < ee) break;
+        ++step;
+    }
+    int ci[FLAT_U], cj[FLAT_U], ni[FLAT_U], nj[FLAT_U];
+    double cv[FLAT_U], nv[FLAT_U];
+    auto request = [&](int bs, int en, int *ii, int *jj, double *vv) {
+#pragma unroll
+        for (int u = 0; u < FLAT_U; ++u) {
+            const int t = bs + u * TW + tid;
+            const bool ok = t < en;
+            ii[u] = ok ? (int)v.Li16[t + dl] : -1;
+            jj[u] = ok ? (int)v.Lj16[t + dl] : 0;
+            vv[u] = ok ? v.Lx[t] : 0.0;
+        }
+    };
+#pragma unroll
+    for (int u = 0; u < FLAT_U; ++u) {
+        ci[u] = first.i[u];
+        cj[u] = first.j[u];
+        cv[u] = first.v[u];
+    }
     while (step < nl) {
         int nstep = step, nbase = base + TW * FLAT_U, nee = ee;
         if (nbase >= nee) {
@@ -986,7 +1101,8 @@
 __device__ __forceinline__ void irs_symv(const LdlView &v, const IrView &ir, const int *runs, const double (&c)[NPT],
                                          bool keep_e, double *xs, double *red, double *tacc3, int k, int s0,
                                          int nloc, int nleaf, const double *xt, double *out_norm, double *out_share,
-                                         int du) {
+                                         int du, bool have_fl, int fl_b, int fl_e, bool next_fwd,
+                                         const int *lev_e, int nl, int dl, FlatBatch &nextb) {
     double cl[NLP];
     const int *__restrict__ Up = v.Up;
     const unsigned short *__restrict__ Ucol16 = v.Ucol16, *__restrict__ Urow16 = v.Urow16;
@@ -1003,7 +1119,7 @@
         tb[u] = i < nleaf ? Up[s0 + i] : 0;
         te[u] = i < nleaf ? Up[s0 + i + 1] : 0;
     }
-    const int fb = Up[s0 + nleaf], fe = Up[s0 + nloc];
+    const int fb = have_fl ? fl_b : Up[s0 + nleaf], fe = have_fl ? fl_e : Up[s0 + nloc];
     {
         RunWalk rw{runs, 0};
         double bq[NPT];
@@ -1081,8 +1197,8 @@
         }
     }
     {
-        int ii[FLAT_U], jj[FLAT_U], ni[FLAT_U], nj[FLAT_U];
-        double vv[FLAT_U], nv[FLAT_U];
+        int fi[FLAT_U], fj[FLAT_U], ni[FLAT_U], nj[FLAT_U];
+        double fv[FLAT_U], nv[FLAT_U];
         auto request = [&](int bs, int *pi, int *pj, double *pv) {
 #pragma unroll
             for (int u = 0; u < FLAT_U; ++u) {
@@ -1093,7 +1209,7 @@
                 pv[u] = ok ? Ux[t] : 0.0;
             }
         };
-        if (fb < fe) request(fb, ii, jj, vv);
+        if (fb < fe) request(fb, fi, fj, fv);
         for (int base = fb; base < fe; base += TW * FLAT_U) {
             if (base + TW * FLAT_U < fe) request(base + TW * FLAT_U, ni, nj, nv);
             else {
@@ -1102,28 +1218,29 @@
             }
 #pragma unroll
             for (int u = 0; u < FLAT_U; ++u) {
-                const int i = ii[u], j = jj[u];
+                const int i = fi[u], j = fj[u];
                 if (i < 0) continue;
                 const double xi = xs[xpos(i - nleaf)];
                 if (j >= nloc) {
-                    atomicAdd(&xs[i], -(vv[u] * xt[j - nloc]));
-                    if (k == 1) tpart += vv[u] * xi;
-                    else atomicAdd(&tacc3[j - nloc], vv[u] * xi);
+                    atomicAdd(&xs[i], -(fv[u] * xt[j - nloc]));
+                    if (k == 1) tpart += fv[u] * xi;
+                    else atomicAdd(&tacc3[j - nloc], fv[u] * xi);
                 } else if (j == i) {
-                    atomicAdd(&xs[i], -(vv[u] * xi));
+                    atomicAdd(&xs[i], -(fv[u] * xi));
                 } else {
-                    atomicAdd(&xs[i], -(vv[u] * xs[xpos(j - nleaf)]));
-                    atomicAdd(&xs[j], -(vv[u] * xi));
+                    atomicAdd(&xs[i], -(fv[u] * xs[xpos(j - nleaf)]));
+                    atomicAdd(&xs[j], -(fv[u] * xi));
                 }
             }
 #pragma unroll
             for (int u = 0; u < FLAT_U; ++u) {
-                ii[u] = ni[u];
-                jj[u] = nj[u];
-                vv[u] = nv[u];
-            }
-        }
-    }
+                fi[u] = ni[u];
+                fj[u] = nj[u];
+                fv[u] = nv[u];
+            }
+        }
+    }
+    if (next_fwd) flat_request_first<true, TW>(v, lev_e, nl, dl, tid, nextb);
     lds_barrier();
     double m = mleaf;
 #pragma unroll
@@ -1167,13 +1284,31 @@
     __shared__ double tacc3[8];
     __shared__ IrState st;
     __shared__ int pat[2];
-    const int nb = bv.nb, G = gridDim.x, tid = threadIdx.x, b = blockIdx.x;
+    __shared__ int hdr[12];
+    const int nb = bv.nb, G = gridDim.x, b = blockIdx.x;
+    int tid = threadIdx.x;
     const int k = fold.k;
     const bool folded = k > 0;
     const int NF = k ? fold.NF : ir.N;
     if (ir.test_drop && b == G - 1 && G > 1) return;
-    const int s0 = bv.bundle_ptr[b], nloc = bv.bundle_ptr[b + 1] - s0;
-    const int nleaf = bv.blvl[bv.blvl_ptr[b] + 1] - s0;
+    const bool use_desc = (ir.sf_flags & IRS_F_DESC) != 0;
+    const bool ahead = (ir.sf_flags & IRS_F_CHAINED) == 0;
+    static_assert(IRS_DESC_RUNS == IR_MAXRUNS && IRS_DESC_LEVELS + 1 <= FLAT_MAXLEV + 1 && TW >= IRS_DESC_INTS, "IrsDesc");
+    if (use_desc && tid < IRS_DESC_INTS) {
+        constexpr int LEV0 = offsetof(IrsDesc, lev_e) / sizeof(int), RUN0 = offsetof(IrsDesc, runs) / sizeof(int);
+        static_assert(LEV0 == 12 && offsetof(IrsDesc, dl) == 16, "IrsDesc: head of 12 ints");
+        const int w = ((const int *)(ir.desc + b))[tid];
+        if (tid < LEV0) hdr[tid] = w;
+        else if (tid < RUN0) lev_e[tid - LEV0] = w;
+        else st.runs[tid - RUN0] = w;
+        if (tid == 4 || tid == 5) pat[tid - 4] = w;
+    }
+    int s0 = 0, nloc = 0, nleaf = 0, nl = 0;
+    if (!use_desc) {
+        s0 = bv.bundle_ptr[b], nloc = bv.bundle_ptr[b + 1] - s0;
+        nleaf = bv.blvl[bv.blvl_ptr[b] + 1] - s0;
+        nl = bv.blvl_ptr[b + 1] - bv.blvl_ptr[b] - 1;
+    }
     double *pnb = ir.part;
     double *pn = pnb + nb;
     double *shf = pn + 2 * nb;
@@ -1189,8 +1324,10 @@
         st.par = 0;
         st.gen = 0;
         st.pad = 0;
-        pat[0] = ir.pat_off ? ir.pat_off[2 * b] : 0;
-        pat[1] = ir.pat_off ? ir.pat_off[2 * b + 1] : 0;
+        if (!use_desc) {
+            pat[0] = ir.pat_off ? ir.pat_off[2 * b] : 0;
+            pat[1] = ir.pat_off ? ir.pat_off[2 * b + 1] : 0;
+        }
         if (b == 0) {
             ir.res[0] = 0;
             ir.res[2] = 0;
@@ -1200,12 +1337,21 @@
         st.ltt[tid] = 0.0;
         st.ktt[tid] = 0.0;
     }
-    {
+    if (!use_desc) {
         const int r0 = ir.run_ptr[b], nruns = ir.run_ptr[b + 1] - r0;
         if (tid < 3 * nruns) st.runs[tid] = ir.runs[3 * r0 + tid];
-    }
-    flat_level_table(v, bv, b, lev_e);
+        flat_level_table(v, bv, b, lev_e);
+    }
     __syncthreads();
+    int fl_b = 0, fl_e = 0;
+    if (use_desc) {
+        s0 = __builtin_amdgcn_readfirstlane(hdr[0]);
+        nloc = __builtin_amdgcn_readfirstlane(hdr[1]);
+        nleaf = __builtin_amdgcn_readfirstlane(hdr[2]);
+        nl = __builtin_amdgcn_readfirstlane(hdr[3]);
+        fl_b = __builtin_amdgcn_readfirstlane(hdr[6]);
+        fl_e = __builtin_amdgcn_readfirstlane(hdr[7]);
+    }
     auto load_top_constants = [&]() {
         if (tid < 8) {
             st.btop[tid] = tid < k ? rhs_of(ir.perm[NF + tid]) : 0.0;
@@ -1237,9 +1383,34 @@
     __shared__ double redm[4 * 16];
     const int nmsg = 2 * k + 2;
     const int tagbase = ir.epoch << 8;
-    auto barrier = [&](bool fwd, bool resid, int rpar, bool first) -> int {
+    double dinv[NPT];
+    FlatBatch fwdb, bwdb;
+    bool dinv_have = false, bwd_have = false, fwd_have = false;
+    flat_batch_clear(fwdb);
+    flat_batch_clear(bwdb);
+#pragma unroll
+    for (int u = 0; u < NPT; ++u) dinv[u] = 0.0;
+    auto request_dinv = [&]() {
+        const int t_ = opaque_tid();
+#pragma unroll
+        for (int u = 0; u < NPT; ++u) {
+            const int i = t_ + u * TW;
+            dinv[u] = v.Dinv[s0 + (i < nloc ? i : nloc - 1)];
+        }
+    };
+    auto barrier = [&](bool fwd, bool resid, int rpar, bool first, bool issue_bwd) -> int {
         if (tid == 0) st.gen += 1;
-        const int state = ir_arrive_nowait(ir.ctl, st.gen, G);
+        auto issue = [&]() {
+            if (ahead) request_dinv();
+            if (ahead) flat_request_first<false, TW>(v, lev_e, nl, __builtin_amdgcn_readfirstlane(pat[0]), opaque_tid(), bwdb);
+        };
+        int state;
+        if (issue_bwd) {
+            state = ir_arrive_nowait_issue(ir.ctl, st.gen, G, issue);
+            dinv_have = bwd_have = ahead;
+        } else {
+            state = ir_arrive_nowait(ir.ctl, st.gen, G);
+        }
         const int tag = tagbase | (__builtin_amdgcn_readfirstlane(st.gen) & 0xff);
         if (state == IR_LAST) {
             double f0 = 0.0, r0 = 0.0, mb = 0.0, m = 0.0;
@@ -1358,6 +1529,10 @@
             const int i = tid + u * TW;
             c[u] = i < nloc ? rhs_of(rw.orig(i)) : 0.0;
         }
+        if (ahead) {
+            flat_request_first<true, TW>(v, lev_e, nl, __builtin_amdgcn_readfirstlane(pat[0]), opaque_tid(), fwdb);
+            fwd_have = true;
+        }
         double mx = 0.0;
         bool nan = false;
 #pragma unroll
@@ -1380,15 +1555,22 @@
     bool spec_done = false;
     for (int round = 0;; ++round) {
         const int par = round & 1;
+        asm volatile("" : "+v"(tid));
         __syncthreads();
         stamp();
-        bundle_sweep_flat<true, TW>(v, bv, b, xs, nullptr, st.tacc, k, lev_e, __builtin_amdgcn_readfirstlane(pat[0]));
+        {
+            const int dl = __builtin_amdgcn_readfirstlane(pat[0]);
+            if (!fwd_have) flat_request_first<true, TW>(v, lev_e, nl, dl, opaque_tid(), fwdb);
+            fwd_have = false;
+            bundle_sweep_flat_ahead<true, TW>(v, xs, nullptr, st.tacc, k, lev_e, dl, nloc, nl, fwdb);
+            flat_batch_clear(fwdb);
+        }
         stamp();
         if (tid < k) ir_store(&shf[(size_t)b * k + tid], st.tacc[tid]);
         if (folded) {
             stamp();
             if (round == 0) load_top_constants();
-            if (barrier(true, pending, par ^ 1, round == 1) == IR_TIMEOUT) {
+            if (barrier(true, pending, par ^ 1, round == 1, true) == IR_TIMEOUT) {
                 if (tid == 0) ir.res[2] = 1;
                 return;
             }
@@ -1415,7 +1597,22 @@
         }
         __syncthreads();
         stamp();
-        bundle_sweep_flat<false, TW>(v, bv, b, xs, st.dxt, nullptr, k, lev_e, __builtin_amdgcn_readfirstlane(pat[0]));
+        {
+            const int dl = __builtin_amdgcn_readfirstlane(pat[0]);
+            if (!dinv_have) request_dinv();
+            if (!bwd_have) flat_request_first<false, TW>(v, lev_e, nl, dl, opaque_tid(), bwdb);
+            dinv_have = bwd_have = false;
+            const int t_ = opaque_tid();
+#pragma unroll
+            for (int u = 0; u < NPT; ++u) {
+                const int i = t_ + u * TW;
+                if (i < nloc) xs[i] *= dinv[u];
+            }
+            bundle_sweep_flat_ahead<false, TW>(v, xs, st.dxt, nullptr, k, lev_e, dl, nloc, nl, bwdb);
+            flat_batch_clear(bwdb);
+#pragma unroll
+            for (int u = 0; u < NPT; ++u) dinv[u] = 0.0;
+        }
         stamp();
         const bool more_possible = ir.ir_enable && round < ir.maxiter;
         double c[NPT];
@@ -1492,12 +1689,14 @@
             stamp();
             irs_symv<TW, NPT, NLP>(v, ir, st.runs, c, more_possible, xs, red, tacc3, k, s0, nloc, nleaf, st.candt,
                                    &pn[(size_t)par * nb + b], &shs[(size_t)par * nb * k + (size_t)b * k],
-                                   __builtin_amdgcn_readfirstlane(pat[1]));
+                                   __builtin_amdgcn_readfirstlane(pat[1]), use_desc, fl_b, fl_e,
+                                   ahead && folded && more_possible, lev_e, nl, __builtin_amdgcn_readfirstlane(pat[0]), fwdb);
+            fwd_have = ahead && folded && more_possible;
         }
         pending = true;
         if (folded && more_possible) continue;
         stamp();
-        if (barrier(false, true, par, round == 0) == IR_TIMEOUT) {
+        if (barrier(false, true, par, round == 0, false) == IR_TIMEOUT) {
             if (tid == 0) ir.res[2] = 1;
             return;
         }
diff --git a/clarabel.rs_amd/csrc/capi.cpp b/clarabel.rs_amd/csrc/capi.cpp
--- a/clarabel.rs_amd/csrc/capi.cpp
+++ b/clarabel.rs_amd/csrc/capi.cpp
@@ -206,6 +206,12 @@
     bool rhs_deferred = false;
     int *ir_run_ptr = nullptr, *ir_runs = nullptr;
     bool ir_sf = false, bp_stale = false;
+    std::vector<int> h_irs_desc;
+    int *irs_desc = nullptr;
+    bool irs_desc_shared = false;
+#ifdef CHIP_TESTING
+    std::vector<int> t_bundle_ptr, t_blvl_ptr, t_blvl, t_Lp, t_Up, t_run_ptr, t_runs, t_pat_off;
+#endif
     int pend_update = 0;
     int pend_update_ok = 1;
     std::vector<int> pend_slots;
@@ -493,6 +499,54 @@
     std::vector<int> o(n);
     for (size_t i = 0; i < n; i++) o[i] = (int)v[i];
     return o;
+}
+
+static void bundle_perm_runs(const Symbolic &S, i64 n, i64 m, std::vector<int> &rp, std::vector<int> &runs) {
+    rp.assign(1, 0);
+    runs.clear();
+    const std::vector<i32> &pm = S.perm;
+    const i64 n1 = n, n2 = n + m;
+    auto range_of = [&](i64 o) { return o < n1 ? 0 : (o < n2 ? 1 : 2); };
+    const int nb = S.bundle_ptr.empty() ? 0 : (int)S.bundle_ptr.size() - 1;
+    for (int b = 0; b < nb; b++) {
+        const int s0 = S.bundle_ptr[(size_t)b], s1 = S.bundle_ptr[(size_t)b + 1];
+        int t = s0;
+        while (t < s1) {
+            int e = t + 1;
+            while (e < s1 && pm[(size_t)e] == pm[(size_t)e - 1] + 1 && range_of(pm[(size_t)e]) == range_of(pm[(size_t)t])) e++;
+            runs.push_back(t - s0);
+            runs.push_back(pm[(size_t)t]);
+            runs.push_back(e - t);
+            t = e;
+        }
+        rp.push_back((int)(runs.size() / 3));
+    }
+}
+static std::vector<int> irs_descriptors(const Symbolic &S, const std::vector<int> &rp, const std::vector<int> &runs,
+                                        const std::vector<i32> *pat_off) {
+    const int nb = S.bundle_ptr.empty() ? 0 : (int)S.bundle_ptr.size() - 1;
+    std::vector<int> out;
+    if (nb <= 0 || (int)rp.size() != nb + 1) return out;
+    for (int b = 0; b < nb; b++)
+        if (!dev::irs_desc_fits(S.blvl_ptr[(size_t)b + 1] - S.blvl_ptr[(size_t)b] - 1, rp[(size_t)b + 1] - rp[(size_t)b])) return out;
+    out.assign((size_t)nb * dev::IRS_DESC_INTS, 0);
+    for (int b = 0; b < nb; b++) {
+        dev::IrsDesc d{};
+        const i32 *lv = S.blvl.data() + S.blvl_ptr[(size_t)b];
+        d.s0 = S.bundle_ptr[(size_t)b];
+        d.nloc = S.bundle_ptr[(size_t)b + 1] - d.s0;
+        d.nleaf = lv[1] - d.s0;
+        d.nl = S.blvl_ptr[(size_t)b + 1] - S.blvl_ptr[(size_t)b] - 1;
+        d.dl = pat_off ? (*pat_off)[2 * (size_t)b] : 0;
+        d.du = pat_off ? (*pat_off)[2 * (size_t)b + 1] : 0;
+        d.fb = S.Up[(size_t)(d.s0 + d.nleaf)];
+        d.fe = S.Up[(size_t)(d.s0 + d.nloc)];
+        d.nruns = rp[(size_t)b + 1] - rp[(size_t)b];
+        for (int l = 0; l <= d.nl; l++) d.lev_e[l] = S.Lp[(size_t)lv[l]];
+        std::copy_n(&runs[3 * (size_t)rp[(size_t)b]], 3 * (size_t)d.nruns, d.runs);
+        std::memcpy(&out[(size_t)b * dev::IRS_DESC_INTS], &d, sizeof d);
+    }
+    return out;
 }
 
 int32_t chip_kkt_create(chip_kkt **out, int64_t n, int64_t m, const uint64_t *Pcolptr,
@@ -538,6 +592,7 @@
     clk("analysis (total)");
     Engine &E = h->E;
     PatternShare pat;
+    bool pat_cand = false;
     {
         const i32 nbun = S.bundle_ptr.empty() ? 0 : (i32)S.bundle_ptr.size() - 1;
         bool cand = !S.Li16.empty() && S.gf_ng == 0 && S.nfold >= 1 && nbun > 0;
@@ -551,8 +606,25 @@
             E.note_patterns(pat);
             clk("pattern classes");
         }
+        pat_cand = cand;
+    }
+    const bool pat_shared = !pat.off.empty() && !pat.mismatches && !switches().no_shared_pattern;
+    std::vector<int> run_ptr, runs;
+    if (pat_cand) {
+        bundle_perm_runs(S, K.n, K.m, run_ptr, runs);
+        bool fit = true;
+        for (size_t b = 0; b + 1 < run_ptr.size() && fit; b++) fit = run_ptr[b + 1] - run_ptr[b] <= dev::IRS_DESC_RUNS;
+        if (fit) h->h_irs_desc = irs_descriptors(S, run_ptr, runs, pat_shared ? &pat.off : nullptr);
+        clk("bundle descriptors");
     }
     if (st.device == CHIP_DEVICE_HOST_ONLY) {
+#ifdef CHIP_TESTING
+        if (pat_cand) {
+            h->t_bundle_ptr = S.bundle_ptr, h->t_blvl_ptr = S.blvl_ptr, h->t_blvl = S.blvl;
+            h->t_Lp = S.Lp, h->t_Up = S.Up, h->t_run_ptr = run_ptr, h->t_runs = runs;
+            if (pat_shared) h->t_pat_off = pat.off;
+        }
+#endif
         E.init_host_only(S, st);
         *out = h.release();
         return CHIP_OK;
@@ -798,23 +870,8 @@
     if ((rc = E.alloc(&h->d_tmp, h->tmp_len))) return rc;
     CHIP_HIP(hipMemset(h->wk[0].bp, 0, (size_t)(K.N ? K.N : 1) * sizeof(double)));
     if (E.ir_fused) {
-        std::vector<int> rp(1, 0), runs;
-        const std::vector<i32> &pm = E.h_perm;
-        const i64 n1 = K.n, n2 = K.n + K.m;
-        auto range_of = [&](i64 o) { return o < n1 ? 0 : (o < n2 ? 1 : 2); };
-        for (int b = 0; b < E.bundles.nb; b++) {
-            const int s0 = S.bundle_ptr[(size_t)b], s1 = S.bundle_ptr[(size_t)b + 1];
-            int t = s0;
-            while (t < s1) {
-                int e = t + 1;
-                while (e < s1 && pm[(size_t)e] == pm[(size_t)e - 1] + 1 && range_of(pm[(size_t)e]) == range_of(pm[(size_t)t])) e++;
-                runs.push_back(t - s0);
-                runs.push_back(pm[(size_t)t]);
-                runs.push_back(e - t);
-                t = e;
-            }
-            rp.push_back((int)(runs.size() / 3));
-        }
+        if (run_ptr.empty()) bundle_perm_runs(S, K.n, K.m, run_ptr, runs);
+        const std::vector<int> &rp = run_ptr;
         if (!runs.empty() && (i64)(runs.size() / 3) * 64 <= (i64)E.NF) {
             if ((rc = E.upload(&h->ir_run_ptr, rp, rp.size()))) return rc;
             if ((rc = E.upload(&h->ir_runs, runs, runs.size()))) return rc;
@@ -828,6 +885,10 @@
             }
             h->ir_sf = sf && dev::bundle_irs_capacity_ok(E.bundles);
             if (h->ir_sf && !switches().no_shared_pattern && (rc = E.upload_patterns(pat))) return rc;
+            if (h->ir_sf && !h->h_irs_desc.empty() && (E.pat_off != nullptr) == pat_shared &&
+                (rc = E.upload(&h->irs_desc, h->h_irs_desc, h->h_irs_desc.size())))
+                return rc;
+            h->irs_desc_shared = pat_shared;
         }
     }
     clk("maps, cone tables");
@@ -1430,7 +1491,7 @@
             return a && b_ && a < b_ + nb_ && b_ < a + na;
         };
         const size_t n = (size_t)h->K.n, m = (size_t)h->K.m;
-        const int flags = switches().irs_flags < 0 ? 3 : switches().irs_flags;
+        const int flags = (switches().irs_flags < 0 ? 3 : switches().irs_flags) & ~dev::IRS_F_DESC;
         ir.sf_flags = flags;
         ir.spec_out = (flags & 2) && !(overlap(lhsx_dev, n, ir.rx, n) || overlap(lhsx_dev, n, ir.rz, m) || overlap(lhsz_dev, m, ir.rx, n) ||
                         overlap(lhsz_dev, m, ir.rz, m));
@@ -1456,6 +1517,10 @@
             lv.Ucol16 = E.pat_Ucol16;
             lv.Urow16 = E.pat_Urow16;
             ir.pat_off = E.pat_off;
+        }
+        if (h->irs_desc && !(ir.sf_flags & (dev::IRS_F_CHAINED)) && h->irs_desc_shared == (ir.pat_off != nullptr)) {
+            ir.desc = (const dev::IrsDesc *)h->irs_desc;
+            ir.sf_flags |= dev::IRS_F_DESC;
         }
         rc = dev::bundle_ir(E.stream, lv, E.bundles, E.fold, ir, E.ir_grid, E.ir_tw, E.gfold);
     } else {
@@ -2118,7 +2183,31 @@
     else if (k == "pattern_mismatches") *out = E.pat_mismatches;
     else if (k == "pattern_shared_bundles")
         *out = (h->ir_sf && E.pat_off && !switches().no_shared_pattern) ? E.bundles.nb : 0;
+    else if (k == "irs_desc_bundles") {
+        const bool shared = E.pat_off && !switches().no_shared_pattern;
+        const int flags = switches().irs_flags < 0 ? 3 : switches().irs_flags;
+        *out = (h->ir_sf && h->irs_desc && !(flags & dev::IRS_F_CHAINED) && h->irs_desc_shared == shared) ? E.bundles.nb : 0;
+    }
     else return fail(CHIP_ERR_ARG, "chip_debug_counter: unknown name");
+    return CHIP_OK;
+}
+int32_t chip_debug_kkt_ints(const void *handle, const char *name, int64_t *len, int32_t *out) {
+    const chip_kkt *h = (const chip_kkt *)handle;
+    if (!h || !name || !len) return fail(CHIP_ERR_ARG, "chip_debug_kkt_ints: bad argument");
+    const std::string k(name);
+    const std::vector<int> *v = nullptr;
+    if (k == "irs_desc") v = &h->h_irs_desc;
+    else if (k == "bundle_ptr") v = &h->t_bundle_ptr;
+    else if (k == "blvl_ptr") v = &h->t_blvl_ptr;
+    else if (k == "blvl") v = &h->t_blvl;
+    else if (k == "Lp") v = &h->t_Lp;
+    else if (k == "Up") v = &h->t_Up;
+    else if (k == "run_ptr") v = &h->t_run_ptr;
+    else if (k == "runs") v = &h->t_runs;
+    else if (k == "pat_off") v = &h->t_pat_off;
+    else return fail(CHIP_ERR_ARG, "chip_debug_kkt_ints: unknown name");
+    *len = (int64_t)v->size();
+    if (out) std::copy(v->begin(), v->end(), out);
     return CHIP_OK;
 }
 int32_t chip_debug_psd_create(void **out, int64_t ncones, const int64_t *dims) {
diff --git a/clarabel.rs_amd/csrc/grid_sync.hpp b/clarabel.rs_amd/csrc/grid_sync.hpp
--- a/clarabel.rs_amd/csrc/grid_sync.hpp
+++ b/clarabel.rs_amd/csrc/grid_sync.hpp
@@ -77,6 +77,24 @@
     }
     __syncthreads();
     return s_state2;
+}
+template <class F> __device__ __forceinline__ int ir_arrive_nowait_issue(int *ctl, int gen, int nwg, F &&issue) {
+    __shared__ int s_state5;
+    __syncthreads();
+    if (threadIdx.x == 0) {
+        __builtin_amdgcn_fence(__ATOMIC_RELEASE, "workgroup");
+        __builtin_amdgcn_s_waitcnt(0);
+        const int sub = blockIdx.x % IR_NSUB;
+        const int members = nwg / IR_NSUB + (sub < nwg % IR_NSUB ? 1 : 0);
+        int state = IR_WAITED;
+        if (atomicAdd(ctl + 32 * (1 + sub), 1) + 1 == members * gen) {
+            if (atomicAdd(ctl, 1) + 1 == min(IR_NSUB, nwg) * gen) state = IR_LAST;
+        }
+        s_state5 = state;
+    }
+    issue();
+    lds_barrier();
+    return s_state5;
 }
 __device__ __forceinline__ int ir_wait_word(const int *word, int gen) {
     __shared__ int s_state3;
diff --git a/clarabel.rs_amd/csrc/kernels.hpp b/clarabel.rs_amd/csrc/kernels.hpp
--- a/clarabel.rs_amd/csrc/kernels.hpp
+++ b/clarabel.rs_amd/csrc/kernels.hpp
@@ -121,6 +121,23 @@
 void bundle_bwd(hipStream_t s, const LdlView &v, const BundleView &bv, double *x, const double *addv);
 void bundle_symv(hipStream_t s, const BundleView &bv, const int *Up, const int *Ucol, const double *Ux,
                  const double *x, const double *b, double *e, unsigned long long *nrm, int *nan, const FoldView &fold, hipEvent_t ev0 = nullptr, hipEvent_t ev1 = nullptr);
+constexpr int IRS_DESC_LEVELS = 19;
+constexpr int IRS_DESC_RUNS = 32;
+struct alignas(16) IrsDesc {
+    int s0, nloc, nleaf, nl;
+    int dl, du;
+    int fb, fe;
+    int nruns, pad[3];
+    int lev_e[IRS_DESC_LEVELS + 1];
+    int runs[3 * IRS_DESC_RUNS];
+};
+static_assert(sizeof(IrsDesc) == 512, "IrsDesc: 128 ints, read as one dword per lane by two waves");
+constexpr int IRS_DESC_INTS = (int)(sizeof(IrsDesc) / sizeof(int));
+inline bool irs_desc_fits(int nlevels, int nruns) { return nlevels >= 1 && nlevels <= IRS_DESC_LEVELS && nruns >= 1 && nruns <= IRS_DESC_RUNS; }
+constexpr int IRS_F_X0_REGS = 1;
+constexpr int IRS_F_SPEC_OUT = 2;
+constexpr int IRS_F_CHAINED = 4;
+constexpr int IRS_F_DESC = 256;
 struct IrView {
     const double *rx, *rz;
     int n, m, N;
@@ -131,6 +148,7 @@
     union {
         double *ebuf;
         const int *pat_off;
+        const IrsDesc *desc;
     };
     double *lhsx, *lhsz;
     double *part;
diff --git a/include/clarabel_hip_testing.h b/include/clarabel_hip_testing.h
--- a/include/clarabel_hip_testing.h
+++ b/include/clarabel_hip_testing.h
@@ -7,6 +7,7 @@
 int32_t chip_debug_spin(int32_t device, int32_t blocks, int32_t threads, int32_t lds_bytes, double usec);
 int32_t chip_debug_set_switch(const char *name, const char *value_or_null);
 int32_t chip_debug_counter(const void *kkt_handle, const char *name, double *out);
+int32_t chip_debug_kkt_ints(const void *kkt_handle, const char *name, int64_t *len, int32_t *out);
 int32_t chip_comm_debug_spin(void *comm, int32_t blocks, int32_t threads, double usec);
 int32_t chip_debug_transform_create(void **out, int64_t n, int64_t m, const uint64_t *Pcolptr, const uint64_t *Prowval,
                                     const double *Pnzval, const double *q, const uint64_t *Acolptr,
```
